# samuel-vitorino/sopro

Measured on AMD Instinct MI355X. Metric: audio_seconds_per_second, higher is better.
Workload: dtype f32; 1 GPU; Sopro-135M synthesize, 32 utterances x 200 frames per GPU (BASELINE configs[1]), S=64 text tokens, 32 distinct 150-frame reference voice(s) per batch prepared outside the timed region, top_p=0.9 T=1.05 anti_loop (reference defaults), synthetic weights with EOS suppressed; batch_per_gpu=32, frames=200, voices_per_batch=32, parallelism=replicas x1 (utterance sharding, no collective), lanes_per_gpu=4

## Files before the change

include/sopro_hip.h:

```cpp
#ifndef SOPRO_HIP_H
#define SOPRO_HIP_H

#include <stdint.h>

#ifdef __cplusplus
extern "C" {
#endif

#define SOPRO_ABI_VERSION 43

const char* sopro_last_error(void);
int sopro_abi_version(void);
int sopro_build_flags(void);
int sopro_set_lds_floor(int bytes);
int sopro_set_host_wait(int blocking);
int sopro_device_info(int device, int* out4);

int sopro_capture_begin(void* stream);
int sopro_capture_end(void* stream, void** graph_exec_out);
int sopro_graph_launch(void* graph_exec, void* stream);
int sopro_graph_launch_n(void* graph_exec, void* stream, int32_t n);
int sopro_graph_destroy(void* graph_exec);
int sopro_stream_create_cu_range(int first_cu, int n_cus, void** stream_out);
int sopro_stream_create_cu_mask(const uint32_t* mask, int32_t words, void** stream_out);
int sopro_stream_destroy(void* stream);
int sopro_host_alloc(int64_t bytes, void** out);
int sopro_host_free(void* p);
int sopro_copy_to_host_async(void* dst_host, const void* src_dev, int64_t bytes, void* stream);

enum { SOPRO_PRO_NONE = 0, SOPRO_PRO_ELU = 1, SOPRO_PRO_ADDVEC = 2 };
enum { SOPRO_EPI_NONE = 0, SOPRO_EPI_GELU = 1, SOPRO_EPI_GLU = 2, SOPRO_EPI_RES = 3, SOPRO_EPI_TANH = 4,
       SOPRO_EPI_GLU_DW = 5 ,
       SOPRO_EPI_ROPE = 6  };

typedef struct sopro_gemm_args {
  const float* A; int64_t lda; int64_t a_seg_stride;
  const float* W; int64_t ldw;
  const float* bias;
  float* C; int64_t ldc; int64_t c_seg_stride;
  const float* R; int64_t ldr; int64_t r_seg_stride;
  const float* scale;
  const float* pro_vec;
  long long* dbg;
  int32_t M, N, K, rows_per_seg;
  int32_t prologue, epilogue;
} sopro_gemm_args;
int sopro_gemm_f32(const sopro_gemm_args* args, void* stream);
int sopro_gemm_set_tile_override(int cfg);

typedef struct sopro_gemm_split_ext {
  int32_t a_format;
  int32_t c_mode;
  float* C2; int64_t ldc2; int64_t c2_seg_stride;
  int32_t rms_norm; float rms_eps;
  int32_t ksplit;
  int32_t n_tickets;
  float* ws; int64_t ws_bytes;
  int32_t* tickets;
  int32_t group_m;
  float acc_scale;
  int32_t* range_events;
  const float* rope_cos; const float* rope_sin;
  int32_t rope_cols, rope_dh, rope_pos0, rope_rows_per_seg;
  const float* ln_stats;
  float* ln_stats_out;
} sopro_gemm_split_ext;
int sopro_gemm_bf16x3(const sopro_gemm_args* a, const void* packed_w, const sopro_gemm_split_ext* ext, void* stream);
int64_t sopro_packed_w_rows_bytes(int32_t N, int32_t K);
int sopro_pack_w_rows_bf16(const float* W, int64_t ldw, int32_t N, int32_t K, void* packed, void* stream);
int sopro_gemm_8p_takes(const sopro_gemm_args* a, const sopro_gemm_split_ext* ext);
int sopro_gemm_bf16x3_8p(const sopro_gemm_args* a, const void* w_rows, const sopro_gemm_split_ext* ext, void* stream);
int sopro_gemm_bf16x6(const sopro_gemm_args* a, const void* packed_w, const sopro_gemm_split_ext* ext, void* stream);
int sopro_gemm_bf16x1(const sopro_gemm_args* a, const void* packed_w, const sopro_gemm_split_ext* ext, void* stream);
int sopro_pack_w_bf16(const float* W, int64_t ldw, int32_t N, int32_t K, int32_t pieces, void* packed, void* stream);
int sopro_pack_w_f16x2(const float* W, int64_t ldw, int32_t N, int32_t K, float wscale, void* packed, void* stream);
float sopro_f16x3_a_scale(void);
int sopro_gemm_f16x3(const sopro_gemm_args* a, const void* packed_w, const sopro_gemm_split_ext* ext, void* stream);
int64_t sopro_packed_w_bytes(int32_t N, int32_t K, int32_t pieces);
int sopro_gemm_bf16_set_tile_override(int cfg);
int sopro_gemm_set_group_m(int g);
int sopro_gemm_auto_ksplit(int32_t M, int32_t N, int32_t K, int32_t pieces, int32_t f16, int32_t epilogue, int64_t ws_bytes, int32_t n_tickets);

typedef struct sopro_skinny_args {
  const float* X; int64_t ldx;
  const float* W; int64_t ldw;
  const float* bias;
  float* Y; int64_t ldy;
  const float* R; int64_t ldr;
  const float* scale;
  float* ring;
  const float* dw_w;
  const float* dw_b;
  const int32_t* step;
  const float* Xp; int64_t xp_stride;
  int64_t y_part_stride;
  long long* dbg;
  float eps;
  int32_t B, N, K, epilogue;
  int32_t ring_len, ring_bcap, dil, ksize;
  int32_t np, ksplit, rms_norm;
  int32_t w_layout;
  const float* aux_W; const float* aux_bias; const float* aux_R; float* aux_Y;
  int64_t aux_ldy, aux_ldr, aux_y_part_stride;
  int32_t aux_tiles, aux_flags;
  int32_t ring_format;
  int32_t mt, nt;
} sopro_skinny_args;
int sopro_skinny_f32(const sopro_skinny_args* args, void* stream);
int sopro_pack_skinny_w(const float* W, int64_t ldw, int32_t N, int32_t K, int32_t glu, float* out, void* stream);
int64_t sopro_skinny_packed_floats(int32_t N, int32_t K, int32_t glu);
int sopro_pack_skinny_w_bf16(const float* W, int64_t ldw, int32_t N, int32_t K, int32_t glu, void* out, void* stream);

int sopro_fill2d_u32(void* p, int64_t pitch, int32_t rows, int32_t width, uint32_t value, void* stream);
int sopro_copy2d_u32(void* dst, int64_t dpitch, const void* src, int64_t spitch, int32_t rows, int32_t width, void* stream);
int sopro_nar_seed_i32(int32_t* tokens, int32_t Q, const int32_t* cb0, int64_t cb0_bstride, int32_t B, int32_t T, int32_t vmax, void* stream);
int sopro_cvt_f32_bf16(const float* src, void* dst, int64_t n, void* stream);
int sopro_cvt_bf16_f32(const void* src, float* dst, int64_t n, void* stream);
enum { SOPRO_NORM_RMS = 0, SOPRO_NORM_LN = 1 };
int sopro_norm_f32(const float* x, int64_t ldx, int64_t x_seg_stride , float* out, int64_t ldo, const float* w, const float* b,
                   const float* mul, const float* add, int32_t rows, int32_t rows_per_seg, int32_t C,
                   float eps, int32_t kind, void* stream);
int sopro_row_stats_f32(const float* x, int64_t ldx, int64_t x_seg_stride , int32_t rows, int32_t rows_per_seg, int32_t C,
                        float* stats, void* stream);
int sopro_rms_match_f32(const float* a, const float* x, float* out, int32_t rows, int32_t C, void* stream);
int sopro_tanh_affine_f32(const float* in, float* out, float c0, float c1, int64_t n, void* stream);
int sopro_add_pos_f32(const float* rowvec, const float* table, float* out, int32_t B, int32_t T, int32_t C,
                      int32_t pos0, void* stream);
int sopro_masked_mean_f32(const float* x, const int32_t* lens, float* out, int32_t B, int32_t T, int32_t C,
                          void* stream);

int sopro_stats_pool_f32(const float* h, const float* logit, const int32_t* lens, float* out, int32_t B, int32_t T,
                         int32_t C, void* stream);
int sopro_l2norm_f32(const float* x, float* out, int32_t rows, int32_t C, float eps, void* stream);

int sopro_dwconv_f32(const float* x, const float* w, const float* bias, const float* res, float* out,
                     const int32_t* lens, int32_t B, int32_t T, int32_t C, int32_t ksize, int32_t dil,
                     int32_t left, int32_t mode, void* stream);

int sopro_codebook_sum_f32(const int32_t* tok, int32_t ldt, const int32_t* col, const int32_t* off, const float* wq,
                           int32_t nq, const float* table, int64_t table_rows, const float* base, float alpha,
                           float beta, float* out, int64_t ldo, int64_t o_seg_stride, int32_t rows,
                           int32_t rows_per_seg, int32_t D, void* stream);
int sopro_text_embed_f32(const int32_t* ids, const int32_t* lens, const float* table, int64_t table_rows,
                         const float* pe, float* out, int32_t B, int32_t T, int32_t C, void* stream);
int sopro_argmax_rows_f32(const float* x, int64_t ldx, int32_t* out, int64_t ldo, int32_t inner, int32_t rows, int32_t N,
                          void* stream);
int sopro_argmax_partials_i32(const float* partials, int64_t ldp, int32_t* out, int64_t ldo, int32_t heads, int32_t per_head, int32_t V,
                              int32_t rows, void* stream);

int sopro_fir1_f32(const float* x, int64_t x_seg_stride, int32_t n_in, const float* w, const float* bias, float* out,
                   int64_t ldo, int64_t o_seg_stride, int32_t B, int32_t n_out, int32_t C, int32_t K, int32_t stride,
                   int32_t left, void* stream);
int sopro_rvq_assign_f32(const float* scores, int64_t lds, int32_t V, const float* table, float* res, int64_t ldr,
                         int32_t D, int32_t* codes, int64_t ldc, int32_t rows, void* stream);

typedef struct sopro_attn_args {
  const float* Q; int64_t ldq; int64_t q_bstride;
  const float* K; int64_t ldk; int64_t k_bstride;
  const float* V; int64_t ldv; int64_t v_bstride;
  float* O; int64_t ldo; int64_t o_bstride;
  const int32_t* klens;
  int32_t B, H, dh, Tq, Tk;
  int32_t causal, q_pos0, k_pos0, window;
  float scale;
  const int32_t* kv_index;
} sopro_attn_args;
int sopro_attention_f32(const sopro_attn_args* args, void* stream);
int sopro_attention_split_bf16(const sopro_attn_args* args, int32_t passes, void* stream);
int sopro_attn_decode_f32(const sopro_attn_args* args, void* stream);
typedef struct sopro_xattn_args {
  const float* X; int64_t ldx;
  const float* Xp; int64_t xp_stride;
  const float* norm_w;
  const float* Kp; const float* Vp;
  const int32_t* klens;
  float* Y; int64_t y_part_stride;
  float eps, gate, scale;
  int32_t np, B, H, D, S_cap;
  const float* Qp; int64_t qp_stride;
  int32_t nqp, k_unfolded;
  int32_t kv_format;
} sopro_xattn_args;
int sopro_xattn_step_f32(const sopro_xattn_args* args, void* stream);

int sopro_rope_f32(float* x, int64_t ldx, const float* cos_t, const float* sin_t, int32_t rows,
                   int32_t rows_per_seg, int32_t pos0, int32_t H, int32_t dh, void* stream);

int sopro_upsample2_f32(const float* x, const float* w, float* y, int64_t y_seg_stride, int32_t B, int32_t T,
                        int32_t C, void* stream);
int sopro_final_conv_f32(const float* h, int64_t h_seg_stride, const float* w, float bias, float* wav,
                         int64_t wav_seg_stride, int32_t B, int32_t T, void* stream);

int sopro_seanet_tail_f32(const float* h, int64_t h_seg_stride, const float* w1, const float* b1, const float* w2,
                          const float* b2, const float* wf, float bf, float* wav, int64_t wav_seg_stride, int32_t B,
                          int32_t T, void* stream);
int sopro_seanet_tail_p_f32(const float* h, int64_t h_seg_stride, const float* w1, const float* b1, const float* w2,
                            const float* b2, const float* wf, float bf, float* wav, int64_t wav_seg_stride, int32_t B,
                            int32_t T, int32_t passes, void* stream);
int sopro_seanet_res128_f32(const float* h, int64_t h_seg_stride, const float* w1, const float* b1, const float* w2, const float* b2,
                            float* out, int64_t out_seg_stride, int32_t B, int32_t T, void* stream);
int sopro_seanet_res128_p_f32(const float* h, int64_t h_seg_stride, const float* w1, const float* b1, const float* w2, const float* b2,
                              float* out, int64_t out_seg_stride, int32_t B, int32_t T, int32_t passes , void* stream);
int sopro_seanet_res_set_tiles(int tiles);
int sopro_seanet_up128_f32(const float* x, int64_t x_seg_stride, const float* w, const float* bias, float* out,
                           int64_t out_seg_stride, int32_t B, int32_t T, int32_t passes, void* stream);
int sopro_seanet_res128_bf16(const void* h, int64_t h_seg_stride, const float* w1, const float* b1, const float* w2, const float* b2,
                             void* out, int64_t out_seg_stride, int32_t B, int32_t T, void* stream);
int sopro_seanet_up128_bf16(const void* x, int64_t x_seg_stride, const float* w, const float* bias, void* out, int64_t out_seg_stride,
                            int32_t B, int32_t T, void* stream);
int sopro_seanet_tail_bf16(const void* h, int64_t h_seg_stride, const float* w1, const float* b1, const float* w2, const float* b2,
                           const float* wf, float bf, float* wav, int64_t wav_seg_stride, int32_t B, int32_t T, void* stream);
int sopro_seanet_up_set_tiles(int tiles);
int sopro_seanet_uptail_f32(const float* x, int64_t x_seg_stride, const float* wu, const float* bu, const float* w1, const float* b1,
                            const float* w2, const float* b2, const float* wf, float bf, float* wav, int64_t wav_seg_stride, int32_t B,
                            int32_t T, int32_t passes, void* stream);
int sopro_seanet_uptail_bf16(const void* x, int64_t x_seg_stride, const float* wu, const float* bu, const float* w1, const float* b1,
                             const float* w2, const float* b2, const float* wf, float bf, float* wav, int64_t wav_seg_stride, int32_t B,
                             int32_t T, void* stream);
int sopro_seanet_uptail_set_tiles(int tiles);
int sopro_seanet_tail_set_tiles(int tiles);

typedef struct sopro_prof_row {
  char family[40];
  int64_t launches, gpu_bound;
// ... 251 lines not shown
```

sopro_amd/csrc/gemm_8p.hip:

```cpp
#include "common.h"
#include "gemm_epilogue.h"
#include "gemm_host.h"

namespace {

constexpr int P_BM = 256, P_BN = 256, P_NT = 512;
constexpr int P_ROWB = 128;
constexpr int P_TILE = 256 * P_ROWB;
constexpr int P_BUF = 2 * P_TILE;
constexpr int P_LDS = 2 * P_BUF;
constexpr int P_CLD = 128 + 4;
static_assert(2 * 64 * P_CLD * 4 <= P_LDS, "epilogue tiles alias the operand buffers");

typedef __bf16 pbf16x8 __attribute__((ext_vector_type(8)));
typedef unsigned pu32x4 __attribute__((ext_vector_type(4)));
typedef __attribute__((address_space(3))) void p_lds_void;
typedef const __attribute__((address_space(1))) void p_glb_void;

__device__ __forceinline__ pbf16x8 pfrag(const pu32x4& v) { return __builtin_bit_cast(pbf16x8, v); }
__device__ __forceinline__ void dma16(const void* g, unsigned lds_off) {
  __builtin_amdgcn_global_load_lds((p_glb_void*)(uintptr_t)g, (p_lds_void*)(uintptr_t)lds_off, 16, 0, 0);
}

template <int EPI, int OUT>
__global__ __launch_bounds__(P_NT, 1) void gemm_8p_kernel(const sopro_gemm_args g, const unsigned char* __restrict__ Wr, const sopro_gemm_split_ext ext) {
  extern __shared__ __attribute__((aligned(1024))) unsigned char smem[];
  const int tid = threadIdx.x, lane = tid & 63, wave = __builtin_amdgcn_readfirstlane(tid >> 6);
  const int wm = wave >> 2, wn = wave & 3;
  const int ntn = g.N / P_BN;
  const int bid = xcd_contiguous((int)blockIdx.x, (int)gridDim.x);
  int mt = bid / ntn, nt = bid % ntn;
  if (ext.group_m > 1) {
    const int ntm_all = (g.M + P_BM - 1) / P_BM;
    const int per = ext.group_m * ntn;
    const int grp = bid / per, rem = bid - grp * per;
    const int first = grp * ext.group_m;
    const int gsz = min(ntm_all - first, ext.group_m);
    mt = first + rem % gsz;
    nt = rem / gsz;
  }
  const int m0 = mt * P_BM, n0 = nt * P_BN;
  const int KT = g.K >> 5;
  const int64_t ldw = (int64_t)g.K * 4;

  const unsigned char* asrc[2][2];
  const unsigned char* wsrc[2][2];
  const int rps = g.rows_per_seg;
#pragma unroll
  for (int h = 0; h < 2; ++h)
#pragma unroll
    for (int q = 0; q < 2; ++q) {
      const int r = 128 * h + 8 * (wave + 8 * q) + (lane >> 3);
      const int ch = (lane & 7) ^ ((r >> 1) & 7);
      const int m = min(m0 + r, g.M - 1);
      const int seg = m / rps, rr = m - seg * rps;
      asrc[h][q] = reinterpret_cast<const unsigned char*>(g.A) + ((int64_t)seg * g.a_seg_stride + (int64_t)rr * g.lda) * 4 + ch * 16;
      wsrc[h][q] = Wr + (int64_t)(n0 + r) * ldw + ch * 16;
    }
  const unsigned lds0 = (unsigned)(uintptr_t)smem;
  auto issue_one = [&](bool isW, int h, int kt, int buf, int q) {
    const int ktc = min(kt, KT - 1);
    const unsigned char* src = (isW ? wsrc[h][q] : asrc[h][q]) + (int64_t)ktc * P_ROWB;
    dma16(src, lds0 + buf * P_BUF + (isW ? P_TILE : 0) + (128 * h + 8 * (wave + 8 * q)) * P_ROWB);
  };

  const int frow = lane & 31, fg = lane >> 5;
  const int swz = (frow >> 1) & 7;
  int foff[2][2];
#pragma unroll
  for (int p = 0; p < 2; ++p)
#pragma unroll
    for (int s = 0; s < 2; ++s) foff[p][s] = ((p * 4 + s * 2 + fg) ^ swz) * 16;
  const int arow = (wm * 32 + frow) * P_ROWB;
  const int brow = (wn * 32 + frow) * P_ROWB;

  f32x16 acc[4][2];
#pragma unroll
  for (int i = 0; i < 4; ++i)
#pragma unroll
    for (int j = 0; j < 2; ++j)
#pragma unroll
      for (int r = 0; r < 16; ++r) acc[i][j][r] = 0.f;

  pu32x4 af[2][2][2];
  pu32x4 bf[2][2][2];
  auto read_a = [&](int buf, int qi) {
    const unsigned char* base = smem + buf * P_BUF + arow + qi * 2 * 64 * P_ROWB;
#pragma unroll
    for (int i = 0; i < 2; ++i)
#pragma unroll
      for (int s = 0; s < 2; ++s)
#pragma unroll
        for (int p = 0; p < 2; ++p) af[i][s][p] = *reinterpret_cast<const pu32x4*>(base + i * 64 * P_ROWB + foff[p][s]);
  };
  auto read_b = [&](int buf, int j) {
    const unsigned char* base = smem + buf * P_BUF + P_TILE + brow + j * 128 * P_ROWB;
#pragma unroll
    for (int s = 0; s < 2; ++s)
#pragma unroll
      for (int p = 0; p < 2; ++p) bf[j][s][p] = *reinterpret_cast<const pu32x4*>(base + foff[p][s]);
  };
  auto phase_mfma = [&](int qi, int j, bool isW, int h, int kt, int buf) {
    constexpr int PA[3] = {1, 0, 0}, PB[3] = {0, 1, 0};
    int n = 0;
#pragma unroll
    for (int s = 0; s < 2; ++s)
#pragma unroll
      for (int q = 0; q < 3; ++q)
#pragma unroll
        for (int i = 0; i < 2; ++i) {
          acc[qi * 2 + i][j] = __builtin_amdgcn_mfma_f32_32x32x16_bf16(pfrag(af[i][s][PA[q]]), pfrag(bf[j][s][PB[q]]), acc[qi * 2 + i][j], 0, 0, 0);
          ++n;
          if (n == 4 || n == 8) {
            __builtin_amdgcn_sched_barrier(0);
            issue_one(isW, h, kt, buf, n == 4 ? 0 : 1);
            __builtin_amdgcn_sched_barrier(0);
          }
        }
  };
#define P_PHASE(QI, J, W_, H_, KT_, B_)                     \
  asm volatile("s_waitcnt vmcnt(6)" ::: "memory");          \
  __builtin_amdgcn_s_barrier();                             \
  asm volatile("s_waitcnt lgkmcnt(0)" ::: "memory");        \
  __builtin_amdgcn_sched_barrier(0);                        \
  __builtin_amdgcn_s_setprio(1);                            \
  phase_mfma(QI, J, W_, H_, KT_, B_);                       \
  __builtin_amdgcn_s_setprio(0);                            \
  __builtin_amdgcn_sched_barrier(0);                        \
  __builtin_amdgcn_s_barrier();

#pragma unroll
  for (int q = 0; q < 2; ++q) issue_one(false, 0, 0, 0, q);
#pragma unroll
  for (int q = 0; q < 2; ++q) issue_one(true, 0, 0, 0, q);
#pragma unroll
  for (int q = 0; q < 2; ++q) issue_one(true, 1, 0, 0, q);
#pragma unroll
  for (int q = 0; q < 2; ++q) issue_one(false, 1, 0, 0, q);
#pragma unroll
  for (int q = 0; q < 2; ++q) issue_one(false, 0, 1, 1, q);
#pragma unroll
  for (int q = 0; q < 2; ++q) issue_one(true, 0, 1, 1, q);
  asm volatile("s_waitcnt vmcnt(8)" ::: "memory");
  __builtin_amdgcn_s_barrier();
  if (wm == 1) __builtin_amdgcn_s_barrier();

  for (int t = 0; t < KT; ++t) {
    const int b = t & 1;
    read_a(b, 0);
    read_b(b, 0);
    P_PHASE(0, 0, true, 1, t + 1, b ^ 1)
    read_b(b, 1);
    P_PHASE(0, 1, false, 1, t + 1, b ^ 1)
    read_a(b, 1);
    P_PHASE(1, 1, false, 0, t + 2, b)
    P_PHASE(1, 0, true, 0, t + 2, b)
  }
#undef P_PHASE
  if (wm == 0) __builtin_amdgcn_s_barrier();
  asm volatile("s_waitcnt vmcnt(0)" ::: "memory");
  __syncthreads();

  float* Cs[2] = {reinterpret_cast<float*>(smem), reinterpret_cast<float*>(smem) + 64 * P_CLD};
#pragma unroll
  for (int i = 0; i < 4; ++i)
#pragma unroll
    for (int j = 0; j < 2; ++j) {
      const int nb = n0 + 128 * j;
      const int n = nb + wn * 32 + frow;
      const float bv[1] = {(g.bias && n < g.N) ? g.bias[n] : 0.f};
      gemm_store_tile<2, 4, 1, 1, EPI, OUT>(g, Cs[(i * 2 + j) & 1], reinterpret_cast<f32x16(&)[1][1]>(acc[i][j]), bv, m0 + 64 * i, nb, &ext, nullptr);
    }
}

__global__ __launch_bounds__(256) void pack_w_rows_kernel(const float* __restrict__ W, int64_t ldw, int N, int K, uint4* __restrict__ out, int64_t total) {
  const int64_t i = (int64_t)blockIdx.x * blockDim.x + threadIdx.x;
  if (i >= total) return;
  const int c = (int)(i & 7);
  const int64_t gi = i >> 3;
  const int kg = (int)(gi % (K >> 5));
  const int n = (int)(gi / (K >> 5));
  const float* src = W + (int64_t)n * ldw + kg * 32 + (c & 3) * 8;
  unsigned w[4];
#pragma unroll
  for (int e = 0; e < 4; ++e) {
    unsigned hi, lo;
    split2_bf16(src[2 * e], src[2 * e + 1], hi, lo);
    w[e] = (c >> 2) ? lo : hi;
  }
  out[i] = make_uint4(w[0], w[1], w[2], w[3]);
}

template <int EPI, int OUT>
int launch_8p(const sopro_gemm_args& g, const void* wrows, const sopro_gemm_split_ext& ext, hipStream_t s) {
  auto kern = gemm_8p_kernel<EPI, OUT>;
  SOPRO_SET_MAX_LDS_ONCE(kern, P_LDS);
  const int ntm = (g.M + P_BM - 1) / P_BM, ntn = g.N / P_BN;
  hipLaunchKernelGGL(kern, dim3(ntm * ntn), dim3(P_NT), P_LDS, s, g, reinterpret_cast<const unsigned char*>(wrows), ext);
  SOPRO_LAUNCH_CHECK();
}

}

extern "C" int64_t sopro_packed_w_rows_bytes(int32_t N, int32_t K) {
  if (N <= 0 || K <= 0 || (K & 31) != 0) return 0;
  return (int64_t)N * K * 4;
}

extern "C" int sopro_pack_w_rows_bf16(const float* W, int64_t ldw, int32_t N, int32_t K, void* packed, void* stream) {
  SOPRO_CHECK_ARG(W && packed && N > 0 && K > 0 && ldw >= K, "bad pointers or sizes");
  SOPRO_CHECK_ARG((K & 31) == 0 && (ldw & 1) == 0 && (reinterpret_cast<uintptr_t>(W) & 7u) == 0, "K % 32 == 0, 8-byte aligned rows");
  SOPRO_CHECK_ARG((reinterpret_cast<uintptr_t>(packed) & 127u) == 0, "packed must be 128-byte aligned");
  const int64_t total = (int64_t)N * (K >> 5) * 8;
  hipLaunchKernelGGL(pack_w_rows_kernel, dim3((unsigned)((total + 255) / 256)), dim3(256), 0, (hipStream_t)stream, W, ldw, N, K,
                     reinterpret_cast<uint4*>(packed), total);
  SOPRO_LAUNCH_CHECK();
}

extern "C" int sopro_gemm_8p_takes(const sopro_gemm_args* a, const sopro_gemm_split_ext* x) {
  if (!a || !x) return 0;
  if (x->a_format != 1 || a->prologue != SOPRO_PRO_NONE || a->epilogue != SOPRO_EPI_NONE || x->rms_norm || x->ln_stats || x->ln_stats_out) return 0;
  if (x->ksplit > 1) return 0;
  if (!(x->c_mode == 0 || x->c_mode == 1 || x->c_mode == 2 || x->c_mode == 4)) return 0;
  if ((a->N % P_BN) != 0 || (a->K & 31) != 0 || a->K < 1024) return 0;
  const int64_t tiles = (int64_t)((a->M + P_BM - 1) / P_BM) * (a->N / P_BN);
  return tiles >= 128 ? 1 : 0;
}

extern "C" int sopro_gemm_bf16x3_8p(const sopro_gemm_args* a, const void* w_rows, const sopro_gemm_split_ext* x, void* stream) {
  SOPRO_CHECK_ARG(a != nullptr && x != nullptr && w_rows != nullptr, "args / ext / w_rows is NULL");
  sopro_gemm_args g = *a;
  sopro_gemm_split_ext ext = *x;
  if (int rc = gemm_check_basic(__func__, g, &ext, w_rows, GEMM_SPLIT_ROWS)) return rc;
  SOPRO_CHECK_ARG((g.N % P_BN) == 0 && (g.K & 31) == 0, "the long-K form takes N % 256 == 0, K % 32 == 0");
  SOPRO_CHECK_ARG(ext.a_format == 1 && g.prologue == SOPRO_PRO_NONE, "A must be split-form rows (a_format 1, no prologue)");
  SOPRO_CHECK_ARG(g.epilogue == SOPRO_EPI_NONE && !ext.rms_norm && !ext.ln_stats && !ext.ln_stats_out && ext.ksplit <= 1,
                  "epilogue NONE, no fused norm, no split-K");
  SOPRO_CHECK_ARG(g.A && g.C && (reinterpret_cast<uintptr_t>(g.A) & 127u) == 0 && (g.lda & 31) == 0 && (g.a_seg_stride & 31) == 0,
                  "split-form A: 128-byte aligned base, lda / a_seg_stride multiples of 32");
  SOPRO_CHECK_ARG((reinterpret_cast<uintptr_t>(w_rows) & 127u) == 0, "w_rows must be 128-byte aligned (sopro_pack_w_rows_bf16)");
  SOPRO_CHECK_ARG(ext.c_mode == 0 || ext.c_mode == 1 || ext.c_mode == 2 || ext.c_mode == 4, "c_mode must be 0, 1, 2 or 4");
  if (int rc = gemm_check_out_rows(__func__, g, ext, true)) return rc;
  hipStream_t s = reinterpret_cast<hipStream_t>(stream);
  switch (ext.c_mode) {
    case 0: return launch_8p<SOPRO_EPI_NONE, 0>(g, w_rows, ext, s);
    case 1: return launch_8p<SOPRO_EPI_NONE, 1>(g, w_rows, ext, s);
    case 2: return launch_8p<SOPRO_EPI_NONE, 2>(g, w_rows, ext, s);
    default: return launch_8p<SOPRO_EPI_NONE, 4>(g, w_rows, ext, s);
  }
}
```

sopro_amd/csrc/gemm_bf16s.hip:

```cpp
#include "common.h"
#include "gemm_epilogue.h"
#include "gemm_host.h"

namespace {

constexpr int BK = 32;


typedef __bf16 bf16x8 __attribute__((ext_vector_type(8)));
typedef _Float16 f16x8 __attribute__((ext_vector_type(8)));
typedef _Float16 f16x2_t __attribute__((ext_vector_type(2)));

__device__ __forceinline__ bf16x8 as_frag(const uint4& v) { return *reinterpret_cast<const bf16x8*>(&v); }
__device__ __forceinline__ f16x8 as_frag16(const uint4& v) { return *reinterpret_cast<const f16x8*>(&v); }

constexpr float A16_SCALE = 8.0f;

template <int NPL, bool F16 = false>
__device__ __forceinline__ void split_pair(float x, float y, unsigned (&pc)[NPL]) {
#pragma unroll
  for (int p = 0; p < NPL; ++p) {
    const f32x2_t v = {x, y};
    if constexpr (F16) {
      const f16x2_t h = __builtin_convertvector(v, f16x2_t);
      pc[p] = *reinterpret_cast<const unsigned*>(&h);
      x -= (float)h[0];
      y -= (float)h[1];
    } else {
      const bf16x2_t h = __builtin_convertvector(v, bf16x2_t);
      pc[p] = *reinterpret_cast<const unsigned*>(&h);
      x -= __uint_as_float(pc[p] << 16);
      y -= __uint_as_float(pc[p] & 0xffff0000u);
    }
  }
}

template <int NPL, int WM, int WN, int TM, int TN, int EPI, int AMODE, int OUT, bool SK, bool F16 = false>
__global__ __launch_bounds__(WM* WN * 64) void gemm_bf16s_kernel(const sopro_gemm_args g, const uint4* __restrict__ Wp,
                                                                 int ksubs, const sopro_gemm_split_ext ext) {
  constexpr int AROW = NPL * 64 + 16;
  constexpr bool FOLD = F16;
  constexpr int NT = WM * WN * 64;
  constexpr int BM = WM * TM * 32;
  constexpr int BN = WN * TN * 32;
  constexpr int A_F4 = BM * 8 / NT;
  constexpr int RSTEP = NT / 8;
  extern __shared__ float4 smem4[];
  unsigned char* As = reinterpret_cast<unsigned char*>(smem4);

  const int tid = threadIdx.x, lane = tid & 63, wave = tid >> 6;
  const int wm = wave / WN, wn = wave % WN;
  const int ntn = (g.N + BN - 1) / BN;
  const int bid = xcd_contiguous((int)blockIdx.x, (int)gridDim.x);
  int mt = bid / ntn, nt = bid % ntn;
  if (ext.group_m > 1) {
    const int ntm_all = (g.M + BM - 1) / BM;
    const int per = ext.group_m * ntn;
    const int grp = bid / per, rem = bid - grp * per;
    const int first = grp * ext.group_m;
    const int gsz = min(ntm_all - first, ext.group_m);
    mt = first + rem % gsz;
    nt = rem / gsz;
  }
  const int m0 = mt * BM, n0 = nt * BN;
  const int lrow = tid >> 3, lc4 = tid & 7;
  const int rps = g.rows_per_seg;
  long long* dbg = g.dbg ? g.dbg + (int64_t)blockIdx.x * 8 : nullptr;
  if (dbg && tid == 0) dbg[0] = clock64();

  static_assert(AMODE != 5 || NPL == 1, "bf16 rows are a one-pass (bf16 mode) operand form");
  constexpr int AES = AMODE == 5 ? 2 : 4;
  const char* ap[A_F4];
#pragma unroll
  for (int i = 0; i < A_F4; ++i) {
    const int m = min(m0 + lrow + i * RSTEP, g.M - 1);
    const int seg = m / rps;
    const int r = m - seg * rps;
    ap[i] = reinterpret_cast<const char*>(g.A) + ((int64_t)seg * g.a_seg_stride + (int64_t)r * g.lda) * AES;
  }
  const int ntiles = (g.N + 31) >> 5;
  const uint4* bp[TN];
#pragma unroll
  for (int j = 0; j < TN; ++j) {
    const int t = min((n0 >> 5) + wn * TN + j, ntiles - 1);
    bp[j] = Wp + ((int64_t)t * ksubs * NPL) * 64 + lane;
  }
  int boff[TN];
#pragma unroll
  for (int j = 0; j < TN; ++j) {
    const int t = min((n0 >> 5) + wn * TN + j, ntiles - 1);
    boff[j] = (t * ksubs * NPL) * 64 + lane;
  }
  float biasv[TN];
#pragma unroll
  for (int j = 0; j < TN; ++j) {
    const int n = n0 + (wn * TN + j) * 32 + (lane & 31);
    biasv[j] = (g.bias && n < g.N) ? g.bias[n] : 0.f;
  }

  float4 raA[A_F4], raB[A_F4];
  float ssq[A_F4];
  float rsc[A_F4];
  float a16max = 0.f;
#pragma unroll
  for (int i = 0; i < A_F4; ++i) { ssq[i] = 0.f; rsc[i] = A16_SCALE; }
  float sapin[A_F4];
#pragma unroll
  for (int i = 0; i < A_F4; ++i) sapin[i] = A16_SCALE;
  float lmu[A_F4], lrs[A_F4];
  float4 pvA = make_float4(0.f, 0.f, 0.f, 0.f), pvB = pvA;
  const int KT = (g.K + BK - 1) / BK;
  const int klast = g.K - 4;

  auto gload = [&](int kt, float4 (&ra)[A_F4], float4& pv) {
    const int k = min(kt * BK + lc4 * 4, klast);
    if constexpr (AMODE == 5) {
#pragma unroll
      for (int i = 0; i < A_F4; ++i) {
        const uint2 v = *reinterpret_cast<const uint2*>(ap[i] + (int64_t)k * 2);
        ra[i].x = __uint_as_float(v.x);
        ra[i].y = __uint_as_float(v.y);
      }
    } else {
#pragma unroll
      for (int i = 0; i < A_F4; ++i) ra[i] = *reinterpret_cast<const float4*>(ap[i] + (int64_t)k * 4);
    }
    if (AMODE == 3) pv = *reinterpret_cast<const float4*>(g.pro_vec + k);
  };
  auto bload = [&](int kt, uint4 (&rb)[TN][2][NPL]) {
#pragma unroll
    for (int j = 0; j < TN; ++j)
#pragma unroll
      for (int s = 0; s < 2; ++s)
#pragma unroll
        for (int p = 0; p < NPL; ++p) rb[j][s][p] = bp[j][((int64_t)(kt * 2 + s) * NPL + p) * 64];
  };
  auto lstore_piece = [&](int buf, float4 (&ra)[A_F4], const float4& pv, int i, bool fresh, bool first) {
    if constexpr (FOLD) {
      if constexpr (AMODE == 4) asm volatile("" : "+v"(rsc[i]), "+v"(ssq[i]));
      else asm volatile("" : "+v"(sapin[i]));
    }
    if constexpr (AMODE == 5) {
      unsigned char* a = As + buf * BM * AROW + lrow * AROW + lc4 * 8;
      *reinterpret_cast<uint2*>(a + i * RSTEP * AROW) = make_uint2(__float_as_uint(ra[i].x), __float_as_uint(ra[i].y));
    } else if constexpr (AMODE == 2) {
      unsigned char* a = As + buf * BM * AROW + lrow * AROW + lc4 * 16;
      *reinterpret_cast<f32x4*>(a + i * RSTEP * AROW) = (f32x4){ra[i].x, ra[i].y, ra[i].z, ra[i].w};
    } else {
      if constexpr (AMODE == 1) {
        ra[i].x = eluf_(ra[i].x); ra[i].y = eluf_(ra[i].y); ra[i].z = eluf_(ra[i].z); ra[i].w = eluf_(ra[i].w);
      } else if constexpr (AMODE == 3) {
        ra[i].x += pv.x; ra[i].y += pv.y; ra[i].z += pv.z; ra[i].w += pv.w;
      } else if constexpr (AMODE == 6) {
        const f32x2_t r2 = {lrs[i], lrs[i]}, n2 = {lmu[i], lmu[i]};
        const f32x2_t lo2 = (f32x2_t){ra[i].x, ra[i].y} * r2 + n2, hi2 = (f32x2_t){ra[i].z, ra[i].w} * r2 + n2;
        ra[i].x = lo2[0]; ra[i].y = lo2[1]; ra[i].z = hi2[0]; ra[i].w = hi2[1];
      }
      if constexpr (AMODE == 4) {
        if (fresh) ssq[i] = fmaf(ra[i].x, ra[i].x, fmaf(ra[i].y, ra[i].y, fmaf(ra[i].z, ra[i].z, fmaf(ra[i].w, ra[i].w, ssq[i]))));
      }
      unsigned char* a = As + buf * BM * AROW + lrow * AROW + lc4 * 8;
      {
        unsigned c0[NPL], c1[NPL];
        if constexpr (F16) {
          const float F16MAX = 65504.0f;
          if constexpr (AMODE == 4) {
            if (first) {
              float mx = fmaxf(fmaxf(fabsf(ra[i].x), fabsf(ra[i].y)), fmaxf(fabsf(ra[i].z), fabsf(ra[i].w)));
              mx = fmaxf(mx, __shfl_xor(mx, 1, 64));
              mx = fmaxf(mx, __shfl_xor(mx, 2, 64));
              mx = fmaxf(mx, __shfl_xor(mx, 4, 64));
              const int ex = (int)((__float_as_uint(mx) >> 23) & 255u);
              rsc[i] = (ex == 0 || ex == 255) ? A16_SCALE : __uint_as_float((unsigned)min(max(261 - ex, 2), 252) << 23);
            }
          }
          const float sa = AMODE == 4 ? rsc[i] : sapin[i];
          const float vx = ra[i].x * sa, vy = ra[i].y * sa, vz = ra[i].z * sa, vw = ra[i].w * sa;
          a16max = fmaxf(a16max, fmaxf(fmaxf(fabsf(vx), fabsf(vy)), fmaxf(fabsf(vz), fabsf(vw))));
          split_pair<NPL, true>(__builtin_amdgcn_fmed3f(vx, -F16MAX, F16MAX), __builtin_amdgcn_fmed3f(vy, -F16MAX, F16MAX), c0);
          split_pair<NPL, true>(__builtin_amdgcn_fmed3f(vz, -F16MAX, F16MAX), __builtin_amdgcn_fmed3f(vw, -F16MAX, F16MAX), c1);
        } else {
          split_pair<NPL>(ra[i].x, ra[i].y, c0);
          split_pair<NPL>(ra[i].z, ra[i].w, c1);
        }
#pragma unroll
        for (int p = 0; p < NPL; ++p) *reinterpret_cast<uint2*>(a + i * RSTEP * AROW + p * 64) = make_uint2(c0[p], c1[p]);
      }
    }
  };
  auto lstore = [&](int buf, float4 (&ra)[A_F4], const float4& pv, bool fresh = true, bool first = false) {
#pragma unroll
    for (int i = 0; i < A_F4; ++i) lstore_piece(buf, ra, pv, i, fresh, first);
  };

  f32x16 acc[TM][TN];
#pragma unroll
  for (int i = 0; i < TM; ++i)
#pragma unroll
    for (int j = 0; j < TN; ++j)
#pragma unroll
      for (int r = 0; r < 16; ++r) acc[i][j][r] = 0.f;

  const int frow = lane & 31, fg = lane >> 5;
  constexpr int NPAIR = NPL == 1 ? 1 : (NPL == 2 ? 3 : 6);
  constexpr int PA[6] = {NPL == 1 ? 0 : (NPL == 2 ? 1 : 2), 0, NPL == 2 ? 0 : 1, 1, 0, 0};
  constexpr int PB[6] = {0, NPL == 2 ? 1 : 2, NPL == 2 ? 0 : 1, 0, 1, 0};
  auto compute = [&](int buf, const uint4 (&rb)[TN][2][NPL]) {
    const unsigned char* a = As + buf * BM * AROW + (wm * TM * 32 + frow) * AROW + fg * 16;
#pragma unroll
    for (int s = 0; s < 2; ++s) {
      uint4 af[TM][NPL];
#pragma unroll
      for (int i = 0; i < TM; ++i)
#pragma unroll
        for (int p = 0; p < NPL; ++p) af[i][p] = *reinterpret_cast<const uint4*>(a + i * 32 * AROW + p * 64 + s * 32);
#pragma unroll
      for (int q = 0; q < NPAIR; ++q)
#pragma unroll
        for (int i = 0; i < TM; ++i)
#pragma unroll
          for (int j = 0; j < TN; ++j)
            if constexpr (F16)
              acc[i][j] = __builtin_amdgcn_mfma_f32_32x32x16_f16(as_frag16(af[i][PA[q]]), as_frag16(rb[j][s][PB[q]]), acc[i][j], 0, 0, 0);
            else
              acc[i][j] = __builtin_amdgcn_mfma_f32_32x32x16_bf16(as_frag(af[i][PA[q]]), as_frag(rb[j][s][PB[q]]), acc[i][j], 0, 0, 0);
    }
  };

  auto compute_spread = [&](int buf, const uint4 (&rb)[TN][2][NPL], int kA, float4 (&ra)[A_F4], float4& pv, int kB, uint4 (&rbn)[TN][2][NPL],
                            float4 (&rs)[A_F4], const float4& pvs, bool fresh_s) {
    constexpr int NB = TN * 2 * NPL, NL = NB + A_F4, NM = 2 * NPAIR * TM * TN;
    constexpr int STRIDE = NM / NL > 0 ? NM / NL : 1;
    const int kcol = min(kA * BK + lc4 * 4, klast);
    if (AMODE == 3) pv = *reinterpret_cast<const float4*>(g.pro_vec + kcol);
    auto issue = [&](int n) {
      if (n < NB) {
        const int j = n / (2 * NPL), ss = (n / NPL) % 2, p = n % NPL;
        const uint4* wk = Wp + (int64_t)__builtin_amdgcn_readfirstlane(kB) * (2 * NPL * 64);
        rbn[j][ss][p] = wk[boff[j] + (ss * NPL + p) * 64];
      } else if (n < NL) {
        const int i = n - NB;
        if constexpr (AMODE == 5) {
          const uint2 v = *reinterpret_cast<const uint2*>(ap[i] + (int64_t)kcol * 2);
          ra[i].x = __uint_as_float(v.x);
          ra[i].y = __uint_as_float(v.y);
        } else {
          ra[i] = *reinterpret_cast<const float4*>(ap[i] + (int64_t)kcol * 4);
        }
      }
    };
    const unsigned char* a = As + buf * BM * AROW + (wm * TM * 32 + frow) * AROW + fg * 16;
    int m = 0, nl = 0;
#pragma unroll
    for (int s = 0; s < 2; ++s) {
      uint4 af[TM][NPL];
#pragma unroll
      for (int i = 0; i < TM; ++i)
#pragma unroll
        for (int p = 0; p < NPL; ++p) af[i][p] = *reinterpret_cast<const uint4*>(a + i * 32 * AROW + p * 64 + s * 32);
#pragma unroll
      for (int q = 0; q < NPAIR; ++q)
#pragma unroll
        for (int i = 0; i < TM; ++i)
#pragma unroll
          for (int j = 0; j < TN; ++j) {
            if constexpr (F16)
              acc[i][j] = __builtin_amdgcn_mfma_f32_32x32x16_f16(as_frag16(af[i][PA[q]]), as_frag16(rb[j][s][PB[q]]), acc[i][j], 0, 0, 0);
            else
              acc[i][j] = __builtin_amdgcn_mfma_f32_32x32x16_bf16(as_frag(af[i][PA[q]]), as_frag(rb[j][s][PB[q]]), acc[i][j], 0, 0, 0);
            ++m;
            if constexpr (FOLD) {
#pragma unroll
              for (int i = 0; i < A_F4; ++i)
                if (m == NM / 2 + i * (NM / 2) / A_F4) {
                  __builtin_amdgcn_sched_barrier(0x104);
                  lstore_piece(buf ^ 1, rs, pvs, i, fresh_s, false);
                }
            }
            if (m % STRIDE == 0 && nl < NL) {
              if constexpr (NPL == 1) {
                __builtin_amdgcn_sched_barrier(0);
                issue(nl++);
                __builtin_amdgcn_sched_barrier(0);
              } else {
                __builtin_amdgcn_sched_barrier(0x786);
                issue(nl++);
                __builtin_amdgcn_sched_barrier(0x786);
              }
            }
          }
    }
#pragma unroll
    for (int n = 0; n < NL; ++n)
      if (n >= nl) issue(n);
  };

  const int KS = SK ? ext.ksplit : 1;
  const int per = (KT + KS - 1) / KS;
  const int kt0 = (int)blockIdx.y * per;
  const int nkt = max(0, min(KT, kt0 + per) - kt0);
  const int ktl = max(kt0, kt0 + nkt - 1);

  uint4 rb0[TN][2][NPL], rb1[TN][2][NPL];
  constexpr bool DEEP = true;
  gload(min(kt0, KT - 1), raA, pvA);
  bload(min(kt0, KT - 1), rb0);
  if (DEEP) gload(min(min(kt0 + 1, ktl), KT - 1), raB, pvB);
  if constexpr (AMODE == 6) {
    const int P = g.K >> 6;
#pragma unroll
    for (int i = 0; i < A_F4; ++i) {
      const float2* st = reinterpret_cast<const float2*>(ext.ln_stats) + (int64_t)min(m0 + lrow + i * RSTEP, g.M - 1) * P;
      float sm = 0.f;
      for (int p = lc4; p < P; p += 8) sm += st[p].x;
      sm += __shfl_xor(sm, 1, 64); sm += __shfl_xor(sm, 2, 64); sm += __shfl_xor(sm, 4, 64);
      const float mean = sm / (float)P;
      float m2 = 0.f;
      for (int p = lc4; p < P; p += 8) {
        const float2 v = st[p];
        const float d = v.x - mean;
        m2 += fmaf(64.0f * d, d, v.y);
      }
      m2 += __shfl_xor(m2, 1, 64); m2 += __shfl_xor(m2, 2, 64); m2 += __shfl_xor(m2, 4, 64);
      lrs[i] = rsqrtf(m2 / (float)g.K + ext.rms_eps);
      lmu[i] = -mean * lrs[i];
    }
  }
  lstore(0, raA, pvA, true, true);
  __syncthreads();
  if (dbg && tid == 0) dbg[1] = clock64();
  {
    int it = 0;
    for (; it + 1 < nkt; it += 2) {
      const int k1 = min(kt0 + it + 1, ktl), k2 = min(kt0 + it + 2, ktl), k3 = min(kt0 + it + 3, ktl);
      compute_spread(0, rb0, k2, raA, pvA, k1, rb1, raB, pvB, true);
      if constexpr (!FOLD) lstore(1, raB, pvB, true);
      __syncthreads();
      compute_spread(1, rb1, k3, raB, pvB, k2, rb0, raA, pvA, it + 2 < nkt);
      if constexpr (!FOLD) lstore(0, raA, pvA, it + 2 < nkt);
      __syncthreads();
    }
    if (it < nkt) {
      compute(0, rb0);
      __syncthreads();
    }
  }
  if (dbg && tid == 0) dbg[2] = clock64();
  if constexpr (SK) {
    constexpr int PER_THREAD = TM * TN * 16;
    const int tile = bid, ntile = gridDim.x;
    float* mine = ext.ws + ((int64_t)((int64_t)blockIdx.y * ntile + tile) * NT + tid) * PER_THREAD;
#pragma unroll
    for (int i = 0; i < TM; ++i)
#pragma unroll
      for (int j = 0; j < TN; ++j)
#pragma unroll
        for (int r = 0; r < 16; r += 4)
          *reinterpret_cast<float4*>(mine + (i * TN + j) * 16 + r) = make_float4(acc[i][j][r], acc[i][j][r + 1], acc[i][j][r + 2], acc[i][j][r + 3]);
    __syncthreads();
    int* flag = reinterpret_cast<int*>(smem4);
    if (tid == 0) {
      __atomic_thread_fence(__ATOMIC_RELEASE);
      const int old = __hip_atomic_fetch_add(ext.tickets + tile, 1, __ATOMIC_ACQ_REL, __HIP_MEMORY_SCOPE_AGENT);
      *flag = old;
      if (old == KS - 1) __hip_atomic_store(ext.tickets + tile, 0, __ATOMIC_RELAXED, __HIP_MEMORY_SCOPE_AGENT);
    }
    __syncthreads();
    if (*flag != KS - 1) return;
    __atomic_thread_fence(__ATOMIC_ACQUIRE);
    __syncthreads();
#pragma unroll
    for (int i = 0; i < TM; ++i)
#pragma unroll
      for (int j = 0; j < TN; ++j)
#pragma unroll
        for (int r = 0; r < 16; ++r) acc[i][j][r] = 0.f;
    const int64_t sl_stride = (int64_t)ntile * NT * PER_THREAD;
    const float* part0 = ext.ws + ((int64_t)tile * NT + tid) * PER_THREAD;
    for (int s0 = 0; s0 < KS; s0 += 16) {
#pragma unroll
      for (int i = 0; i < TM; ++i)
#pragma unroll
        for (int j = 0; j < TN; ++j)
#pragma unroll
          for (int r = 0; r < 16; r += 4) {
            f32x4 v[16];
#pragma unroll
            for (int u = 0; u < 16; ++u) {
              const int sl = min(s0 + u, KS - 1);
              v[u] = __builtin_nontemporal_load(reinterpret_cast<const f32x4*>(part0 + sl * sl_stride + (i * TN + j) * 16 + r));
            }
#pragma unroll
            for (int u = 0; u < 16; ++u) {
              if (s0 + u < KS) {
                acc[i][j][r] += v[u][0]; acc[i][j][r + 1] += v[u][1]; acc[i][j][r + 2] += v[u][2]; acc[i][j][r + 3] += v[u][3];
              }
            }
          }
    }
  }
  float cscale = 1.0f;
  if constexpr (F16) {
    cscale = AMODE == 4 ? ext.acc_scale * A16_SCALE : ext.acc_scale;
    if (ext.range_events && !(a16max <= 65504.0f)) atomicAdd(ext.range_events, 1);
  }
  const float* rs = nullptr;
  if constexpr (AMODE == 4) {
    float* rsl = reinterpret_cast<float*>(smem4) + BM * (BN + 4);
#pragma unroll
    for (int i = 0; i < A_F4; ++i) {
      float v = ssq[i];
      v += __shfl_xor(v, 1, 64);
      v += __shfl_xor(v, 2, 64);
      v += __shfl_xor(v, 4, 64);
      float r = rsqrtf(v / (float)g.K + ext.rms_eps);
      if constexpr (F16) r *= __uint_as_float(0x7f000000u - __float_as_uint(rsc[i])) * cscale;
      if (lc4 == 0) rsl[lrow + i * RSTEP] = r;
    }
    __syncthreads();
    rs = rsl;
  }
  gemm_store_tile<WM, WN, TM, TN, EPI, OUT>(g, reinterpret_cast<float*>(smem4), acc, biasv, m0, n0, &ext, rs, cscale);
  if (dbg && tid == 0) dbg[3] = clock64();
}

template <int NPL, bool F16 = false>
__global__ __launch_bounds__(256) void pack_w_kernel(const float* __restrict__ W, int64_t ldw, int N, int K, uint4* __restrict__ out,
                                                     int ksubs, int64_t total, float wscale = 1.0f) {
  const int64_t i = (int64_t)blockIdx.x * blockDim.x + threadIdx.x;
  if (i >= total) return;
  const int lane = (int)(i & 63);
  const int64_t pk = i >> 6;
  const int p = (int)(pk % NPL);
  const int64_t tk = pk / NPL;
  const int ks = (int)(tk % ksubs);
  const int t = (int)(tk / ksubs);
  const int n = t * 32 + (lane & 31);
  const int k0 = ks * 16 + (lane >> 5) * 8;
  unsigned w[4];
#pragma unroll
  for (int e = 0; e < 4; ++e) {
    const int k = k0 + 2 * e;
    const float x = (n < N && k < K) ? W[(int64_t)n * ldw + k] : 0.f;
    const float y = (n < N && k + 1 < K) ? W[(int64_t)n * ldw + k + 1] : 0.f;
    unsigned pc[NPL];
    if constexpr (F16) split_pair<NPL, true>(x * wscale, y * wscale, pc);
    else split_pair<NPL>(x, y, pc);
    w[e] = pc[p];
  }
  out[i] = make_uint4(w[0], w[1], w[2], w[3]);
}

template <int NPL, int WM, int WN, int TM, int TN, int EPI, int AMODE, int OUT, bool F16 = false>
int launch_one(const sopro_gemm_args& g, const uint4* wp, int ksubs, const sopro_gemm_split_ext& ext, hipStream_t s) {
  constexpr int BM = WM * TM * 32, BN = WN * TN * 32;
  constexpr size_t lds_main = (size_t)2 * BM * (NPL * 64 + 16), lds_epi = (size_t)BM * (BN + 4 + (AMODE == 4 ? 1 : 0)) * sizeof(float);
  constexpr size_t lds = lds_main > lds_epi ? lds_main : lds_epi;
  const int ks = ext.ksplit > 1 ? ext.ksplit : 1;
  auto kern = ks > 1 ? gemm_bf16s_kernel<NPL, WM, WN, TM, TN, EPI, AMODE, OUT, true, F16> : gemm_bf16s_kernel<NPL, WM, WN, TM, TN, EPI, AMODE, OUT, false, F16>;
  constexpr size_t lds_cap = lds > (size_t)96 * 1024 ? lds : (size_t)96 * 1024;
  if (ks > 1) SOPRO_SET_MAX_LDS_ONCE(kern, lds_cap);
  else SOPRO_SET_MAX_LDS_ONCE(kern, lds_cap);
  const size_t lds_req = lds > (size_t)g_sopro_lds_floor ? lds : (size_t)g_sopro_lds_floor;
  const int ntm = (g.M + BM - 1) / BM, ntn = (g.N + BN - 1) / BN;
  if (ks > 1) {
    const int64_t need = (int64_t)ks * ntm * ntn * BM * BN * (int64_t)sizeof(float);
    if (!ext.ws || !ext.tickets || ext.ws_bytes < need || ext.n_tickets < ntm * ntn) {
      sopro_set_error("split-K needs a %lld-byte workspace and %d tickets (got %lld, %d)", (long long)need, ntm * ntn,
                      (long long)ext.ws_bytes, ext.n_tickets);
      return -2;
    }
  }
  hipLaunchKernelGGL(kern, dim3(ntm * ntn, ks), dim3(WM * WN * 64), lds_req, s, g, wp, ksubs, ext);
  SOPRO_LAUNCH_CHECK();
}

inline int amode_of(const sopro_gemm_args& g, const sopro_gemm_split_ext& ext) {
  if (ext.a_format == 1) return 2;
  if (ext.a_format == 2) return 5;
  if (ext.rms_norm) return 4;
  if (ext.ln_stats) return 6;
  return g.prologue == SOPRO_PRO_ELU ? 1 : (g.prologue == SOPRO_PRO_ADDVEC ? 3 : 0);
}

template <int NPL, int WM, int WN, int TM, int TN>
int launch_cfg3(const sopro_gemm_args& g, const uint4* wp, int ksubs, const sopro_gemm_split_ext& ext, hipStream_t s) {
  const int key = g.epilogue * 100 + amode_of(g, ext) * 10 + ext.c_mode;
#define SOPRO_CASE(E, A, O) \
  case (E) * 100 + (A) * 10 + (O): return launch_one<NPL, WM, WN, TM, TN, ((E) == SOPRO_EPI_GELU ? SOPRO_EPI_GELU_FAST : (E)), A, O>(g, wp, ksubs, ext, s)
  switch (key) {
    SOPRO_CASE(SOPRO_EPI_NONE, 0, 0);
    SOPRO_CASE(SOPRO_EPI_GELU, 0, 0);
    SOPRO_CASE(SOPRO_EPI_RES, 0, 0);
    SOPRO_CASE(SOPRO_EPI_ROPE, 0, 0);
    SOPRO_CASE(SOPRO_EPI_NONE, 6, 0);
    SOPRO_CASE(SOPRO_EPI_GELU, 6, 0);
    SOPRO_CASE(SOPRO_EPI_ROPE, 6, 0);
    SOPRO_CASE(SOPRO_EPI_NONE, 1, 0);
    SOPRO_CASE(SOPRO_EPI_RES, 1, 0);
    SOPRO_CASE(SOPRO_EPI_NONE, 0, 3);
    SOPRO_CASE(SOPRO_EPI_NONE, 0, 4);
    SOPRO_CASE(SOPRO_EPI_RES, 0, 3);
    default: break;
  }
  if constexpr (NPL == 1) {
    switch (key) {
      SOPRO_CASE(SOPRO_EPI_NONE, 0, 7);
      SOPRO_CASE(SOPRO_EPI_NONE, 5, 8);
      SOPRO_CASE(SOPRO_EPI_NONE, 5, 7);
      SOPRO_CASE(SOPRO_EPI_RES, 5, 7);
      SOPRO_CASE(SOPRO_EPI_NONE, 5, 6);
      SOPRO_CASE(SOPRO_EPI_NONE, 5, 0);
      default: break;
    }
  }
  if constexpr (NPL == 2) {
    switch (key) {
      SOPRO_CASE(SOPRO_EPI_NONE, 0, 1);
      SOPRO_CASE(SOPRO_EPI_NONE, 0, 2);
      SOPRO_CASE(SOPRO_EPI_NONE, 2, 0);
      SOPRO_CASE(SOPRO_EPI_NONE, 2, 1);
      SOPRO_CASE(SOPRO_EPI_NONE, 2, 2);
      SOPRO_CASE(SOPRO_EPI_NONE, 2, 4);
      SOPRO_CASE(SOPRO_EPI_RES, 2, 1);
      default: break;
    }
  }
#undef SOPRO_CASE
  sopro_set_error("sopro_gemm_bf16x%d: (epilogue %d, prologue %d, a_format %d, c_mode %d) is not an available combination",
                  NPL == 2 ? 3 : NPL, g.epilogue, g.prologue, ext.a_format, ext.c_mode);
  return -2;
}

template <int NPL, int WM, int WN, int TM, int TN, bool F16 = false>
int launch_cfg6(const sopro_gemm_args& g, const uint4* wp, int ksubs, const sopro_gemm_split_ext& ext, hipStream_t s) {
  const int key = g.epilogue * 10 + amode_of(g, ext);
#define SOPRO_CASE(E, A) \
  case (E) * 10 + (A): return launch_one<NPL, WM, WN, TM, TN, (((E) == SOPRO_EPI_GELU && (F16 || NPL != 3)) ? SOPRO_EPI_GELU_FAST : (E)), A, 0, F16>(g, wp, ksubs, ext, s)
  switch (key) {
    SOPRO_CASE(SOPRO_EPI_NONE, 0);
    SOPRO_CASE(SOPRO_EPI_GELU, 0);
    SOPRO_CASE(SOPRO_EPI_RES, 0);
    SOPRO_CASE(SOPRO_EPI_NONE, 3);
    SOPRO_CASE(SOPRO_EPI_GELU, 4);
    SOPRO_CASE(SOPRO_EPI_NONE, 4);
    default: break;
  }
#undef SOPRO_CASE
  if constexpr (WN * TN * 32 >= 64) {
    constexpr int GLU_ = (F16 || NPL != 3) ? SOPRO_EPI_GLU_FAST : SOPRO_EPI_GLU;
    if (key == SOPRO_EPI_GLU * 10) return launch_one<NPL, WM, WN, TM, TN, GLU_, 0, 0, F16>(g, wp, ksubs, ext, s);
    if (key == SOPRO_EPI_GLU * 10 + 4) return launch_one<NPL, WM, WN, TM, TN, GLU_, 4, 0, F16>(g, wp, ksubs, ext, s);
  }
  sopro_set_error("sopro_gemm_%s: (epilogue %d, prologue %d) is not an available combination", F16 ? "f16x3" : (NPL == 3 ? "bf16x6" : "bf16x1"), g.epilogue, g.prologue);
  return -2;
}

#define SOPRO_TILES(X) \
  X(T64, 2, 2, 1, 1) X(T64x128, 2, 2, 1, 2) X(T128x64, 2, 2, 2, 1) X(T128, 2, 2, 2, 2) X(T256x128, 2, 2, 4, 2) X(T128_W8, 2, 4, 2, 1) X(T128_W1x4, 1, 4, 4, 1)
#define SOPRO_TILE(T, WM, WN, TM, TN) T,
enum Tile { SOPRO_TILES(SOPRO_TILE) };
#undef SOPRO_TILE
struct TileSize { int bm, bn; };
TileSize tile_size(Tile t) {
#define SOPRO_TILE(T, WM, WN, TM, TN) if (t == T) return {WM * TM * 32, WN * TN * 32};
  SOPRO_TILES(SOPRO_TILE)
#undef SOPRO_TILE
  return {0, 0};
}

enum Family { BF16X1, BF16X3, BF16X6, F16X3 };

Tile default_tile(Family f, int M, int N, int epilogue) {
  const Tile small = epilogue == SOPRO_EPI_GLU ? T64x128 : T64;
  switch (f) {
    case BF16X3:
      return (N <= 64 || M <= 64) ? T64 : T128;
    case BF16X1: {
      const int64_t t128 = (int64_t)((M + 127) / 128) * ((N + 127) / 128);
      return (N <= 64 || M <= 64 || t128 < 256) ? small : T128;
    }
    case BF16X6:
      return small;
    case F16X3:
      return M >= 8192 ? T128 : small;
  }
  return T64;
}

enum Form { FORM_CFG3, FORM_CFG6, FORM_ARGMAX };

template <int NPL, bool F16, Form FORM>
constexpr bool has_tile(Tile t) {
#ifdef SOPRO_DEV_SWITCHES
  if (t == T128_W1x4) return NPL == 2 && FORM == (F16 ? FORM_CFG6 : FORM_CFG3);
#endif
  if (t == T64 || t == T128) return true;
  if (FORM != FORM_CFG3) return t == (FORM == FORM_ARGMAX ? T128x64 : T64x128);
  return NPL == 2 && (t == T128x64 || t == T256x128 || t == T128_W8);
}

struct Call {
  sopro_gemm_args g;
  sopro_gemm_split_ext ext;
  const uint4* wp;
  int ksubs;
  hipStream_t s;
};

template <int NPL, bool F16, Form FORM>
int launch_tile(Tile t, const Call& c) {
  switch (t) {
#define SOPRO_TILE(T, WM, WN, TM, TN)                                                                                                     \
  case T:                                                                                                                                 \
    if constexpr (!has_tile<NPL, F16, FORM>(T)) break;                                                                                    \
    else if constexpr (FORM == FORM_ARGMAX) return launch_one<NPL, WM, WN, TM, TN, SOPRO_EPI_NONE, 0, 5, F16>(c.g, c.wp, c.ksubs, c.ext, c.s); \
    else if constexpr (FORM == FORM_CFG6) return launch_cfg6<NPL, WM, WN, TM, TN, F16>(c.g, c.wp, c.ksubs, c.ext, c.s);                  \
    else return launch_cfg3<NPL, WM, WN, TM, TN>(c.g, c.wp, c.ksubs, c.ext, c.s);
    SOPRO_TILES(SOPRO_TILE)
#undef SOPRO_TILE
  }
  sopro_set_error("tile %d is not built for this kernel family", (int)t);
  return -2;
}

template <int NPL, bool F16 = false>
int launch_argmax(const Call& c) {
  const sopro_gemm_args& g = c.g;
  const sopro_gemm_split_ext& ext = c.ext;
  SOPRO_CHECK_ARG(g.epilogue == SOPRO_EPI_NONE && g.prologue == SOPRO_PRO_NONE && !ext.rms_norm && ext.a_format == 0,
                  "arg-max output takes a plain contraction (no prologue / epilogue / fused norm)");
  SOPRO_CHECK_ARG(ext.C2 && ext.ldc2 >= (g.N + 63) / 64, "arg-max output: C2 = [M][ldc2 >= ceil(N / 64)] (value, index) pairs");
  static const bool tm1 = SOPRO_DEV_ENV("SOPRO_ARGMAX_TM") != nullptr && SOPRO_DEV_ENV("SOPRO_ARGMAX_TM")[0] == '1';
  static const bool tn1 = SOPRO_DEV_ENV("SOPRO_ARGMAX_TN") != nullptr && SOPRO_DEV_ENV("SOPRO_ARGMAX_TN")[0] == '1';
  Tile t = T64;
  if (g.M >= 8192 && !tm1) t = (g.N >= 2048 && (g.N & 127) == 0 && !tn1) ? T128 : T128x64;
  return launch_tile<NPL, F16, FORM_ARGMAX>(t, c);
}

int check_rope(const sopro_gemm_args& g, const sopro_gemm_split_ext& ext) {
  if (g.epilogue != SOPRO_EPI_ROPE) return 0;
  const int dh = ext.rope_dh;
  SOPRO_CHECK_ARG(ext.rope_cos && ext.rope_sin && aligned16(ext.rope_cos) && aligned16(ext.rope_sin), "EPI_ROPE needs 16-byte aligned cos / sin tables");
  SOPRO_CHECK_ARG(dh >= 8 && dh <= 64 && (dh & (dh - 1)) == 0, "EPI_ROPE: rope_dh must be a power of two in 8..64 (heads must not straddle a 64-column tile)");
  SOPRO_CHECK_ARG(ext.rope_cols > 0 && ext.rope_cols <= g.N && ext.rope_cols % dh == 0, "EPI_ROPE: rope_cols must be whole heads within N");
  SOPRO_CHECK_ARG(ext.rope_rows_per_seg > 0 && ext.rope_pos0 >= 0, "EPI_ROPE: rope_rows_per_seg > 0, rope_pos0 >= 0");
  SOPRO_CHECK_ARG(ext.c_mode == 0 && ext.a_format == 0 && g.prologue == SOPRO_PRO_NONE && !ext.rms_norm, "EPI_ROPE is a plain fp32-rows form");
  SOPRO_CHECK_ARG((g.N & 3) == 0 && (g.ldc & 3) == 0 && (g.c_seg_stride & 3) == 0 && aligned16(g.C), "EPI_ROPE: 16-byte aligned output rows");
  return 0;
}

int check_ln(const sopro_gemm_args& g, const sopro_gemm_split_ext& ext) {
  if (ext.ln_stats) {
    SOPRO_CHECK_ARG((g.K & 63) == 0 && (reinterpret_cast<uintptr_t>(ext.ln_stats) & 7u) == 0, "fused LayerNorm: K % 64 == 0, 8-byte aligned ln_stats");
    SOPRO_CHECK_ARG(ext.a_format == 0 && g.prologue == SOPRO_PRO_NONE && !ext.rms_norm && ext.c_mode == 0, "fused LayerNorm takes plain fp32 rows (no prologue, c_mode 0)");
    SOPRO_CHECK_ARG(g.epilogue == SOPRO_EPI_NONE || g.epilogue == SOPRO_EPI_GELU || g.epilogue == SOPRO_EPI_ROPE, "fused LayerNorm: epilogue NONE, GELU or ROPE");
    SOPRO_CHECK_ARG(ext.rms_eps > 0.f, "fused LayerNorm: rms_eps carries the norm's eps (> 0)");
  }
  if (ext.ln_stats_out) {
    SOPRO_CHECK_ARG(g.epilogue == SOPRO_EPI_RES && ext.c_mode == 0 && (g.N & 63) == 0 && (reinterpret_cast<uintptr_t>(ext.ln_stats_out) & 7u) == 0,
                    "ln_stats_out: an EPI_RES contraction with fp32 output rows, N % 64 == 0, 8-byte aligned pairs");
    SOPRO_CHECK_ARG((g.ldc & 3) == 0 && (g.c_seg_stride & 3) == 0 && aligned16(g.C) && (g.ldr & 3) == 0 && (g.r_seg_stride & 3) == 0 && aligned16(g.R),
                    "ln_stats_out: 16-byte aligned output / residual rows");
  }
  return 0;
}

int check_common(sopro_gemm_args& g, sopro_gemm_split_ext& ext, const void* packed_w) {
  if (int rc = gemm_check_basic(__func__, g, &ext, packed_w, GEMM_PACKED_W)) return rc;
  SOPRO_CHECK_ARG(ext.ksplit >= 0 && ext.ksplit <= 64, "ksplit must be in 0..64");
  SOPRO_CHECK_ARG(ext.ksplit <= 1 || g.dbg == nullptr, "the clock-stamp probe is for unsplit launches");
  return 0;
}

int check_rms(const char* who, const sopro_gemm_args& g, const sopro_gemm_split_ext& ext, bool plain_out) {
  SOPRO_CHECK_AS(who, !ext.rms_norm || ((g.K & 31) == 0 && ext.ksplit <= 1 && g.prologue == SOPRO_PRO_NONE && ext.rms_eps > 0.f && (!plain_out || ext.c_mode == 0)),
                 plain_out ? "fused RMSNorm needs K % 32 == 0, no split-K, no prologue, eps > 0 and a plain output"
                           : "fused RMSNorm needs K % 32 == 0, no split-K, no prologue and eps > 0");
  return 0;
}

int g_group_m = 0;

typedef int (*forms_check)(const char* who, const sopro_gemm_args& g, const sopro_gemm_split_ext& ext);
int prepare(const char* who, const sopro_gemm_args* a, const void* packed_w, const sopro_gemm_split_ext* x, void* stream, bool ext_required,
            forms_check forms, Call& c) {
  SOPRO_CHECK_AS(who, a != nullptr && (x != nullptr || !ext_required), ext_required ? "args / ext is NULL (ext carries acc_scale)" : "args is NULL");
  c.g = *a;
  memset(&c.ext, 0, sizeof(c.ext));
  if (x) c.ext = *x;
  if (c.ext.group_m == 0) c.ext.group_m = g_group_m;
  if (forms)
    if (int rc = forms(who, c.g, c.ext)) return rc;
  if (int rc = check_common(c.g, c.ext, packed_w)) return rc;
  if (int rc = check_ln(c.g, c.ext)) return rc;
  c.wp = reinterpret_cast<const uint4*>(packed_w);
  c.ksubs = (c.g.K + 31) / 32 * 2;
  c.s = reinterpret_cast<hipStream_t>(stream);
  return 0;
}

int forms_bf16x1(const char* who, const sopro_gemm_args& g, const sopro_gemm_split_ext& ext) {
  SOPRO_CHECK_AS(who, (ext.a_format == 0 || ext.a_format == 2) && (ext.c_mode == 0 || (ext.c_mode >= 3 && ext.c_mode <= 8)),
                 "bf16x1 reads fp32 rows (a_format 0) or bf16 rows (2) and writes fp32 rows (c_mode 0, 3, 4), arg-max partials (5) or bf16 rows (6, 7, 8)");
  if (ext.a_format == 2 || ext.c_mode >= 6) {
    SOPRO_CHECK_AS(who, !ext.rms_norm && g.prologue == SOPRO_PRO_NONE && (g.epilogue == SOPRO_EPI_NONE || g.epilogue == SOPRO_EPI_RES),
                   "bf16 rows: no prologue / fused norm, epilogue NONE or RES (the activation is applied by the producer: c_mode 7 / 8)");
    SOPRO_CHECK_AS(who, ext.a_format != 2 || ((g.lda & 3) == 0 && (g.a_seg_stride & 3) == 0), "bf16 A rows: lda, a_seg_stride multiples of 4 elements");
    SOPRO_CHECK_AS(who, g.epilogue != SOPRO_EPI_RES || ext.c_mode >= 6, "EPI_RES with bf16 A writes bf16 rows (its skip operand R is bf16 then)");
  }
  return check_rms(who, g, ext, true);
}

template <bool F16>
int forms_x6(const char* who, const sopro_gemm_args& g, const sopro_gemm_split_ext& ext) {
  if (F16) SOPRO_CHECK_AS(who, ext.acc_scale > 0.f, "acc_scale = 1 / (sopro_f16x3_a_scale() * the weight's pack scale) must be set");
  SOPRO_CHECK_AS(who, ext.a_format == 0 && (ext.c_mode == 0 || ext.c_mode == 5),
                 F16 ? "the f16 three-pass path reads fp32 rows and writes fp32 rows, or arg-max partials (c_mode 5)"
                     : "the six-pass path reads fp32 rows and writes fp32 rows, or arg-max partials (c_mode 5)");
  return check_rms(who, g, ext, false);
}

}

extern "C" int sopro_gemm_set_group_m(int g) {
  g_group_m = g > 1 ? g : 0;
  return 0;
}

static bool eight_waves(const sopro_gemm_args& g) {
  static const bool on = SOPRO_DEV_ENV("SOPRO_GEMM_W8") != nullptr && SOPRO_DEV_ENV("SOPRO_GEMM_W8")[0] == '1';
  return on && g.N >= 512 && g.M >= 1024;
}

#ifdef SOPRO_DEV_SWITCHES
bool sopro_gemm_astat_takes(const sopro_gemm_args& g, const sopro_gemm_split_ext& ext);
int sopro_gemm_astat_bf16x3(const sopro_gemm_args& g, const void* packed_w, hipStream_t s);
#endif

static int g_tile_override = 0;
extern "C" int sopro_gemm_bf16_set_tile_override(int cfg) {
  g_tile_override = cfg;
  return 0;
}

extern "C" int sopro_gemm_auto_ksplit(int32_t M, int32_t N, int32_t K, int32_t pieces, int32_t f16, int32_t epilogue, int64_t ws_bytes, int32_t n_tickets) {
  static const bool no_splitk = getenv("SOPRO_NO_SPLITK") && getenv("SOPRO_NO_SPLITK")[0] == '1';
  if (no_splitk || M <= 0 || N <= 0 || K <= 0) return 1;
  if (f16 && M >= 8192) return 1;
  const TileSize t = tile_size(default_tile(f16 ? F16X3 : pieces == 3 ? BF16X6 : pieces == 1 ? BF16X1 : BF16X3, M, N, epilogue));
  const int64_t tiles = (int64_t)((M + t.bm - 1) / t.bm) * ((N + t.bn - 1) / t.bn);
  const int kt = (K + 31) / 32;
  if (tiles >= 96 || kt < 32 || tiles > n_tickets) return 1;
  int ks = (int)lrint(sqrt(2.5 * kt));
  if (ks > 16) ks = 16;
  if (ks > 512 / (int)tiles) ks = 512 / (int)tiles;
  if (ks < 1) ks = 1;
  while (ks > 1 && (int64_t)ks * tiles * t.bm * t.bn * 4 > ws_bytes) --ks;
  return ks;
}

extern "C" int64_t sopro_packed_w_bytes(int32_t N, int32_t K, int32_t pieces) {
  if (N <= 0 || K <= 0 || pieces < 1 || pieces > 3) return 0;
  return (int64_t)((N + 31) / 32) * ((K + 31) / 32 * 2) * pieces * 64 * 16;
}

extern "C" int sopro_pack_w_bf16(const float* W, int64_t ldw, int32_t N, int32_t K, int32_t pieces, void* packed, void* stream) {
  SOPRO_CHECK_ARG(W && packed && N > 0 && K > 0 && ldw >= K, "bad pointers or sizes");
  SOPRO_CHECK_ARG(pieces >= 1 && pieces <= 3, "pieces must be 1 (bf16x1), 2 (bf16x3) or 3 (bf16x6)");
  SOPRO_CHECK_ARG(aligned16(packed), "packed must be 16-byte aligned");
  const int ksubs = (K + 31) / 32 * 2;
  const int64_t total = (int64_t)((N + 31) / 32) * ksubs * pieces * 64;
  const dim3 grid((unsigned)((total + 255) / 256));
  if (pieces == 1)
    hipLaunchKernelGGL(pack_w_kernel<1>, grid, dim3(256), 0, (hipStream_t)stream, W, ldw, N, K, reinterpret_cast<uint4*>(packed), ksubs, total);
  else if (pieces == 2)
    hipLaunchKernelGGL(pack_w_kernel<2>, grid, dim3(256), 0, (hipStream_t)stream, W, ldw, N, K, reinterpret_cast<uint4*>(packed), ksubs, total);
  else
    hipLaunchKernelGGL(pack_w_kernel<3>, grid, dim3(256), 0, (hipStream_t)stream, W, ldw, N, K, reinterpret_cast<uint4*>(packed), ksubs, total);
  SOPRO_LAUNCH_CHECK();
}

extern "C" int sopro_gemm_bf16x3(const sopro_gemm_args* a, const void* packed_w, const sopro_gemm_split_ext* x, void* stream) {
  Call c;
  if (int rc = prepare(__func__, a, packed_w, x, stream, false, nullptr, c)) return rc;
  const sopro_gemm_args& g = c.g;
  const sopro_gemm_split_ext& ext = c.ext;
  SOPRO_CHECK_ARG(g.prologue == SOPRO_PRO_NONE || g.prologue == SOPRO_PRO_ELU, "prologue must be NONE or ELU");
  SOPRO_CHECK_ARG(g.epilogue == SOPRO_EPI_NONE || g.epilogue == SOPRO_EPI_GELU || g.epilogue == SOPRO_EPI_RES || g.epilogue == SOPRO_EPI_ROPE,
                  "epilogue must be NONE, GELU, RES or ROPE");
  if (int rc = check_rope(g, ext)) return rc;
  SOPRO_CHECK_ARG(ext.a_format == 0 || ext.a_format == 1, "a_format must be 0 (fp32) or 1 (split form)");
  SOPRO_CHECK_ARG(!ext.rms_norm, "fused RMSNorm is a six-pass (sopro_gemm_bf16x6) feature");
  if (ext.a_format == 1) {
    SOPRO_CHECK_ARG(g.prologue == SOPRO_PRO_NONE, "split-form A carries its activation already");
    SOPRO_CHECK_ARG((g.K & 31) == 0 && (g.lda & 31) == 0 && (g.a_seg_stride & 31) == 0 && (reinterpret_cast<uintptr_t>(g.A) & 127u) == 0,
                    "split-form A: K, lda, a_seg_stride multiples of 32 and a 128-byte aligned base");
  }
  SOPRO_CHECK_ARG(ext.c_mode >= 0 && ext.c_mode <= 4, "c_mode must be 0..4");
  if (int rc = gemm_check_out_rows(__func__, g, ext, true)) return rc;
#ifdef SOPRO_DEV_SWITCHES
  if (g_tile_override == 9 && sopro_gemm_astat_takes(g, ext)) return sopro_gemm_astat_bf16x3(g, packed_w, c.s);
#endif
  Tile t = default_tile(BF16X3, g.M, g.N, g.epilogue);
  static const bool narrow = SOPRO_DEV_ENV("SOPRO_GEMM_NARROW") != nullptr && SOPRO_DEV_ENV("SOPRO_GEMM_NARROW")[0] == '1';
  if (t == T128 && eight_waves(g)) t = T128_W8;
  else if (t == T128 && narrow && g.N <= 512 && g.M >= 8192) t = T128x64;
  switch (g_tile_override) {
    case 1: t = T128; break;
    case 2: t = T256x128; break;
    case 4: t = T128x64; break;
    case 5: t = T64; break;
    case 7: t = T128_W8; break;
#ifdef SOPRO_DEV_SWITCHES
    case 3: t = T128_W1x4; break;
#endif
    default: break;
  }
  return launch_tile<2, false, FORM_CFG3>(t, c);
}

extern "C" int sopro_gemm_bf16x1(const sopro_gemm_args* a, const void* packed_w, const sopro_gemm_split_ext* x, void* stream) {
  Call c;
  if (int rc = prepare(__func__, a, packed_w, x, stream, false, forms_bf16x1, c)) return rc;
  const sopro_gemm_args& g = c.g;
  const sopro_gemm_split_ext& ext = c.ext;
  if (ext.c_mode == 5) return launch_argmax<1>(c);
  if (int rc = gemm_check_out_rows(__func__, g, ext, false)) return rc;
  const Tile t = default_tile(BF16X1, g.M, g.N, g.epilogue);
  if (ext.rms_norm || g.epilogue == SOPRO_EPI_GLU || g.prologue == SOPRO_PRO_ADDVEC) {
    SOPRO_CHECK_ARG(ext.c_mode == 0 && (g.prologue == SOPRO_PRO_NONE || g.prologue == SOPRO_PRO_ADDVEC), "GLU / RMSNorm / ADDVEC forms write plain fp32");
    return launch_tile<1, false, FORM_CFG6>(t, c);
  }
  SOPRO_CHECK_ARG(g.prologue == SOPRO_PRO_NONE || g.prologue == SOPRO_PRO_ELU, "prologue must be NONE or ELU (or ADDVEC, with a plain fp32 output)");
  SOPRO_CHECK_ARG(g.epilogue == SOPRO_EPI_NONE || g.epilogue == SOPRO_EPI_GELU || g.epilogue == SOPRO_EPI_RES || g.epilogue == SOPRO_EPI_ROPE,
                  "epilogue must be NONE, GELU, RES or ROPE (or GLU, with a plain fp32 output)");
  if (int rc = check_rope(g, ext)) return rc;
  return launch_tile<1, false, FORM_CFG3>(t, c);
}

template <int NPL, bool F16>
static int gemm_x6(const char* who, const sopro_gemm_args* a, const void* packed_w, const sopro_gemm_split_ext* x, void* stream, int env_tile) {
  Call c;
  if (int rc = prepare(who, a, packed_w, x, stream, F16, forms_x6<F16>, c)) return rc;
  SOPRO_CHECK_AS(who, c.g.prologue == SOPRO_PRO_NONE || c.g.prologue == SOPRO_PRO_ADDVEC, "prologue must be NONE or ADDVEC");
  SOPRO_CHECK_AS(who, c.g.epilogue == SOPRO_EPI_NONE || c.g.epilogue == SOPRO_EPI_GELU || c.g.epilogue == SOPRO_EPI_RES || c.g.epilogue == SOPRO_EPI_GLU,
                 "epilogue must be NONE, GELU, RES or GLU");
  if (c.ext.c_mode == 5) return launch_argmax<NPL, F16>(c);
  const Tile small = default_tile(BF16X6, c.g.M, c.g.N, c.g.epilogue);
  Tile t = env_tile ? small : default_tile(F16 ? F16X3 : BF16X6, c.g.M, c.g.N, c.g.epilogue);
  switch (g_tile_override ? g_tile_override : env_tile) {
    case 1: t = T128; break;
#ifdef SOPRO_DEV_SWITCHES
    case 3: if (F16) t = T128_W1x4; break;
#endif
    case 4: t = T64x128; break;
    case 5: t = small; break;
    default: break;
  }
  return launch_tile<NPL, F16, FORM_CFG6>(t, c);
}

extern "C" int sopro_gemm_bf16x6(const sopro_gemm_args* a, const void* packed_w, const sopro_gemm_split_ext* x, void* stream) {
  return gemm_x6<3, false>(__func__, a, packed_w, x, stream, 0);
}

extern "C" int sopro_pack_w_f16x2(const float* W, int64_t ldw, int32_t N, int32_t K, float wscale, void* packed, void* stream) {
  SOPRO_CHECK_ARG(W && packed && N > 0 && K > 0 && ldw >= K, "bad pointers or sizes");
  SOPRO_CHECK_ARG(aligned16(packed), "packed must be 16-byte aligned");
  int ex = 0;
  SOPRO_CHECK_ARG(wscale > 0.f && frexpf(wscale, &ex) == 0.5f, "wscale must be a power of two (the scaling has to be exact)");
  const int ksubs = (K + 31) / 32 * 2;
  const int64_t total = (int64_t)((N + 31) / 32) * ksubs * 2 * 64;
  hipLaunchKernelGGL((pack_w_kernel<2, true>), dim3((unsigned)((total + 255) / 256)), dim3(256), 0, (hipStream_t)stream, W, ldw, N, K,
                     reinterpret_cast<uint4*>(packed), ksubs, total, wscale);
  SOPRO_LAUNCH_CHECK();
}

extern "C" float sopro_f16x3_a_scale(void) { return A16_SCALE; }

extern "C" int sopro_gemm_f16x3(const sopro_gemm_args* a, const void* packed_w, const sopro_gemm_split_ext* x, void* stream) {
  static const int env_tile = SOPRO_DEV_ENV("SOPRO_F16X3_TILE") ? atoi(SOPRO_DEV_ENV("SOPRO_F16X3_TILE")) : 0;
  return gemm_x6<2, true>(__func__, a, packed_w, x, stream, env_tile);
}
```

sopro_amd/csrc/gemm_epilogue.h:

```cpp
#pragma once
#include "common.h"

constexpr int SOPRO_EPI_GELU_FAST = 100;
constexpr int SOPRO_EPI_GLU_FAST = 101;
template <int WM, int WN, int TM, int TN, int EPI, int OUT = 0>
__device__ __forceinline__ void gemm_store_tile(const sopro_gemm_args& g, float* __restrict__ Cs, f32x16 (&acc)[TM][TN],
                                                const float (&biasv)[TN], int m0, int n0,
                                                const sopro_gemm_split_ext* __restrict__ ext = nullptr,
                                                const float* __restrict__ rs = nullptr, float cscale = 1.0f) {
  constexpr int NT = WM * WN * 64;
  constexpr int BM = WM * TM * 32;
  constexpr int BN = WN * TN * 32;
  const int tid = threadIdx.x, lane = tid & 63, wave = tid >> 6;
  const int wm = wave / WN, wn = wave % WN;
  const int rps = g.rows_per_seg;
  const bool big = (int64_t)g.M * g.N * (OUT >= 6 ? 2 : 4) >= SOPRO_BIG_BYTES;
  constexpr int CLD = BN + 4;
  constexpr bool RES_AHEAD = EPI == SOPRO_EPI_RES && OUT < 5;
  constexpr int RA_TPR = BN / 4, RA_RPP = NT / RA_TPR, RA_NPASS = BM / RA_RPP;
  float4 rahead[RES_AHEAD ? RA_NPASS : 1];
  const bool whole_tile = m0 + BM <= g.M && n0 + BN <= g.N && (m0 / rps) == ((m0 + BM - 1) / rps);
  if constexpr (RES_AHEAD) {
    const int prow = tid / RA_TPR, ocol = n0 + (tid % RA_TPR) * 4;
    const bool rvec = ((g.N & 3) == 0) && ((g.ldr & 3) == 0) && ((g.r_seg_stride & 3) == 0) && ((reinterpret_cast<uintptr_t>(g.R) & 15u) == 0);
    int m = m0 + prow;
    int seg = m / rps, rr = m - seg * rps;
    if (whole_tile && rvec) {
      const float* rptr = g.R + (int64_t)seg * g.r_seg_stride + (int64_t)rr * g.ldr + ocol;
      const int64_t rstep = (int64_t)RA_RPP * g.ldr;
#pragma unroll
      for (int q = 0; q < RA_NPASS; ++q) rahead[q] = *reinterpret_cast<const float4*>(rptr + q * rstep);
    } else {
#pragma unroll
    for (int q = 0; q < RA_NPASS; ++q) {
      rahead[q] = make_float4(0.f, 0.f, 0.f, 0.f);
      if (ocol < g.N && m < g.M) {
        const float* rptr = g.R + (int64_t)seg * g.r_seg_stride + (int64_t)rr * g.ldr + ocol;
        if (rvec) {
          rahead[q] = *reinterpret_cast<const float4*>(rptr);
        } else {
          rahead[q].x = rptr[0];
          if (ocol + 1 < g.N) rahead[q].y = rptr[1];
          if (ocol + 2 < g.N) rahead[q].z = rptr[2];
          if (ocol + 3 < g.N) rahead[q].w = rptr[3];
        }
      }
      m += RA_RPP; rr += RA_RPP;
      while (rr >= rps) { rr -= rps; ++seg; }
    }
    }
  }
  {
    const int col = lane & 31;
#pragma unroll
    for (int i = 0; i < TM; ++i)
#pragma unroll
      for (int k = 0; k < 4; ++k) {
        const int row0 = (wm * TM + i) * 32 + 8 * k + 4 * (lane >> 5);
        float rs4[4] = {cscale, cscale, cscale, cscale};
        if (rs) {
          const float4 t = *reinterpret_cast<const float4*>(rs + row0);
          rs4[0] = t.x; rs4[1] = t.y; rs4[2] = t.z; rs4[3] = t.w;
        }
#pragma unroll
        for (int j = 0; j < TN; ++j)
#pragma unroll
          for (int e = 0; e < 4; ++e) {
            float p = acc[i][j][4 * k + e] * rs4[e];
            if (rs) asm("" : "+v"(p));
            Cs[(row0 + e) * CLD + (wn * TN + j) * 32 + col] = p + biasv[j];
          }
      }
  }
  __syncthreads();
#ifdef SOPRO_DEV_SWITCHES
  if (g.dbg && tid == 0) g.dbg[(int64_t)blockIdx.x * 8 + 4] = clock64();
#endif
  if constexpr (OUT == 5) {
    constexpr int TPR5 = NT / BM;
    constexpr int CPT = BN / TPR5;
    const int row = tid / TPR5, part = tid % TPR5;
    float best = -INFINITY;
    int bi = 0x7fffffff;
#pragma unroll 8
    for (int c = 0; c < CPT; ++c) {
      const int n = n0 + part * CPT + c;
      const float v = Cs[row * CLD + part * CPT + c];
      if (n < g.N && v > best) { best = v; bi = n; }
    }
    constexpr int GRP = CPT >= 64 ? 1 : 64 / CPT;
    static_assert(BN % 64 == 0 && (CPT >= 64 ? CPT == 64 : 64 % CPT == 0), "arg-max partials are per 64 columns");
#pragma unroll
    for (int o = 1; o < GRP; o <<= 1) {
      const float ov = __shfl_xor(best, o, 64);
      const int oi = __shfl_xor(bi, o, 64);
      if (ov > best || (ov == best && oi < bi)) { best = ov; bi = oi; }
    }
    if (part % GRP == 0 && m0 + row < g.M) {
      float* pp = ext->C2 + ((int64_t)(m0 + row) * ext->ldc2 + n0 / 64 + part / GRP) * 2;
      pp[0] = best;
      pp[1] = __int_as_float(bi);
    }
    return;
  }
  if constexpr (OUT >= 6) {
    constexpr bool hres = EPI == SOPRO_EPI_RES;
    static_assert(EPI == SOPRO_EPI_NONE || EPI == SOPRO_EPI_RES, "bf16 rows take EPI_NONE or EPI_RES");
    constexpr int HTPR = BN / 4, HRPP = NT / HTPR, HNPASS = BM / HRPP;
    const int prow = tid / HTPR, pc4 = tid % HTPR;
    const int ocol = n0 + pc4 * 4;
    const bool col_ok = ocol < g.N;
    float4 sc4 = make_float4(1.f, 1.f, 1.f, 1.f);
    if (hres && g.scale && col_ok) sc4 = make_float4(g.scale[ocol], g.scale[ocol + 1], g.scale[ocol + 2], g.scale[ocol + 3]);
    int m = m0 + prow;
    int seg = m / rps, rr = m - seg * rps;
    char* const rawb = reinterpret_cast<char*>(g.C);
    char* const actb = OUT == 8 ? reinterpret_cast<char*>(ext->C2) : rawb;
    const int64_t ldact = OUT == 8 ? ext->ldc2 : g.ldc, segact = OUT == 8 ? ext->c2_seg_stride : g.c_seg_stride;
    const char* const rb = reinterpret_cast<const char*>(g.R);
    auto at = [&](int64_t sg, int64_t r, int64_t ld, int64_t sstride) { return (sg * sstride + r * ld + ocol) * 2; };
    const float* csrc = Cs + prow * CLD + pc4 * 4;
    constexpr int HB = HNPASS < 8 ? HNPASS : 8;
#pragma unroll 1
    for (int p0 = 0; p0 < HNPASS; p0 += HB) {
      int64_t oraw[HB], oact[HB];
      bool okq[HB];
      uint2 rv[HB];
#pragma unroll
      for (int q = 0; q < HB; ++q) {
        okq[q] = col_ok && m < g.M;
        oraw[q] = at(seg, rr, g.ldc, g.c_seg_stride);
        oact[q] = at(seg, rr, ldact, segact);
        rv[q] = make_uint2(0u, 0u);
        if (hres && okq[q]) rv[q] = *reinterpret_cast<const uint2*>(rb + at(seg, rr, g.ldr, g.r_seg_stride));
        m += HRPP; rr += HRPP;
        while (rr >= rps) { rr -= rps; ++seg; }
      }
#pragma unroll
      for (int q = 0; q < HB; ++q) {
        if (!okq[q]) continue;
        float4 v = *reinterpret_cast<const float4*>(csrc + (p0 + q) * HRPP * CLD);
        if (hres) {
          v.x = __uint_as_float(rv[q].x << 16) + sc4.x * v.x; v.y = __uint_as_float(rv[q].x & 0xffff0000u) + sc4.y * v.y;
          v.z = __uint_as_float(rv[q].y << 16) + sc4.z * v.z; v.w = __uint_as_float(rv[q].y & 0xffff0000u) + sc4.w * v.w;
        }
        unsigned lo_;
        if (OUT != 7) {
          uint2 h;
          split2_bf16(v.x, v.y, h.x, lo_);
          split2_bf16(v.z, v.w, h.y, lo_);
          bulk_store_u2(rawb + oraw[q], h, big);
        }
        if (OUT != 6) {
          uint2 h;
          split2_bf16(eluf_(v.x), eluf_(v.y), h.x, lo_);
          split2_bf16(eluf_(v.z), eluf_(v.w), h.y, lo_);
          bulk_store_u2(actb + oact[q], h, big);
        }
      }
    }
    return;
  }
  constexpr bool glu = EPI == SOPRO_EPI_GLU || EPI == SOPRO_EPI_GLU_FAST;
  constexpr bool res = EPI == SOPRO_EPI_RES;
  if constexpr (glu && OUT == 0) {
    constexpr int GT = BN / 4, GRPP = NT / GT, GNP = BM / GRPP;
    const int prow = tid / GT, t = tid % GT;
    const int grp = t >> 4, u = t & 15;
    const int ocol = ((n0 + grp * 64) >> 6) * 32 + 2 * u;
    const bool col_ok = n0 + grp * 64 < g.N;
    const bool st2 = ((g.ldc & 1) == 0) && ((g.c_seg_stride & 1) == 0) && ((reinterpret_cast<uintptr_t>(g.C) & 7u) == 0);
    const float* csrc = Cs + prow * CLD + grp * 64 + 2 * u;
    auto piece = [&](int q, float* cp) {
      const float2 v = *reinterpret_cast<const float2*>(csrc + q * GRPP * CLD), gt = *reinterpret_cast<const float2*>(csrc + q * GRPP * CLD + 32);
      const float ox = v.x * (EPI == SOPRO_EPI_GLU_FAST ? sigmoid_fast(gt.x) : sigmoidf_(gt.x)), oy = v.y * (EPI == SOPRO_EPI_GLU_FAST ? sigmoid_fast(gt.y) : sigmoidf_(gt.y));
      if (st2) {
        bulk_store_u2(cp, make_uint2(__float_as_uint(ox), __float_as_uint(oy)), big);
      } else {
        cp[0] = ox;
        cp[1] = oy;
      }
    };
    if (!col_ok) return;
    if (m0 + BM <= g.M && (m0 / rps) == ((m0 + BM - 1) / rps)) {
      const int m = m0 + prow, seg = m / rps, rr = m - seg * rps;
      float* cptr = g.C + (int64_t)seg * g.c_seg_stride + (int64_t)rr * g.ldc + ocol;
      const int64_t cstep = (int64_t)GRPP * g.ldc;
#pragma unroll
      for (int q = 0; q < GNP; ++q) {
        piece(q, cptr + q * cstep);
#ifdef SOPRO_DEV_SWITCHES
        if (g.dbg && tid == 0 && q == GNP / 2 - 1) g.dbg[(int64_t)blockIdx.x * 8 + 5] = clock64();
#endif
      }
    } else {
#pragma unroll 1
      for (int q = 0; q < GNP; ++q) {
        const int m = m0 + prow + q * GRPP;
        if (m >= g.M) break;
        const int seg = m / rps, rr = m - seg * rps;
        piece(q, g.C + (int64_t)seg * g.c_seg_stride + (int64_t)rr * g.ldc + ocol);
      }
    }
    return;
  }
  constexpr int TPR = BN / 4;
  constexpr int RPP = NT / TPR;
  constexpr int NPASS = BM / RPP;
  const int prow = tid / TPR, pc4 = tid % TPR;
  const int n_out_total = glu ? g.N / 2 : g.N;
  const int ncol = n0 + pc4 * 4;
  const int ocol = glu ? (ncol >> 6) * 32 + (ncol & 31) : ncol;
  const bool col_ok = ocol < n_out_total && (!glu || ((pc4 * 4) & 32) == 0);
  const bool vec_ok = ((n_out_total & 3) == 0) && ((g.ldc & 3) == 0) && ((g.c_seg_stride & 3) == 0) &&
                      ((reinterpret_cast<uintptr_t>(g.C) & 15u) == 0) &&
                      (!res || (((g.ldr & 3) == 0) && ((g.r_seg_stride & 3) == 0) && ((reinterpret_cast<uintptr_t>(g.R) & 15u) == 0)));
  float4 sc4 = make_float4(1.f, 1.f, 1.f, 1.f);
  if (res && g.scale) {
    sc4.x = ncol + 0 < g.N ? g.scale[ncol + 0] : 1.f; sc4.y = ncol + 1 < g.N ? g.scale[ncol + 1] : 1.f;
    sc4.z = ncol + 2 < g.N ? g.scale[ncol + 2] : 1.f; sc4.w = ncol + 3 < g.N ? g.scale[ncol + 3] : 1.f;
  }
  int m = m0 + prow;
  int seg = m / rps, rr = m - seg * rps;
// ... 126 lines not shown
```

sopro_amd/csrc/gemm_host.h:

```cpp
#pragma once
#include "common.h"

#define SOPRO_CHECK_AS(who, cond, msg)                        \
  do {                                                        \
    if (!(cond)) {                                            \
      sopro_set_error("%s: bad argument: %s", who, msg);      \
      return -2;                                              \
    }                                                         \
  } while (0)

enum gemm_operands {
  GEMM_F32_ROWS,
  GEMM_PACKED_W,
  GEMM_SPLIT_ROWS
};

inline int gemm_check_basic(const char* who, sopro_gemm_args& g, sopro_gemm_split_ext* ext, const void* w, gemm_operands ops) {
  if (g.a_seg_stride == 0) g.a_seg_stride = (int64_t)g.rows_per_seg * g.lda;
  if (g.c_seg_stride == 0) g.c_seg_stride = (int64_t)g.rows_per_seg * g.ldc;
  if (g.r_seg_stride == 0) g.r_seg_stride = (int64_t)g.rows_per_seg * g.ldr;
  if (ext && ext->c2_seg_stride == 0) ext->c2_seg_stride = (int64_t)g.rows_per_seg * ext->ldc2;
  if (ops == GEMM_SPLIT_ROWS) {
    SOPRO_CHECK_AS(who, g.M > 0 && g.N > 0 && g.K > 0 && g.rows_per_seg > 0, "M, N, K, rows_per_seg must be positive");
    return 0;
  }
  const bool packed = ops == GEMM_PACKED_W;
  SOPRO_CHECK_AS(who, g.M > 0 && g.N > 0 && g.K > 0, "M, N, K must be positive");
  SOPRO_CHECK_AS(who, (g.K & 3) == 0, "K must be a multiple of 4");
  SOPRO_CHECK_AS(who, g.rows_per_seg > 0, "rows_per_seg must be positive");
  SOPRO_CHECK_AS(who, g.A && w && (g.C || (ext && ext->c_mode == 5)), packed ? "A, packed_w, C must be non-NULL" : "A, W, C must be non-NULL");
  SOPRO_CHECK_AS(who, aligned16(g.A) && aligned16(w), packed ? "A and packed_w must be 16-byte aligned" : "A and W must be 16-byte aligned");
  SOPRO_CHECK_AS(who, (g.lda & 3) == 0 && (packed || (g.ldw & 3) == 0) && (g.a_seg_stride & 3) == 0,
                 packed ? "lda, a_seg_stride must be multiples of 4" : "lda, ldw, a_seg_stride must be multiples of 4");
  SOPRO_CHECK_AS(who, g.epilogue != SOPRO_EPI_RES || g.R != nullptr, "EPI_RES needs R");
  SOPRO_CHECK_AS(who, g.prologue != SOPRO_PRO_ADDVEC || (g.pro_vec && aligned16(g.pro_vec)), "PRO_ADDVEC needs an aligned pro_vec");
  SOPRO_CHECK_AS(who, g.epilogue != SOPRO_EPI_GLU || (g.N % 64) == 0, "EPI_GLU needs N % 64 == 0 (packed value/gate blocks)");
  return 0;
}

inline int gemm_check_out_rows(const char* who, const sopro_gemm_args& g, const sopro_gemm_split_ext& ext, bool n_apart) {
  if (ext.c_mode >= 6) {
    SOPRO_CHECK_AS(who, (g.N & 3) == 0 && g.C && (reinterpret_cast<uintptr_t>(g.C) & 7u) == 0 && (g.ldc & 3) == 0 && (g.c_seg_stride & 3) == 0 && g.ldc >= g.N,
                   "bf16 output rows must be 8-byte aligned (N, ld, seg stride multiples of 4)");
    SOPRO_CHECK_AS(who, ext.c_mode != 8 || (ext.C2 && (reinterpret_cast<uintptr_t>(ext.C2) & 7u) == 0 && (ext.ldc2 & 3) == 0 && (ext.c2_seg_stride & 3) == 0 && ext.ldc2 >= g.N),
                   "c_mode 8: C2 (the activated bf16 copy) must be given, 8-byte aligned rows");
    SOPRO_CHECK_AS(who, g.epilogue != SOPRO_EPI_RES || ((reinterpret_cast<uintptr_t>(g.R) & 7u) == 0 && (g.ldr & 3) == 0 && (g.r_seg_stride & 3) == 0),
                   "bf16 skip operand rows must be 8-byte aligned");
    return 0;
  }
  if (ext.c_mode < 1 || ext.c_mode > 4) return 0;
  if (n_apart) SOPRO_CHECK_AS(who, (g.N & 3) == 0, "activated output: N % 4 == 0");
  const bool second = ext.c_mode == 2 || ext.c_mode == 4;
  const float* d = second ? ext.C2 : g.C;
  const int64_t ldd = second ? ext.ldc2 : g.ldc, dseg = second ? ext.c2_seg_stride : g.c_seg_stride;
  if (ext.c_mode <= 2)
    SOPRO_CHECK_AS(who, d && (reinterpret_cast<uintptr_t>(d) & 127u) == 0 && (ldd & 31) == 0 && (dseg & 31) == 0 && ldd >= g.N,
                   "split-form output rows must start on 128-byte boundaries (ld, seg stride multiples of 32)");
  else
    SOPRO_CHECK_AS(who, (g.N & 3) == 0 && d && aligned16(d) && (ldd & 3) == 0 && (dseg & 3) == 0 && ldd >= g.N,
                   n_apart ? "activated output rows must be 16-byte aligned (ld, seg stride multiples of 4)"
                           : "activated output rows must be 16-byte aligned (N, ld, seg stride multiples of 4)");
  return 0;
}
```

sopro_amd/csrc/stages.hip:

```cpp
#include <stdlib.h>

#include <algorithm>
#include <map>
#include <string>
#include <vector>

#include "common.h"

int sopro_stream_batch_append(float* cur, float* other, const float* qkv, int32_t hs, int32_t rows, int64_t bstride, int32_t n, int32_t kv_len,
                              int32_t nkeep, hipStream_t s);
int sopro_stream_batch_gather(float* kv, const int32_t* keep, int32_t n_keep, int32_t layers, int32_t rows_cap, int64_t bstride, int32_t hs, int32_t half,
                              int32_t kv_len, hipStream_t s);

namespace {

struct Ten {
  const void* p = nullptr;
  int64_t shape[4] = {0, 0, 0, 0};
  int ndim = 0;
  const float* f() const { return reinterpret_cast<const float*>(p); }
};

struct Wt {
  const float* f32 = nullptr;
  const void* packed = nullptr;
  const void* rows = nullptr;
  int pieces = 0;
  bool f16 = false;
  float acc_scale = 1.f;
};

constexpr float RMS_EPS = 1e-6f;

struct Carver {
  char* base;
  size_t off = 0;
  explicit Carver(void* b) : base(reinterpret_cast<char*>(b)) {}
  template <class T>
  T* take(size_t n) {
    T* p = base ? reinterpret_cast<T*>(base + off) : nullptr;
    off += (n * sizeof(T) + 255) & ~size_t(255);
    return p;
  }
};

struct ArPlan {
  int B = 0, S = 0, S_cap = 0, Tar = 0;
  void* ws = nullptr;
  float *cond, *x[4], *part, *u, *logits, *kp[16], *vp[16], *xp, *params, *rings[16], *nkv, *kvd;
  float *qa = nullptr, *qpart = nullptr;
  bool k_unfold = false;
  float *fold_k = nullptr, *fold_v = nullptr;
  int32_t *klens, *hist, *ctr, *first_eos, *stop_t, *recent;
  uint32_t* nonce;
  uint32_t* key;
  int32_t* row_step;
  sopro_ar_state st;
  void* graph = nullptr;
  int graph_B = 0, graph_S_cap = 0, graph_Tar = 0;
  void* graph_ws = nullptr;
};

}

struct sopro_engine {
  sopro_engine_cfg c;
  std::map<std::string, Ten> t;
  std::map<std::string, Wt> w;
  std::map<std::string, const float*> sk;
  std::vector<void*> owned;
  bool final = false;
  bool has_ar = false, has_nar = false, has_mimi = false, has_cond = false, has_enc = false;
  int32_t *q_col = nullptr, *q_off = nullptr;
  std::vector<int32_t*> nar_cols, nar_offs;
  std::vector<float*> nar_cw, ad_mul, ad_add;
  std::vector<int> nar_known;
  int32_t *sem_col = nullptr, *sem_off = nullptr, *ac_col = nullptr, *ac_off = nullptr;
  float* ones = nullptr;
  ArPlan ar;
  int ar_tiles[4] = {0, 0, 0, 0};
};

namespace {

#define STG(call)                       \
  do {                                  \
    const int rc_ = (call);             \
    if (rc_ != 0) return rc_;           \
  } while (0)

int need(const sopro_engine* e, const std::string& name, const Ten** out, int ndim = 0) {
  auto it = e->t.find(name);
  if (it == e->t.end() || !it->second.p) {
    sopro_set_error("stage API: tensor '%s' was not given to sopro_engine_set_tensor", name.c_str());
    return -2;
  }
  if (ndim && it->second.ndim != ndim) {
    sopro_set_error("stage API: tensor '%s' has %d dimensions, expected %d", name.c_str(), it->second.ndim, ndim);
    return -2;
  }
  *out = &it->second;
  return 0;
}

const Wt& WT(const sopro_engine* e, const std::string& key) {
  static const Wt none;
  auto it = e->w.find(key);
  return it == e->w.end() ? none : it->second;
}

const float* F(const sopro_engine* e, const std::string& name) {
  auto it = e->t.find(name);
  return it == e->t.end() ? nullptr : it->second.f();
}

template <class T>
int dev_alloc(sopro_engine* e, size_t n, T** out) {
  void* p = nullptr;
  SOPRO_HIP(hipMalloc(&p, n * sizeof(T)));
  e->owned.push_back(p);
  *out = reinterpret_cast<T*>(p);
  return 0;
}

template <class T>
int dev_upload(sopro_engine* e, const std::vector<T>& h, T** out) {
  STG(dev_alloc(e, h.size(), out));
  SOPRO_HIP(hipMemcpy(*out, h.data(), h.size() * sizeof(T), hipMemcpyHostToDevice));
  return 0;
}

constexpr int F16X2 = 22;
const char* const NAR_SAFE = "#x6";

int pack_pieces(sopro_engine* e, const std::string& key, const std::string& out_key, int pieces, const char* fold_vec, hipStream_t s,
                bool with_rows = false) {
  const Ten* t;
  STG(need(e, key, &t, 2));
  const int N = (int)t->shape[0], K = (int)t->shape[1];
  const float* src = t->f();
  if (fold_vec) {
    const Ten* v;
    STG(need(e, fold_vec, &v));
    std::vector<float> hw((size_t)N * K), hv(K);
    SOPRO_HIP(hipMemcpy(hw.data(), src, hw.size() * 4, hipMemcpyDeviceToHost));
    SOPRO_HIP(hipMemcpy(hv.data(), v->p, (size_t)K * 4, hipMemcpyDeviceToHost));
    for (int n = 0; n < N; ++n)
      for (int k = 0; k < K; ++k) hw[(size_t)n * K + k] *= hv[k];
    float* d;
    STG(dev_upload(e, hw, &d));
    src = d;
  }
  const bool f16 = pieces == F16X2;
  if (f16) pieces = 2;
  const int64_t bytes = sopro_packed_w_bytes(N, K, pieces);
  char* dst;
  STG(dev_alloc(e, (size_t)bytes, &dst));
  Wt w;
  if (f16) {
    std::vector<float> hw((size_t)N * K);
    SOPRO_HIP(hipMemcpy(hw.data(), src, hw.size() * 4, hipMemcpyDeviceToHost));
    float amax = 0.f;
    for (float v : hw) amax = fmaxf(amax, fabsf(v));
    int ex = 0;
    (void)frexpf(amax, &ex);
    const float wscale = amax > 0.f ? ldexpf(1.0f, 13 - ex + 1) : 1.0f;
    STG(sopro_pack_w_f16x2(src, K, N, K, wscale, dst, s));
    w.f16 = true;
    w.acc_scale = 1.0f / (sopro_f16x3_a_scale() * wscale);
  } else {
    STG(sopro_pack_w_bf16(src, K, N, K, pieces, dst, s));
  }
  if (with_rows && pieces == 2 && !f16 && (K & 31) == 0) {
    char* rows;
    STG(dev_alloc(e, (size_t)sopro_packed_w_rows_bytes(N, K) + 128, &rows));
    rows += (128 - (reinterpret_cast<uintptr_t>(rows) & 127u)) & 127u;
    STG(sopro_pack_w_rows_bf16(src, K, N, K, rows, s));
    w.rows = rows;
  }
  w.f32 = fold_vec ? nullptr : t->f();
  w.packed = dst;
  w.pieces = pieces;
  e->w[out_key] = w;
  return 0;
}

int fold_bias(sopro_engine* e, const std::string& w_key, const std::string& v_key, const std::string& out_key) {
  const Ten *t, *v;
  STG(need(e, w_key, &t, 2));
  STG(need(e, v_key, &v));
  const int N = (int)t->shape[0], K = (int)t->shape[1];
  std::vector<float> hw((size_t)N * K), hv(K), ho(N);
  SOPRO_HIP(hipMemcpy(hw.data(), t->p, hw.size() * 4, hipMemcpyDeviceToHost));
  SOPRO_HIP(hipMemcpy(hv.data(), v->p, (size_t)K * 4, hipMemcpyDeviceToHost));
  for (int n = 0; n < N; ++n) {
    double acc = 0.0;
    for (int k = 0; k < K; ++k) acc += (double)hw[(size_t)n * K + k] * hv[k];
    ho[n] = (float)acc;
  }
  float* d;
  STG(dev_upload(e, ho, &d));
  Ten o;
  o.p = d; o.shape[0] = N; o.ndim = 1;
  e->t[out_key] = o;
  return 0;
}

int plain(sopro_engine* e, const std::string& key) {
  const Ten* t;
  STG(need(e, key, &t));
  Wt w;
  w.f32 = t->f();
  e->w[key] = w;
  return 0;
}

constexpr size_t SPLITK_WS_BYTES = (size_t)32 << 20;
constexpr int SPLITK_TICKETS = 1024;
struct SplitK {
  float* ws = nullptr;
  int32_t* tickets = nullptr;
};

struct G {
  int M = 0, N = 0, K = 0;
  int64_t lda = -1, ldc = -1, ldr = -1, ldw = -1;
  const float *bias = nullptr, *R = nullptr, *scale = nullptr, *pro_vec = nullptr;
  int epi = SOPRO_EPI_NONE, pro = SOPRO_PRO_NONE, rows_per_seg = -1;
  int64_t a_seg = 0, c_seg = 0, r_seg = 0;
  int c_mode = 0;
  int a_fmt = 0;
  float* C2 = nullptr;
  int64_t ldc2 = -1, c2_seg = 0;
  float rms_eps = 0.f;
  const SplitK* sk = nullptr;
  int32_t* range_events = nullptr;
  const float *rope_cos = nullptr, *rope_sin = nullptr;
  int rope_cols = 0, rope_dh = 0, rope_pos0 = 0, rope_rps = 0;
  const float* ln_stats = nullptr;
  float* ln_stats_out = nullptr;
  float ln_eps = 0.f;
};

int attend(const sopro_attn_args& a, hipStream_t s, int split_passes = 0) {
  double pairs = (double)a.Tq * a.Tk;
  if (a.causal) {
    pairs = 0;
    for (int q = 0; q < a.Tq; ++q) {
      const int hi = std::min(a.Tk - 1, a.q_pos0 + q - a.k_pos0), lo = std::max(0, a.q_pos0 + q - a.window + 1 - a.k_pos0);
      pairs += std::max(0, hi - lo + 1);
    }
  }
  sopro_prof_scope prof(split_passes ? "attention_split_kernel" : "attention_kernel", 4.0 * a.dh * pairs * a.B * a.H, s);
  if (split_passes) return sopro_attention_split_bf16(&a, split_passes, s);
  return sopro_attention_f32(&a, s);
}

int gemm(hipStream_t s, const float* A, const Wt& w, const float* w_f32_override, float* C, const G& o) {
  const int n_out = o.epi == SOPRO_EPI_GLU ? o.N / 2 : o.N;
  sopro_gemm_args g;
  memset(&g, 0, sizeof(g));
  g.A = A;
  g.lda = o.lda < 0 ? o.K : o.lda;
  g.a_seg_stride = o.a_seg;
  g.W = w_f32_override ? w_f32_override : w.f32;
  g.ldw = o.ldw < 0 ? o.K : o.ldw;
  g.bias = o.bias;
  g.C = C;
  g.ldc = o.ldc < 0 ? n_out : o.ldc;
  g.c_seg_stride = o.c_seg;
  g.R = o.R;
  g.ldr = o.ldr < 0 ? n_out : o.ldr;
  g.r_seg_stride = o.r_seg;
  g.scale = o.scale;
  g.pro_vec = o.pro_vec;
  g.M = o.M; g.N = o.N; g.K = o.K;
  g.rows_per_seg = o.rows_per_seg < 0 ? o.M : o.rows_per_seg;
  g.prologue = o.pro; g.epilogue = o.epi;
  const bool split = !w_f32_override && w.packed;
  sopro_prof_scope prof(!split ? "gemm_f32_kernel" : w.f16 ? "gemm_f16x3_kernel" : w.pieces == 3 ? "gemm_bf16x6_kernel"
                        : w.pieces == 1 ? "gemm_bf16x1_kernel" : "gemm_bf16x3_kernel", 2.0 * o.M * o.N * o.K, s);
  if (split) {
    sopro_gemm_split_ext x;
    memset(&x, 0, sizeof(x));
    x.c_mode = o.c_mode;
    x.a_format = o.a_fmt;
    x.C2 = o.C2;
    x.ldc2 = o.ldc2 < 0 ? n_out : o.ldc2;
    x.c2_seg_stride = o.c2_seg;
    if (o.rms_eps > 0.f) { x.rms_norm = 1; x.rms_eps = o.rms_eps; }
    x.rope_cos = o.rope_cos; x.rope_sin = o.rope_sin; x.rope_cols = o.rope_cols; x.rope_dh = o.rope_dh; x.rope_pos0 = o.rope_pos0;
    x.rope_rows_per_seg = o.rope_rps;
    x.ln_stats = o.ln_stats; x.ln_stats_out = o.ln_stats_out;
    if (o.ln_stats) x.rms_eps = o.ln_eps;
    if (o.sk && o.sk->ws && o.rms_eps <= 0.f && o.c_mode != 5) {
      const int ks = sopro_gemm_auto_ksplit(o.M, o.N, o.K, w.pieces, w.f16, o.epi, (int64_t)SPLITK_WS_BYTES, SPLITK_TICKETS);
      if (ks > 1) {
        x.ksplit = ks; x.n_tickets = SPLITK_TICKETS; x.ws = o.sk->ws; x.ws_bytes = (int64_t)SPLITK_WS_BYTES; x.tickets = o.sk->tickets;
      }
    }
    if (w.f16) {
      x.acc_scale = w.acc_scale;
      x.range_events = o.range_events;
      return sopro_gemm_f16x3(&g, w.packed, &x, s);
    }
    if (w.pieces == 3) return sopro_gemm_bf16x6(&g, w.packed, &x, s);
    if (w.pieces == 1) return sopro_gemm_bf16x1(&g, w.packed, &x, s);
    if (w.rows) {
      sopro_gemm_split_ext x8 = x;
      x8.ksplit = 0;
      if (sopro_gemm_8p_takes(&g, &x8)) return sopro_gemm_bf16x3_8p(&g, w.rows, &x8, s);
    }
    return sopro_gemm_bf16x3(&g, w.packed, &x, s);
  }
  if (!g.W) {
    sopro_set_error("stage API: a contraction has neither an fp32 nor a packed weight");
    return -2;
  }
  return sopro_gemm_f32(&g, s);
}

int norm(hipStream_t s, const float* x, float* out, const float* w, int rows, int C, float eps, int kind = SOPRO_NORM_RMS,
         const float* b = nullptr, const float* mul = nullptr, const float* add = nullptr, int rows_per_seg = -1, int64_t x_seg = 0) {
  return sopro_norm_f32(x, C, x_seg, out, C, w, b, mul, add, rows, rows_per_seg < 0 ? rows : rows_per_seg, C, eps, kind, s);
}

}

extern "C" {

int sopro_engine_create(const sopro_engine_cfg* cfg, sopro_engine** out) {
  SOPRO_CHECK_ARG(cfg && out, "NULL argument");
  SOPRO_CHECK_ARG(cfg->d_model == 384 && cfg->n_layers_ar >= 1 && cfg->n_layers_ar <= 16 && cfg->n_layers_nar >= 1 && cfg->n_layers_nar <= 16,
                  "d_model must be 384 (kernel family), 1..16 layers");
  SOPRO_CHECK_ARG(cfg->n_stages >= 1 && cfg->n_stages <= 8 && cfg->num_codebooks <= 64 && cfg->mimi_n_ratios >= 1 && cfg->mimi_n_ratios <= 8,
                  "1..8 NAR stages, <= 64 codebooks, 1..8 decoder ratios");
  sopro_engine* e = new sopro_engine();
  e->c = *cfg;
  *out = e;
  return 0;
}

int sopro_engine_set_tensor(sopro_engine* e, const char* name, const void* dev_ptr, const int64_t* shape, int32_t ndim) {
  SOPRO_CHECK_ARG(e && name && dev_ptr && shape && ndim >= 1 && ndim <= 4, "bad arguments");
  SOPRO_CHECK_ARG(!e->final, "the engine is finalized");
  Ten t;
  t.p = dev_ptr;
  t.ndim = ndim;
  for (int i = 0; i < ndim; ++i) t.shape[i] = shape[i];
  e->t[name] = t;
  return 0;
}

int sopro_engine_upload_tensor(sopro_engine* e, const char* name, const float* host_ptr, const int64_t* shape, int32_t ndim, void* stream) {
  SOPRO_CHECK_ARG(e && name && host_ptr && shape && ndim >= 1 && ndim <= 4, "bad arguments");
  SOPRO_CHECK_ARG(!e->final, "the engine is finalized");
  size_t n = 1;
  for (int i = 0; i < ndim; ++i) {
    SOPRO_CHECK_ARG(shape[i] > 0, "empty dimension");
    n *= (size_t)shape[i];
  }
  float* d = nullptr;
  STG(dev_alloc(e, n, &d));
  (void)stream;
  SOPRO_HIP(hipMemcpy(d, host_ptr, n * sizeof(float), hipMemcpyHostToDevice));
  return sopro_engine_set_tensor(e, name, d, shape, ndim);
}

int sopro_engine_set_ar_tiles(sopro_engine* e, int32_t glu, int32_t ff1, int32_t ff2, int32_t head) {
  SOPRO_CHECK_ARG(e != nullptr, "engine is NULL");
  e->ar_tiles[0] = glu; e->ar_tiles[1] = ff1; e->ar_tiles[2] = ff2; e->ar_tiles[3] = head;
  if (e->ar.graph) {
    (void)sopro_graph_destroy(e->ar.graph);
    e->ar.graph = nullptr;
  }
  return 0;
}

int sopro_engine_destroy(sopro_engine* e) {
  if (!e) return 0;
  if (e->ar.graph) (void)sopro_graph_destroy(e->ar.graph);
  for (void* p : e->owned) (void)hipFree(p);
  delete e;
  return 0;
}

int sopro_engine_finalize(sopro_engine* e, void* stream) {
  SOPRO_CHECK_ARG(e && !e->final, "NULL or already finalized engine");
  hipStream_t s = (hipStream_t)stream;
  const sopro_engine_cfg& c = e->c;
  const Ten* t;
  const bool bf16 = c.precision == 1;
  e->has_ar = e->t.count("ar.head.w") != 0;
  e->has_nar = e->t.count("nar.pre.w") != 0;
  e->has_mimi = e->t.count("rvq_proj.w") != 0;
  e->has_cond = e->t.count("text_enc.embed") != 0;
  e->has_enc = e->t.count("enc.conv0.w") != 0;
  if (!e->has_ar && !e->has_nar && !e->has_mimi && !e->has_cond && !e->has_enc) {
    STG(need(e, "ar.blocks.0.glu.w", &t, 2));
  }
  if (e->has_ar) {
    auto pack_skinny = [&](const std::string& key, int glu) -> int {
      STG(need(e, key, &t, 2));
      const int N = (int)t->shape[0], K = (int)t->shape[1];
      const int64_t nfl = sopro_skinny_packed_floats(N, K, glu);
      float* d;
      STG(dev_alloc(e, (size_t)(bf16 ? nfl / 2 : nfl), &d));
      if (bf16) STG(sopro_pack_skinny_w_bf16(t->f(), K, N, K, glu, d, s));
      else STG(sopro_pack_skinny_w(t->f(), K, N, K, glu, d, s));
      e->sk[key] = d;
      return 0;
    };
    for (int i = 0; i < c.n_layers_ar; ++i) {
      const std::string p = "ar.blocks." + std::to_string(i);
      STG(pack_skinny(p + ".glu.w", 1));
      STG(pack_skinny(p + ".ff1.w", 0));
      STG(pack_skinny(p + ".ff2.w", 0));
      for (const char* nm : {".glu.b", ".dw.w", ".dw.b", ".ff1.b", ".ff2.b"}) STG(need(e, p + nm, &t));
      if (c.ar_xattn[i]) {
        const std::string pa = "ar.x_attns." + std::to_string(i);
        for (const char* nm : {".nkv.weight", ".kv.w", ".q.wT", ".o.w"}) STG(need(e, pa + nm, &t));
        if (!bf16 && e->t.count(pa + ".qa.w") && e->t.count(pa + ".qu.w") && e->t.count(pa + ".q.b")) {
          STG(pack_skinny(pa + ".qa.w", 0));
          STG(pack_skinny(pa + ".qu.w", 0));
        }
      }
    }
    STG(pack_skinny("ar.head.w", 0));
    STG(need(e, "ar.head.b", &t));
    STG(need(e, "cb_embed", &t, 2));
  }
  if (e->has_nar) {
    const int np = bf16 ? 1 : F16X2;
    for (int i = 0; i < c.n_layers_nar; ++i) {
      const std::string p = "nar.blocks." + std::to_string(i);
      STG(pack_pieces(e, p + ".glu.w", p + ".glu.wn", np, (p + ".norm.weight").c_str(), s));
      STG(pack_pieces(e, p + ".ff1.w", p + ".ff1.wn", np, (p + ".ff.norm.weight").c_str(), s));
      STG(pack_pieces(e, p + ".ff2.w", p + ".ff2.w", np, nullptr, s));
      if (!bf16) {
        STG(pack_pieces(e, p + ".glu.w", p + ".glu.wn" + NAR_SAFE, 3, (p + ".norm.weight").c_str(), s));
        STG(pack_pieces(e, p + ".ff1.w", p + ".ff1.wn" + NAR_SAFE, 3, (p + ".ff.norm.weight").c_str(), s));
        STG(pack_pieces(e, p + ".ff2.w", p + ".ff2.w" + NAR_SAFE, 3, nullptr, s));
      }
      for (const char* nm : {".glu.b", ".dw.w", ".dw.b", ".ff1.b", ".ff2.b"}) STG(need(e, p + nm, &t));
    }
    STG(pack_pieces(e, "nar.pre.w", "nar.pre.w", np, nullptr, s));
    if (!bf16) STG(pack_pieces(e, "nar.pre.w", std::string("nar.pre.w") + NAR_SAFE, 3, nullptr, s));
    const char* stage_names[8] = {"B", "C", "D", "E", "F", "G", "H", "I"};
    std::vector<int> known = {0};
    for (int sgi = 0; sgi < c.n_stages; ++sgi) {
      const std::string hk = std::string("nar.heads.") + stage_names[sgi];
      STG(pack_pieces(e, hk + ".w", hk + ".w", np, nullptr, s));
      if (!bf16) STG(pack_pieces(e, hk + ".w", hk + ".w" + NAR_SAFE, 3, nullptr, s));
      STG(need(e, hk + ".b", &t));
      std::vector<int32_t> cols(known.begin(), known.end()), offs;
      std::vector<float> cw;
      float mx = -1e30f, sum = 0.f;
      for (int k : known) mx = fmaxf(mx, c.nar_prev_cb_weights[k]);
      for (int k : known) { cw.push_back(expf(c.nar_prev_cb_weights[k] - mx)); sum += cw.back(); }
      for (float& v : cw) v /= sum;
      for (int k : known) offs.push_back(k * c.codebook_size);
      int32_t *dc, *dofs;
      float* dw;
      STG(dev_upload(e, cols, &dc));
      STG(dev_upload(e, offs, &dofs));
      STG(dev_upload(e, cw, &dw));
// ... 1084 lines not shown
```

sopro_amd/hip.py:

```python
from __future__ import annotations

import ctypes as C
import gc
import os
import threading
from typing import List, Optional, Tuple

import torch

_HERE = os.path.dirname(os.path.abspath(__file__))
LIB_PATH = os.path.join(_HERE, "libsopro_hip.so")
ABI_VERSION = 43
DEV_MODE = os.environ.get("SOPRO_DEV", "0") == "1"


def dev_env(name: str, default: str) -> str:
    return os.environ.get(name, default) if DEV_MODE else default


DEFAULT_GROUP_M = 8
PRO_NONE, PRO_ELU, PRO_ADDVEC = 0, 1, 2
EPI_ROPE = 6
EPI_NONE, EPI_GELU, EPI_GLU, EPI_RES, EPI_TANH, EPI_GLU_DW = 0, 1, 2, 3, 4, 5
NORM_RMS, NORM_LN = 0, 1

_p = C.c_void_p
_i32, _i64, _f32 = C.c_int32, C.c_int64, C.c_float


class GemmArgs(C.Structure):
    _fields_ = [("A", _p), ("lda", _i64), ("a_seg_stride", _i64), ("W", _p), ("ldw", _i64), ("bias", _p),
                ("C", _p), ("ldc", _i64), ("c_seg_stride", _i64), ("R", _p), ("ldr", _i64), ("r_seg_stride", _i64),
                ("scale", _p), ("pro_vec", _p), ("dbg", _p), ("M", _i32), ("N", _i32), ("K", _i32), ("rows_per_seg", _i32),
                ("prologue", _i32), ("epilogue", _i32)]


class SplitExt(C.Structure):
    _fields_ = [("a_format", _i32), ("c_mode", _i32), ("C2", _p), ("ldc2", _i64), ("c2_seg_stride", _i64),
                ("rms_norm", _i32), ("rms_eps", _f32), ("ksplit", _i32), ("n_tickets", _i32), ("ws", _p), ("ws_bytes", _i64),
                ("tickets", _p), ("group_m", _i32), ("acc_scale", _f32), ("range_events", _p), ("rope_cos", _p), ("rope_sin", _p),
                ("rope_cols", _i32), ("rope_dh", _i32), ("rope_pos0", _i32), ("rope_rows_per_seg", _i32), ("ln_stats", _p), ("ln_stats_out", _p)]


class SkinnyArgs(C.Structure):
    _fields_ = [("X", _p), ("ldx", _i64), ("W", _p), ("ldw", _i64), ("bias", _p), ("Y", _p), ("ldy", _i64),
                ("R", _p), ("ldr", _i64), ("scale", _p), ("ring", _p), ("dw_w", _p), ("dw_b", _p), ("step", _p),
                ("Xp", _p), ("xp_stride", _i64), ("y_part_stride", _i64), ("dbg", _p), ("eps", _f32),
                ("B", _i32), ("N", _i32), ("K", _i32), ("epilogue", _i32),
                ("ring_len", _i32), ("ring_bcap", _i32), ("dil", _i32), ("ksize", _i32),
                ("np", _i32), ("ksplit", _i32), ("rms_norm", _i32), ("w_layout", _i32),
                ("aux_W", _p), ("aux_bias", _p), ("aux_R", _p), ("aux_Y", _p), ("aux_ldy", _i64), ("aux_ldr", _i64), ("aux_y_part_stride", _i64),
                ("aux_tiles", _i32), ("aux_flags", _i32), ("ring_format", _i32), ("mt", _i32), ("nt", _i32)]


class AttnArgs(C.Structure):
    _fields_ = [("Q", _p), ("ldq", _i64), ("q_bstride", _i64), ("K", _p), ("ldk", _i64), ("k_bstride", _i64),
                ("V", _p), ("ldv", _i64), ("v_bstride", _i64), ("O", _p), ("ldo", _i64), ("o_bstride", _i64),
                ("klens", _p), ("B", _i32), ("H", _i32), ("dh", _i32), ("Tq", _i32), ("Tk", _i32),
                ("causal", _i32), ("q_pos0", _i32), ("k_pos0", _i32), ("window", _i32), ("scale", _f32), ("kv_index", _p)]


class XattnArgs(C.Structure):
    _fields_ = [("X", _p), ("ldx", _i64), ("Xp", _p), ("xp_stride", _i64), ("norm_w", _p), ("Kp", _p), ("Vp", _p), ("klens", _p),
                ("Y", _p), ("y_part_stride", _i64), ("eps", _f32), ("gate", _f32), ("scale", _f32),
                ("np", _i32), ("B", _i32), ("H", _i32), ("D", _i32), ("S_cap", _i32),
                ("Qp", _p), ("qp_stride", _i64), ("nqp", _i32), ("k_unfolded", _i32), ("kv_format", _i32)]


class ArState(C.Structure):
    _fields_ = [("x_cur", _p), ("cond", _p), ("emb", _p), ("hist", _p), ("step", _p), ("row_step", _p),
                ("first_eos", _p), ("stop_t", _p), ("n_stopped", _p), ("recent", _p), ("params", _p), ("seed", C.c_uint64),
                ("B", _i32), ("D", _i32), ("Tar", _i32), ("max_steps", _i32), ("V", _i32), ("bos_row", _i32),
                ("start", _p), ("row_max", _p), ("row_params", _p), ("nonce", _p), ("row_id", _p), ("key", _p), ("dbg", _p)]


AR_MAX_LAYERS = 16


class ArBlock(C.Structure):
    _fields_ = [("glu_w", _p), ("glu_b", _p), ("dw_w", _p), ("dw_b", _p), ("ff1_w", _p), ("ff1_b", _p), ("ff2_w", _p), ("ff2_b", _p),
                ("ring", _p), ("kp", _p), ("vp", _p), ("dil", _i32), ("xattn", _i32), ("gate", _f32), ("pad_", _i32),
                ("qa_w", _p), ("qu_w", _p), ("q_b", _p)]


class ArFrame(C.Structure):
    _fields_ = [("blk", ArBlock * AR_MAX_LAYERS), ("head_w", _p), ("head_b", _p), ("x0", _p), ("xa", _p), ("xb", _p), ("part", _p),
                ("u", _p), ("xp", _p), ("qa", _p), ("qpart", _p), ("logits", _p), ("klens", _p),
                ("n_layers", _i32), ("B", _i32), ("D", _i32), ("S_cap", _i32), ("V1", _i32), ("H", _i32), ("ksize", _i32), ("w_layout", _i32),
                ("tile_glu", _i32), ("tile_ff1", _i32), ("tile_ff2", _i32), ("tile_head", _i32), ("eps", _f32), ("k_unfold", _i32), ("store_format", _i32),
                ("st", ArState)]


class EngineCfg(C.Structure):
    _fields_ = [("d_model", _i32), ("codebook_size", _i32), ("num_codebooks", _i32), ("nar_head_dim", _i32), ("bos_row", _i32),
                ("n_layers_ar", _i32), ("ar_kernel", _i32), ("ar_dilations", _i32 * 16), ("ar_xattn", _i32 * 16), ("ar_gate", _f32 * 16),
                ("n_layers_nar", _i32), ("nar_kernel", _i32), ("nar_dilations", _i32 * 16),
                ("n_stages", _i32), ("stage_first_cb", _i32 * 8), ("stage_n_cb", _i32 * 8), ("nar_mix", (_f32 * 2) * 8),
                ("nar_prev_cb_weights", _f32 * 64),
                ("mimi_hidden", _i32), ("mimi_codebook_dim", _i32), ("mimi_heads", _i32), ("mimi_head_dim", _i32), ("mimi_layers", _i32),
                ("mimi_window", _i32), ("mimi_inter", _i32), ("mimi_n_ratios", _i32), ("mimi_ratios", _i32 * 8), ("mimi_num_filters", _i32),
                ("mimi_kernel", _i32), ("mimi_res_kernel", _i32), ("mimi_last_kernel", _i32), ("mimi_compress", _i32),
                ("mimi_n_semantic", _i32), ("mimi_rope_positions", _i32), ("mimi_norm_eps", _f32), ("mimi_final_bias", _f32), ("precision", _i32),
                ("n_layers_text", _i32), ("ref_enc_layers", _i32), ("ref_xattn_layers", _i32), ("ref_xattn_heads", _i32), ("sv_student_dim", _i32),
                ("enc_kernel", _i32)]


class NarIO(C.Structure):
    _fields_ = [("cond", _p), ("cond_bstride", _i64), ("cb0", _p), ("cb0_bstride", _i64), ("lens", _p), ("tokens", _p), ("range_out", _p),
                ("safe", _i32)]


class MimiStreamState(C.Structure):
    _fields_ = [("kv", _p), ("cap_rows", _i32), ("kv_len", _i32), ("pos", _i32), ("evict", _i32), ("half", _i32)]


class MimiStreamBatch(C.Structure):
    _fields_ = [("kv", _p), ("rows_cap", _i32), ("rows", _i32), ("cap_rows", _i32), ("kv_len", _i32), ("pos", _i32), ("evict", _i32),
                ("half", _i32)]


SYMBOLS = {
    "sopro_last_error": (C.c_char_p, []),
    "sopro_abi_version": (C.c_int, []),
    "sopro_build_flags": (C.c_int, []),
    "sopro_graph_launch_n": (C.c_int, [_p, _p, _i32]),
    "sopro_host_alloc": (C.c_int, [_i64, C.POINTER(_p)]),
    "sopro_host_free": (C.c_int, [_p]),
    "sopro_copy_to_host_async": (C.c_int, [_p, _p, _i64, _p]),
    "sopro_set_lds_floor": (C.c_int, [C.c_int]),
    "sopro_set_host_wait": (C.c_int, [C.c_int]),
    "sopro_device_info": (C.c_int, [C.c_int, C.POINTER(C.c_int)]),
    "sopro_capture_begin": (C.c_int, [_p]),
    "sopro_capture_end": (C.c_int, [_p, C.POINTER(_p)]),
    "sopro_graph_launch": (C.c_int, [_p, _p]),
    "sopro_graph_destroy": (C.c_int, [_p]),
    "sopro_stream_create_cu_range": (C.c_int, [C.c_int, C.c_int, C.POINTER(_p)]),
    "sopro_stream_create_cu_mask": (C.c_int, [_p, _i32, _p]),
    "sopro_stream_destroy": (C.c_int, [_p]),
    "sopro_gemm_f32": (C.c_int, [C.POINTER(GemmArgs), _p]),
    "sopro_gemm_bf16x3": (C.c_int, [_p, _p, _p, _p]),
    "sopro_gemm_bf16x6": (C.c_int, [_p, _p, _p, _p]),
    "sopro_gemm_bf16x1": (C.c_int, [_p, _p, _p, _p]),
    "sopro_pack_w_bf16": (C.c_int, [_p, _i64, _i32, _i32, _i32, _p, _p]),
    "sopro_fill2d_u32": (C.c_int, [_p, _i64, _i32, _i32, C.c_uint32, _p]),
    "sopro_copy2d_u32": (C.c_int, [_p, _i64, _p, _i64, _i32, _i32, _p]),
    "sopro_pack_w_f16x2": (C.c_int, [_p, _i64, _i32, _i32, _f32, _p, _p]),
    "sopro_f16x3_a_scale": (C.c_float, []),
    "sopro_gemm_f16x3": (C.c_int, [_p, _p, _p, _p]),
    "sopro_packed_w_bytes": (C.c_int64, [_i32, _i32, _i32]),
    "sopro_packed_w_rows_bytes": (C.c_int64, [_i32, _i32]),
    "sopro_pack_w_rows_bf16": (C.c_int, [_p, _i64, _i32, _i32, _p, _p]),
    "sopro_gemm_8p_takes": (C.c_int, [_p, _p]),
    "sopro_gemm_auto_ksplit": (C.c_int, [C.c_int32, C.c_int32, C.c_int32, C.c_int32, C.c_int32, C.c_int32, C.c_int64, C.c_int32]),
    "sopro_gemm_bf16x3_8p": (C.c_int, [_p, _p, _p, _p]),
    "sopro_gemm_bf16_set_tile_override": (C.c_int, [C.c_int]),
    "sopro_gemm_set_group_m": (C.c_int, [C.c_int]),
    "sopro_seanet_tail_set_tiles": (C.c_int, [C.c_int]),
    "sopro_seanet_res_set_tiles": (C.c_int, [C.c_int]),
    "sopro_seanet_res128_bf16": (C.c_int, [_p, _i64, _p, _p, _p, _p, _p, _i64, _i32, _i32, _p]),
    "sopro_seanet_up128_bf16": (C.c_int, [_p, _i64, _p, _p, _p, _i64, _i32, _i32, _p]),
    "sopro_seanet_tail_bf16": (C.c_int, [_p, _i64, _p, _p, _p, _p, _p, _f32, _p, _i64, _i32, _i32, _p]),
    "sopro_seanet_up_set_tiles": (C.c_int, [C.c_int]),
    "sopro_seanet_uptail_set_tiles": (C.c_int, [C.c_int]),
    "sopro_seanet_uptail_f32": (C.c_int, [_p, _i64, _p, _p, _p, _p, _p, _p, _p, _f32, _p, _i64, _i32, _i32, _i32, _p]),
    "sopro_seanet_uptail_bf16": (C.c_int, [_p, _i64, _p, _p, _p, _p, _p, _p, _p, _f32, _p, _i64, _i32, _i32, _p]),
    "sopro_seanet_up128_f32": (C.c_int, [_p, _i64, _p, _p, _p, _i64, _i32, _i32, _i32, _p]),
    "sopro_seanet_res128_f32": (C.c_int, [_p, _i64, _p, _p, _p, _p, _p, _i64, _i32, _i32, _p]),
    "sopro_gemm_set_tile_override": (C.c_int, [C.c_int]),
    "sopro_pack_skinny_w": (C.c_int, [_p, _i64, _i32, _i32, _i32, _p, _p]),
    "sopro_pack_skinny_w_bf16": (C.c_int, [_p, _i64, _i32, _i32, _i32, _p, _p]),
    "sopro_skinny_packed_floats": (_i64, [_i32, _i32, _i32]),
    "sopro_skinny_f32": (C.c_int, [C.POINTER(SkinnyArgs), _p]),
    "sopro_row_stats_f32": (C.c_int, [_p, _i64, _i64, _i32, _i32, _i32, _p, _p]),
    "sopro_norm_f32": (C.c_int, [_p, _i64, _i64, _p, _i64, _p, _p, _p, _p, _i32, _i32, _i32, _f32, _i32, _p]),
    "sopro_rms_match_f32": (C.c_int, [_p, _p, _p, _i32, _i32, _p]),
    "sopro_tanh_affine_f32": (C.c_int, [_p, _p, _f32, _f32, _i64, _p]),
    "sopro_add_pos_f32": (C.c_int, [_p, _p, _p, _i32, _i32, _i32, _i32, _p]),
    "sopro_masked_mean_f32": (C.c_int, [_p, _p, _p, _i32, _i32, _i32, _p]),
    "sopro_stats_pool_f32": (C.c_int, [_p, _p, _p, _p, _i32, _i32, _i32, _p]),
    "sopro_l2norm_f32": (C.c_int, [_p, _p, _i32, _i32, _f32, _p]),
    "sopro_dwconv_f32": (C.c_int, [_p, _p, _p, _p, _p, _p, _i32, _i32, _i32, _i32, _i32, _i32, _i32, _p]),
    "sopro_codebook_sum_f32": (C.c_int, [_p, _i32, _p, _p, _p, _i32, _p, _i64, _p, _f32, _f32, _p, _i64, _i64, _i32, _i32, _i32, _p]),
    "sopro_text_embed_f32": (C.c_int, [_p, _p, _p, _i64, _p, _p, _i32, _i32, _i32, _p]),
    "sopro_argmax_rows_f32": (C.c_int, [_p, _i64, _p, _i64, _i32, _i32, _i32, _p]),
    "sopro_argmax_partials_i32": (C.c_int, [_p, _i64, _p, _i64, _i32, _i32, _i32, _i32, _p]),
    "sopro_fir1_f32": (C.c_int, [_p, _i64, _i32, _p, _p, _p, _i64, _i64, _i32, _i32, _i32, _i32, _i32, _i32, _p]),
    "sopro_rvq_assign_f32": (C.c_int, [_p, _i64, _i32, _p, _p, _i64, _i32, _p, _i64, _i32, _p]),
    "sopro_attention_f32": (C.c_int, [C.POINTER(AttnArgs), _p]),
    "sopro_attention_split_bf16": (C.c_int, [C.POINTER(AttnArgs), C.c_int32, _p]),
    "sopro_attn_decode_f32": (C.c_int, [C.POINTER(AttnArgs), _p]),
    "sopro_xattn_step_f32": (C.c_int, [C.POINTER(XattnArgs), _p]),
    "sopro_rope_f32": (C.c_int, [_p, _i64, _p, _p, _i32, _i32, _i32, _i32, _i32, _p]),
    "sopro_upsample2_f32": (C.c_int, [_p, _p, _p, _i64, _i32, _i32, _i32, _p]),
    "sopro_final_conv_f32": (C.c_int, [_p, _i64, _p, _f32, _p, _i64, _i32, _i32, _p]),
    "sopro_seanet_tail_f32": (C.c_int, [_p, _i64, _p, _p, _p, _p, _p, _f32, _p, _i64, _i32, _i32, _p]),
    "sopro_seanet_res128_p_f32": (C.c_int, [_p, _i64, _p, _p, _p, _p, _p, _i64, _i32, _i32, _i32, _p]),
    "sopro_seanet_tail_p_f32": (C.c_int, [_p, _i64, _p, _p, _p, _p, _p, _f32, _p, _i64, _i32, _i32, _i32, _p]),
    "sopro_engine_create": (C.c_int, [C.POINTER(EngineCfg), C.POINTER(_p)]),
    "sopro_engine_set_tensor": (C.c_int, [_p, C.c_char_p, _p, C.POINTER(_i64), _i32]),
    "sopro_engine_finalize": (C.c_int, [_p, _p]),
    "sopro_engine_destroy": (C.c_int, [_p]),
    "sopro_ar_workspace_bytes": (_i64, [_p, _i32, _i32, _i32]),
    "sopro_ar_begin": (C.c_int, [_p, _p, _i32, _p, _p, _p, _i32, _i32, C.POINTER(_f32), C.c_uint64, C.c_uint32, _p]),
    "sopro_ar_run_graph": (C.c_int, [_p, _i32, _p]),
    "sopro_ar_tokens": (C.c_int, [_p, _p, _p, _p, _p]),
    "sopro_nar_workspace_bytes": (_i64, [_p, _i32, _i32]),
    "sopro_nar_refine": (C.c_int, [_p, _p, _p, _i64, _p, _p, _i32, _i32, _p, _p]),
    "sopro_nar_refine_io": (C.c_int, [_p, _p, C.POINTER(NarIO), _i32, _i32, _p]),
    "sopro_nar_seed_i32": (C.c_int, [_p, _i32, _p, _i64, _i32, _i32, _i32, _p]),
    "sopro_mimi_workspace_bytes": (_i64, [_p, _i32, _i32]),
    "sopro_mimi_decode": (C.c_int, [_p, _p, _p, _i32, _i32, _p, _p]),
    "sopro_mimi_chunk_rows": (_i32, [_i32, _i32]),
    "sopro_mimi_decode_parts": (C.c_int, [_p, _p, _p, _i32, _i32, _p, _i32, _p]),
    "sopro_mimi_stream_kv_bytes": (_i64, [_p, _i32]),
    "sopro_mimi_stream_init": (C.c_int, [_p, C.POINTER(MimiStreamState), _p, _i32]),
    "sopro_mimi_stream_trim": (C.c_int, [C.POINTER(MimiStreamState), _i32]),
    "sopro_mimi_decode_stream": (C.c_int, [_p, _p, C.POINTER(MimiStreamState), _p, _i32, _p, _p]),
    "sopro_mimi_stream_batch_kv_bytes": (_i64, [_p, _i32, _i32]),
    "sopro_mimi_stream_batch_init": (C.c_int, [_p, C.POINTER(MimiStreamBatch), _p, _i32, _i32]),
    "sopro_mimi_stream_batch_trim": (C.c_int, [C.POINTER(MimiStreamBatch), _i32]),
    "sopro_mimi_stream_batch_keep": (C.c_int, [_p, C.POINTER(MimiStreamBatch), C.POINTER(_i32), _i32, _p]),
    "sopro_mimi_decode_stream_batch": (C.c_int, [_p, _p, C.POINTER(MimiStreamBatch), _p, _i32, _p, _p]),
    "sopro_ar_init": (C.c_int, [C.POINTER(ArState), _p]),
    "sopro_ar_sample": (C.c_int, [C.POINTER(ArState), _p, _i64, _p]),
    "sopro_ar_admit": (C.c_int, [C.POINTER(ArState), _i32, _p]),
    "sopro_ar_issue_frame": (C.c_int, [C.POINTER(ArFrame), _p]),
    "sopro_ar_fold_text": (C.c_int, [_p, _p, _p, _p, _p, _p, _p, _p, _p, _i32, _i32, _i32, _i32, _i32, _f32, _p]),
    "sopro_ar_fold_text_uk": (C.c_int, [_p, _p, _p, _p, _p, _p, _p, _p, _i32, _i32, _i32, _i32, _i32, _f32, _p]),
    "sopro_engine_upload_tensor": (C.c_int, [_p, C.c_char_p, _p, C.POINTER(_i64), _i32, _p]),
    "sopro_checkpoint_open": (C.c_int, [C.c_char_p, C.c_char_p, C.POINTER(_p)]),
    "sopro_checkpoint_close": (C.c_int, [_p]),
    "sopro_checkpoint_count": (_i32, [_p]),
    "sopro_checkpoint_tensor": (C.c_int, [_p, _i32, C.POINTER(C.c_char_p), C.POINTER(_p), C.POINTER(_i64), C.POINTER(_i32)]),
    "sopro_checkpoint_engine_cfg": (C.c_int, [_p, _i32, C.POINTER(EngineCfg)]),
    "sopro_engine_from_checkpoint": (C.c_int, [_p, _i32, _p, C.POINTER(_p)]),
    "sopro_engine_set_ar_tiles": (C.c_int, [_p, _i32, _i32, _i32, _i32]),
    "sopro_cond_workspace_bytes": (_i64, [_p, _i32, _i32, _i32]),
    "sopro_cond_prepare": (C.c_int, [_p, _p, _p, _p, _i32, _p, _p, _p, _p, _i64, _p, _p, _i32, _i32, _i32, _i32, _p, _p, _p, _p]),
    "sopro_film_coeffs": (C.c_int, [_p, _p, _f32, _i32, _p, _p, _p, _p]),
    "sopro_ref_workspace_bytes": (_i64, [_p, _i32]),
    "sopro_ref_prepare": (C.c_int, [_p, _p, _p, _i32, _p, _p, _p, _p]),
    "sopro_mimi_encode_workspace_bytes": (_i64, [_p, _i32, _i32]),
    "sopro_mimi_encode": (C.c_int, [_p, _p, _p, _i32, _i32, _p, _p]),
    "sopro_cvt_f32_bf16": (C.c_int, [_p, _p, _i64, _p]),
    "sopro_cvt_bf16_f32": (C.c_int, [_p, _p, _i64, _p]),
    "sopro_prof_enable": (C.c_int, [C.c_int]),
    "sopro_prof_collect": (C.c_int, [_p, _i32, _p]),
    "sopro_join_workspace_bytes": (_i64, [_i32, _i64, _i32]),
    "sopro_join_edges_f32": (C.c_int, [_p, _i64, _p, _i32, _i64, _i32, _f32, _i32, _i32, _p, _p, _p]),
    "sopro_join_layout_i64": (C.c_int, [_p, _p, _i32, _p, _p]),
    "sopro_join_mix_f32": (C.c_int, [_p, _i64, _p, _p, _p, _i32, _i32, _p, _i64, _p]),
    "sopro_tsm_out_len": (_i64, [_i64, _i64]),
    "sopro_tsm_blocks": (_i64, [_i64]),
    "sopro_tsm_chunk_out_cap": (_i64, [_i64]),
    "sopro_tsm_state_bytes": (_i64, [_i32]),
    "sopro_tsm_rows_f32": (C.c_int, [_p, _i64, _p, _i64, _p, _i32, _p, _i32, _p, _p, _i64, _i64, _p, _p, _i32, _p]),
    "sopro_pitch_out_len": (_i64, [_i64, _i64]),
    "sopro_pitch_chunk_out_cap": (_i64, [_i64]),
    "sopro_pitch_state_bytes": (_i64, [_i32]),
    "sopro_pitch_rows_f32": (C.c_int, [_p, _i64, _p, _i64, _p, _p, _p, _i32, _i32, _p, _i32, _p, _i64, _i64, _p, _p]),
    "sopro_wm_state_bytes": (_i64, [_i32]),
    "sopro_wm_chunk_out_cap": (_i64, [_i64]),
    "sopro_wm_fold_ws_bytes": (_i64, [_i32, _i64]),
    "sopro_wm_embed_rows_f32": (C.c_int, [_p, _i64, _p, _i64, _p, _p, _i32, _p, _i32, _p, _i32, _p, _p, _i64, _i64, _p, _p]),
    "sopro_wm_fold_rows_f32": (C.c_int, [_p, _i64, _p, _i64, _i32, _p, _p, _p, _p]),
    "sopro_wm_corr_rows_f32": (C.c_int, [_p, _p, _i32, _p, _i32, _p, _p]),
    "sopro_wm_peak_rows_f32": (C.c_int, [_p, _i32, _p, _p]),
    "sopro_sil_state_bytes": (_i64, [_i32]),
    "sopro_sil_chunk_out_cap": (_i64, [_i64]),
    "sopro_sil_ws_bytes": (_i64, [_i32, _i64]),
    "sopro_sil_rows_f32": (C.c_int, [_p, _i64, _p, _i64, _p, _p, _p, _i32, _p, _i32, _p, _p, _p, _i64, _i64, _p, _p, _i32, _p, _p]),
    "sopro_align_ws_bytes": (_i64, [_i32, _i32, _i32]),
    "sopro_align_scores_f32": (C.c_int, [_p, _i64, _i64, _p, _i64, _i64, _p, _p, _i32, _i32, _i32, _i32, _i32, _f32, C.c_uint32, _f32, _i32, _p, _i64,
                                         _i64, _p]),
    "sopro_align_dp_f32": (C.c_int, [_p, _i64, _i64, _p, _p, _i32, _i32, _i32, _p, _i64, _p, _i64, _p, _p, _p, _p]),
    "sopro_align_online_f32": (C.c_int, [_p, _i64, _i64, _p, _p, _p, _i32, _i32, _i32, _i32, _p, _p, _i64, _p]),
    "sopro_denoise_workspace_bytes": (_i64, [_i32, _i64]),
    "sopro_denoise_rows_f32": (C.c_int, [_p, _i64, _p, _p, _i32, _p, _i64, _p, _p, _i64, _p]),
}

_lib: Optional[C.CDLL] = None


class SoproHipError(RuntimeError):
    pass


def load() -> C.CDLL:
    global _lib
    if _lib is not None:
        return _lib
    path = os.environ.get("SOPRO_HIP_LIB") or LIB_PATH
    if not os.path.exists(path):
        raise SoproHipError(
            f"{path} not found: the HIP kernel library is not built. Run `python -c 'import __graft_entry__ as g; g.build()'` "
            "(or `make -C sopro_amd/csrc`). There is no CPU / torch fallback for the Sopro hot path.")
# ... 43 lines not shown
        for r in rows[: n.value]:
            d = out.setdefault(r.family.decode(), new())
            d["launches"] += r.launches
            d["flops"] += r.flops
            d["ms_all"] += r.ms_all
            d["gpu_bound"] += r.gpu_bound
            d["ms_bound"] += r.ms_bound
            d["flops_bound"] += r.flops_bound
        for fam, fl, e0, e1, bound in self.rec:
            d = out.setdefault(fam, new())
            t = e0.elapsed_time(e1)
            d["ms_all"] += t
            d["launches"] += 1
            d["flops"] += fl
            if bound:
                d["gpu_bound"] += 1
                d["ms_bound"] += t
                d["flops_bound"] += fl
        for d in out.values():
            if d["gpu_bound"] * 10 >= d["launches"] and d["ms_bound"] > 0:
                scale = (d["flops"] / d["flops_bound"]) if d["flops_bound"] > 0 else d["launches"] / d["gpu_bound"]
                d["ms"] = d["ms_bound"] * scale
            else:
                d["ms"] = d["ms_all"]
        return out


_prof: Optional[Profiler] = None
phase_log = None


def set_profiler(p: Optional[Profiler]) -> None:
    global _prof
    _prof = p
    load().sopro_prof_enable(1 if p is not None else 0)


def _check(rc: int, what: str) -> None:
    if rc != 0:
        raise SoproHipError(f"{what} failed ({rc}): {load().sopro_last_error().decode()}")


def _stream() -> int:
    return torch.cuda.current_stream().cuda_stream


def ptr(t: Optional[torch.Tensor], dtype: torch.dtype = torch.float32) -> Optional[int]:
    if t is None:
        return None
    if not t.is_cuda:
        raise SoproHipError("tensor is not on a HIP device: the Sopro hot path has no CPU fallback")
    if t.dtype != dtype:
        raise SoproHipError(f"expected {dtype}, got {t.dtype}")
    return t.data_ptr()


def gemm(A: torch.Tensor, W, Cout: torch.Tensor, *, M: int, N: int, K: int, lda: Optional[int] = None,
         ldc: Optional[int] = None, bias: Optional[torch.Tensor] = None, epilogue: int = EPI_NONE,
         prologue: int = PRO_NONE, R: Optional[torch.Tensor] = None, ldr: Optional[int] = None,
         scale: Optional[torch.Tensor] = None, pro_vec: Optional[torch.Tensor] = None, rows_per_seg: Optional[int] = None,
         a_seg_stride: int = 0, c_seg_stride: int = 0, r_seg_stride: int = 0, a_off: int = 0, c_off: int = 0,
         r_off: int = 0, ldw: Optional[int] = None, dbg: Optional[torch.Tensor] = None, a_split: bool = False, c_mode: int = 0,
         C2: Optional[torch.Tensor] = None, ldc2: Optional[int] = None, c2_seg_stride: int = 0,
         c2_off: int = 0, rms_eps: float = 0.0, range_events: Optional[torch.Tensor] = None, rope: Optional[tuple] = None,
         ln_stats: Optional[torch.Tensor] = None, ln_eps: float = 0.0, ln_stats_out: Optional[torch.Tensor] = None,
         long_k: Optional[bool] = None, ksplit: Optional[int] = None, group_m: Optional[int] = None) -> None:
    n_out = N // 2 if epilogue == EPI_GLU else N
    g = GemmArgs()
    a16 = A.dtype == torch.bfloat16
    c16 = c_mode in (6, 7, 8)
    cdt = torch.bfloat16 if c16 else torch.float32
    g.A = ptr(A, A.dtype if a16 else torch.float32) + (2 if a16 else 4) * a_off
    g.lda = K if lda is None else lda
    g.a_seg_stride = a_seg_stride
    packed = isinstance(W, PackedW)
    if packed and (W.N != N or W.K != K):
        raise SoproHipError(f"packed weight is [{W.N}, {W.K}], the call wants [{N}, {K}]")
    g.W = None if packed else ptr(W)
    g.ldw = K if ldw is None else ldw
    g.bias = ptr(bias)
    g.C = (ptr(Cout, cdt) + (2 if c16 else 4) * c_off) if Cout is not None else None
    g.ldc = n_out if ldc is None else ldc
    g.c_seg_stride = c_seg_stride
    g.R = (ptr(R, cdt) + (2 if c16 else 4) * r_off) if R is not None else None
    g.ldr = (n_out if ldr is None else ldr)
    g.r_seg_stride = r_seg_stride
    g.scale = ptr(scale)
    g.pro_vec = ptr(pro_vec)
    g.dbg = ptr(dbg, torch.int64)
    g.M, g.N, g.K = M, N, K
    g.rows_per_seg = M if rows_per_seg is None else rows_per_seg
    g.prologue, g.epilogue = prologue, epilogue
    e0 = _prof.begin() if _prof is not None else None
    x = None
    if packed:
        x = SplitExt()
        if rope is not None:
            x.rope_cos, x.rope_sin = ptr(rope[0]), ptr(rope[1])
            x.rope_cols, x.rope_dh, x.rope_pos0, x.rope_rows_per_seg = int(rope[2]), int(rope[3]), int(rope[4]), int(rope[5])
        if ln_stats is not None:
            x.ln_stats, x.rms_eps = ptr(ln_stats), float(ln_eps)
        x.ln_stats_out = ptr(ln_stats_out)
        if rms_eps > 0.0:
            if W.pieces == 2 and not W.f16:
                raise SoproHipError("fused RMSNorm is a six-pass (pieces = 3), f16 three-pass or one-pass (pieces = 1) feature")
            x.rms_norm, x.rms_eps = 1, float(rms_eps)
        if group_m is not None:
            x.group_m = int(group_m)
        if ksplit is not None:
            ks = int(ksplit)
            t64 = -(-M // 64) * -(-N // 64)
            if ks > 1 and (ks * t64 * 64 * 64 * 4 > _SPLITK_WS_BYTES or t64 > _SPLITK_TICKETS):
                raise SoproHipError(f"ksplit={ks}: {M} x {N} does not fit the split-K workspace / tickets of a stream")
        else:
            ks = _auto_ksplit(M, N, K, W.pieces, epilogue, W.f16) if (dbg is None and _splitk_enabled and rms_eps <= 0.0) else 1
        if ks > 1 or ksplit is not None:
            ws, tk = _splitk_buffers()
            x.ksplit, x.n_tickets, x.ws, x.ws_bytes, x.tickets = ks, int(tk.numel()), ptr(ws), int(ws.numel()) * 4, ptr(tk, torch.int32)
    if (a16 or c16) and not (packed and W.pieces == 1 and not W.f16):
        raise SoproHipError("bf16 rows (a_format 2, c_mode 6 / 7 / 8) belong to the one-pass (pieces = 1) path")
    if packed and W.f16:
        if a_split or c_mode not in (0, 5):
            raise SoproHipError("split-form operands belong to the bf16 three-pass (pieces = 2) path")
        if c_mode == 5:
            x.c_mode, x.C2, x.ldc2 = 5, ptr(C2) + 4 * c2_off, (-(-N // 64) if ldc2 is None else ldc2)
        x.acc_scale = W.acc_scale
        x.range_events = ptr(range_events, torch.int32)
        _check(load().sopro_gemm_f16x3(C.byref(g), ptr(W.data, torch.int32), C.byref(x), _stream()), "sopro_gemm_f16x3")
    elif packed and W.pieces == 1:
        if a_split or c_mode in (1, 2):
            raise SoproHipError("split-form operands belong to the three-pass (pieces = 2) path")
        x.c_mode = c_mode
        x.a_format = 2 if a16 else 0
        x.C2 = (ptr(C2, cdt) + (2 if c16 else 4) * c2_off) if C2 is not None else None
        x.ldc2, x.c2_seg_stride = (n_out if ldc2 is None else ldc2), c2_seg_stride
        _check(load().sopro_gemm_bf16x1(C.byref(g), ptr(W.data, torch.int32), C.byref(x), _stream()), "sopro_gemm_bf16x1")
    elif packed and W.pieces == 3:
        if a_split or c_mode not in (0, 5):
            raise SoproHipError("split-form operands belong to the three-pass (pieces = 2) path")
        if c_mode == 5:
            x.c_mode, x.C2, x.ldc2 = 5, ptr(C2) + 4 * c2_off, (-(-N // 64) if ldc2 is None else ldc2)
        _check(load().sopro_gemm_bf16x6(C.byref(g), ptr(W.data, torch.int32), C.byref(x), _stream()), "sopro_gemm_bf16x6")
    elif packed:
        if a16 or c16:
            raise SoproHipError("bf16 rows (a_format 2, c_mode 6 / 7 / 8) belong to the one-pass (pieces = 1) path")
        x.a_format, x.c_mode = int(bool(a_split)), c_mode
        x.C2 = (ptr(C2) + 4 * c2_off) if C2 is not None else None
        x.ldc2, x.c2_seg_stride = (n_out if ldc2 is None else ldc2), c2_seg_stride
        use_8p = long_k if long_k is not None else (W.rows is not None and bool(load().sopro_gemm_8p_takes(C.byref(g), C.byref(x))))
        if use_8p:
            if W.rows is None:
                raise SoproHipError("the long-K form needs the weight's split-form rows (pack_w_bf16x3(W, rows=True))")
            x.ksplit = 0
            _check(load().sopro_gemm_bf16x3_8p(C.byref(g), W.rows.data_ptr(), C.byref(x), _stream()), "sopro_gemm_bf16x3_8p")
        else:
            _check(load().sopro_gemm_bf16x3(C.byref(g), ptr(W.data, torch.int32), C.byref(x), _stream()), "sopro_gemm_bf16x3")
    elif a_split or c_mode:
        raise SoproHipError("split-plane operands need a PackedW weight (the fp32 kernel reads and writes fp32 rows)")
    elif ksplit is not None or group_m is not None:
        raise SoproHipError("ksplit / group_m belong to the packed-weight paths (sopro_gemm_split_ext)")
    else:
        _check(load().sopro_gemm_f32(C.byref(g), _stream()), "sopro_gemm_f32")
    if e0 is not None:
        fam = "gemm_f32_kernel" if not packed else ("gemm_f16x3_kernel" if W.f16 else {1: "gemm_bf16x1_kernel", 2: "gemm_bf16x3_kernel", 3: "gemm_bf16x6_kernel"}[W.pieces])
        _prof.end(fam, 2.0 * M * N * K, e0)


_splitk_enabled = True
_splitk_pool: dict = {}
_SPLITK_WS_BYTES = 32 << 20
_SPLITK_TICKETS = 1024


def _auto_ksplit(M: int, N: int, K: int, pieces: int, epilogue: int, f16: bool = False) -> int:
    return load().sopro_gemm_auto_ksplit(M, N, K, pieces, int(f16), epilogue, _SPLITK_WS_BYTES, _SPLITK_TICKETS)


def _splitk_buffers():
    key = _stream()
    bufs = _splitk_pool.get(key)
    if bufs is None:
        dev = torch.cuda.current_device()
        bufs = (torch.empty(_SPLITK_WS_BYTES // 4, dtype=torch.float32, device=f"cuda:{dev}"),
                torch.zeros(_SPLITK_TICKETS, dtype=torch.int32, device=f"cuda:{dev}"))
        _splitk_pool[key] = bufs
    return bufs


class PackedW:

    __slots__ = ("data", "N", "K", "pieces", "f16", "acc_scale", "rows")

    def __init__(self, data: torch.Tensor, N: int, K: int, pieces: int, f16: bool = False, acc_scale: float = 1.0):
        self.data, self.N, self.K, self.pieces, self.f16, self.acc_scale = data, N, K, pieces, f16, acc_scale
        self.rows = None


def pack_w_bf16(W: torch.Tensor, pieces: int) -> PackedW:
    if W.dim() != 2 or not W.is_contiguous():
        raise SoproHipError("pack_w_bf16 wants a contiguous [N, K] matrix")
    N, K = int(W.shape[0]), int(W.shape[1])
    lib = load()
    data = torch.empty(int(lib.sopro_packed_w_bytes(N, K, pieces)) // 4, dtype=torch.int32, device=W.device)
    _check(lib.sopro_pack_w_bf16(ptr(W), K, N, K, pieces, ptr(data, torch.int32), _stream()), "sopro_pack_w_bf16")
    return PackedW(data, N, K, pieces)


def pack_w_bf16x3(W: torch.Tensor, rows: bool = False) -> PackedW:
    pw = pack_w_bf16(W, 2)
    if rows:
        N, K = pw.N, pw.K
        lib = load()
        nb = int(lib.sopro_packed_w_rows_bytes(N, K))
        if nb <= 0:
            raise SoproHipError("split-form weight rows need K % 32 == 0")
        buf = torch.empty(nb // 4 + 32, dtype=torch.int32, device=W.device)
        off = (-buf.data_ptr() % 128) // 4
        pw.rows = buf[off: off + nb // 4]
        _check(lib.sopro_pack_w_rows_bf16(ptr(W), K, N, K, pw.rows.data_ptr(), _stream()), "sopro_pack_w_rows_bf16")
    return pw


def pack_w_f16x3(W: torch.Tensor) -> PackedW:
    if W.dim() != 2 or not W.is_contiguous():
        raise SoproHipError("pack_w_f16x3 wants a contiguous [N, K] matrix")
    import math

    N, K = int(W.shape[0]), int(W.shape[1])
    lib = load()
    amax = float(W.abs().max())
    wscale = 2.0 ** (13 - math.frexp(amax)[1] + 1) if amax > 0.0 else 1.0
    data = torch.empty(int(lib.sopro_packed_w_bytes(N, K, 2)) // 4, dtype=torch.int32, device=W.device)
    _check(lib.sopro_pack_w_f16x2(ptr(W), K, N, K, wscale, ptr(data, torch.int32), _stream()), "sopro_pack_w_f16x2")
    return PackedW(data, N, K, 2, f16=True, acc_scale=1.0 / (float(lib.sopro_f16x3_a_scale()) * wscale))


def pack_w_bf16x6(W: torch.Tensor) -> PackedW:
    return pack_w_bf16(W, 3)


def pack_w_bf16x1(W: torch.Tensor) -> PackedW:
    return pack_w_bf16(W, 1)


class SkinnyW:

    __slots__ = ("data", "N", "K", "glu", "bf16")

    def __init__(self, data: torch.Tensor, N: int, K: int, glu: bool, bf16: bool = False):
        self.data, self.N, self.K, self.glu, self.bf16 = data, N, K, glu, bf16


def pack_skinny_w(W: torch.Tensor, glu: bool = False, bf16: bool = False) -> SkinnyW:
    N, K = int(W.shape[0]), int(W.shape[1])
    n = int(load().sopro_skinny_packed_floats(N, K, int(glu)))
    if n <= 0:
        raise SoproHipError(f"pack_skinny_w: unsupported shape {N}x{K} (K % 32 == 0; glu: N even)")
    Wc = W.contiguous()
    with torch.cuda.device(W.device):
        if bf16:
            out = torch.empty(n // 2, dtype=torch.int32, device=W.device)
            _check(load().sopro_pack_skinny_w_bf16(ptr(Wc), K, N, K, int(glu), ptr(out, torch.int32), _stream()), "sopro_pack_skinny_w_bf16")
        else:
            out = torch.empty(n, dtype=torch.float32, device=W.device)
            _check(load().sopro_pack_skinny_w(ptr(Wc), K, N, K, int(glu), ptr(out), _stream()), "sopro_pack_skinny_w")
    return SkinnyW(out, N, K, bool(glu), bool(bf16))


def skinny(X: torch.Tensor, W, Y: torch.Tensor, *, B: int, N: int, K: int, ldx: Optional[int] = None,
           ldy: Optional[int] = None, rms_norm: bool = False, eps: float = 1e-6, bias: Optional[torch.Tensor] = None,
           epilogue: int = EPI_NONE, R: Optional[torch.Tensor] = None, ldr: Optional[int] = None,
           scale: Optional[torch.Tensor] = None, ring: Optional[torch.Tensor] = None, dw_w: Optional[torch.Tensor] = None,
           dw_b: Optional[torch.Tensor] = None, step: Optional[torch.Tensor] = None, ring_len: int = 0, ring_bcap: int = 0,
           dil: int = 1, ksize: int = 1, Xp: Optional[torch.Tensor] = None, np_: int = 0, xp_stride: int = 0,
           ksplit: bool = False, y_part_stride: int = 0, dbg: Optional[torch.Tensor] = None, mt: int = 1, nt: int = 1,
           aux_W=None, aux_Y: Optional[torch.Tensor] = None, aux_bias: Optional[torch.Tensor] = None, aux_R: Optional[torch.Tensor] = None,
           aux_flags: int = 0, aux_y_part_stride: int = 0) -> None:
    a = SkinnyArgs()
    a.X, a.ldx = ptr(X), (K if ldx is None else ldx)
    if isinstance(W, SkinnyW):
        if (W.N, W.K, W.glu) != (N, K, epilogue == EPI_GLU_DW):
            raise SoproHipError(f"packed weight is {W.N}x{W.K} glu={W.glu}, the call says {N}x{K} glu={epilogue == EPI_GLU_DW}")
        a.W, a.ldw, a.w_layout = (ptr(W.data, torch.int32), K, 2) if W.bf16 else (ptr(W.data), K, 1)
    else:
        a.W, a.ldw = ptr(W), K
    a.bias = ptr(bias)
    n_out = N // 2 if epilogue == EPI_GLU_DW else N
    a.Y, a.ldy = ptr(Y), (n_out if ldy is None else ldy)
    a.R, a.ldr, a.scale = ptr(R), (n_out if ldr is None else ldr), ptr(scale)
    ring_bf16 = ring is not None and ring.dtype == torch.bfloat16
    a.ring, a.dw_w, a.dw_b, a.step = ptr(ring, torch.bfloat16 if ring_bf16 else torch.float32), ptr(dw_w), ptr(dw_b), ptr(step, torch.int32)
    a.ring_format = 1 if ring_bf16 else 0
    a.Xp, a.xp_stride, a.y_part_stride, a.dbg = ptr(Xp), xp_stride, y_part_stride, ptr(dbg, torch.int64)
    a.eps = eps
    a.B, a.N, a.K, a.epilogue = B, N, K, epilogue
    a.ring_len, a.ring_bcap, a.dil, a.ksize = ring_len, ring_bcap, dil, ksize
    a.np, a.ksplit, a.rms_norm = np_, int(ksplit), int(rms_norm)
    a.mt, a.nt = int(mt), int(nt)
    if aux_W is not None:
        if not isinstance(aux_W, SkinnyW) or aux_W.K != K or aux_W.glu or aux_W.bf16 != (a.w_layout == 2):
            raise SoproHipError("aux_W must be a packed (non-GLU) weight of the same K and element type as W")
        a.aux_W = ptr(aux_W.data, torch.int32) if aux_W.bf16 else ptr(aux_W.data)
        a.aux_tiles, a.aux_flags = (aux_W.N + 15) // 16, int(aux_flags)
        a.aux_Y, a.aux_ldy, a.aux_bias, a.aux_R, a.aux_ldr = ptr(aux_Y), aux_W.N, ptr(aux_bias), ptr(aux_R), aux_W.N
        a.aux_y_part_stride = aux_y_part_stride
    _check(load().sopro_skinny_f32(C.byref(a), _stream()), "sopro_skinny_f32")


def norm(x: torch.Tensor, out: torch.Tensor, w: torch.Tensor, *, rows: int, C_: int, eps: float, kind: int = NORM_RMS,
         b: Optional[torch.Tensor] = None, mul: Optional[torch.Tensor] = None, add: Optional[torch.Tensor] = None,
         rows_per_seg: Optional[int] = None, ldx: Optional[int] = None, ldo: Optional[int] = None, x_off: int = 0,
         o_off: int = 0, x_seg_stride: int = 0) -> None:
    _check(load().sopro_norm_f32(ptr(x) + 4 * x_off, C_ if ldx is None else ldx, x_seg_stride, ptr(out) + 4 * o_off,
                                 C_ if ldo is None else ldo, ptr(w), ptr(b), ptr(mul), ptr(add), rows,
                                 rows if rows_per_seg is None else rows_per_seg, C_, eps, kind, _stream()), "sopro_norm_f32")


def row_stats(x: torch.Tensor, rows: int, C_: int, stats: torch.Tensor, ldx: Optional[int] = None, x_seg_stride: int = 0,
              rows_per_seg: Optional[int] = None, x_off: int = 0) -> None:
    _check(load().sopro_row_stats_f32(ptr(x) + 4 * x_off, C_ if ldx is None else ldx, x_seg_stride, rows, rows if rows_per_seg is None else rows_per_seg,
                                      C_, ptr(stats), _stream()), "sopro_row_stats_f32")


def rms_match(a: torch.Tensor, x: torch.Tensor, out: torch.Tensor, rows: int, C_: int) -> None:
    _check(load().sopro_rms_match_f32(ptr(a), ptr(x), ptr(out), rows, C_, _stream()), "sopro_rms_match_f32")


def tanh_affine(x: torch.Tensor, out: torch.Tensor, c0: float, c1: float, n: int) -> None:
    _check(load().sopro_tanh_affine_f32(ptr(x), ptr(out), c0, c1, n, _stream()), "sopro_tanh_affine_f32")


def add_pos(rowvec: torch.Tensor, table: torch.Tensor, out: torch.Tensor, B: int, T: int, C_: int, pos0: int = 0) -> None:
    _check(load().sopro_add_pos_f32(ptr(rowvec), ptr(table), ptr(out), B, T, C_, pos0, _stream()), "sopro_add_pos_f32")


def masked_mean(x: torch.Tensor, lens: Optional[torch.Tensor], out: torch.Tensor, B: int, T: int, C_: int) -> None:
    _check(load().sopro_masked_mean_f32(ptr(x), ptr(lens, torch.int32), ptr(out), B, T, C_, _stream()), "sopro_masked_mean_f32")


def stats_pool(h: torch.Tensor, logit: torch.Tensor, lens: Optional[torch.Tensor], out: torch.Tensor, B: int, T: int, C_: int) -> None:
    _check(load().sopro_stats_pool_f32(ptr(h), ptr(logit), ptr(lens, torch.int32), ptr(out), B, T, C_, _stream()), "sopro_stats_pool_f32")


def l2norm(x: torch.Tensor, out: torch.Tensor, rows: int, C_: int, eps: float = 1e-6) -> None:
    _check(load().sopro_l2norm_f32(ptr(x), ptr(out), rows, C_, eps, _stream()), "sopro_l2norm_f32")


def dwconv(x: torch.Tensor, w: torch.Tensor, bias: Optional[torch.Tensor], out: torch.Tensor, *, B: int, T: int, C_: int,
           ksize: int, dil: int, left: int, mode: int = 0, res: Optional[torch.Tensor] = None,
           lens: Optional[torch.Tensor] = None) -> None:
    _check(load().sopro_dwconv_f32(ptr(x), ptr(w), ptr(bias), ptr(res), ptr(out), ptr(lens, torch.int32), B, T, C_, ksize,
                                   dil, left, mode, _stream()), "sopro_dwconv_f32")


def codebook_sum(tok: torch.Tensor, ldt: int, col: torch.Tensor, off: torch.Tensor, wq: torch.Tensor, table: torch.Tensor,
                 out: torch.Tensor, *, rows: int, D: int, base: Optional[torch.Tensor] = None, alpha: float = 0.0,
                 beta: float = 1.0, ldo: Optional[int] = None, rows_per_seg: Optional[int] = None, o_seg_stride: int = 0,
                 o_off: int = 0, tok_off: int = 0) -> None:
    _check(load().sopro_codebook_sum_f32(ptr(tok, torch.int32) + 4 * tok_off, ldt, ptr(col, torch.int32), ptr(off, torch.int32),
                                         ptr(wq), int(col.numel()), ptr(table), int(table.shape[0]), ptr(base), alpha, beta,
                                         ptr(out) + 4 * o_off, D if ldo is None else ldo, o_seg_stride, rows,
                                         rows if rows_per_seg is None else rows_per_seg, D, _stream()), "sopro_codebook_sum_f32")


def text_embed(ids: torch.Tensor, lens: Optional[torch.Tensor], table: torch.Tensor, pe: torch.Tensor, out: torch.Tensor,
               B: int, T: int, C_: int) -> None:
    _check(load().sopro_text_embed_f32(ptr(ids, torch.int32), ptr(lens, torch.int32), ptr(table), int(table.shape[0]), ptr(pe),
                                       ptr(out), B, T, C_, _stream()), "sopro_text_embed_f32")


def argmax_rows(x: torch.Tensor, out: torch.Tensor, *, rows: int, N: int, ldx: Optional[int] = None, ldo: int = 1,
                o_off: int = 0, inner: int = 1) -> None:
    _check(load().sopro_argmax_rows_f32(ptr(x), N if ldx is None else ldx, ptr(out, torch.int32) + 4 * o_off, ldo, inner, rows, N,
# ... 1174 lines not shown
```

Before: 27630 audio-s/s.

## Add 16x16x32 bf16 MFMA variant of three-pass GEMMs with matching weight packing

Adds a K32 template path to the bf16x3 tiled and long-K 8-phase GEMM kernels. It uses 16x16x32 MFMA instructions in place of 32x32x16, together with a new weight packing layout, fragment offsets, accumulator blocks and epilogue indexing. The stage API selects this path by default for bf16 three-pass weights that have split rows, with SOPRO_GEMM_K32=0 to opt out. The aim is higher MFMA throughput or better issue overlap, at the cost of twice as many MFMA instructions and a new layout that must stay numerically correct.

```diff
diff --git a/include/sopro_hip.h b/include/sopro_hip.h
--- a/include/sopro_hip.h
+++ b/include/sopro_hip.h
@@ -70,6 +70,9 @@
 int sopro_pack_w_rows_bf16(const float* W, int64_t ldw, int32_t N, int32_t K, void* packed, void* stream);
 int sopro_gemm_8p_takes(const sopro_gemm_args* a, const sopro_gemm_split_ext* ext);
 int sopro_gemm_bf16x3_8p(const sopro_gemm_args* a, const void* w_rows, const sopro_gemm_split_ext* ext, void* stream);
+int sopro_pack_w_bf16_k32(const float* W, int64_t ldw, int32_t N, int32_t K, void* packed, void* stream);
+int sopro_gemm_bf16x3_k32(const sopro_gemm_args* a, const void* packed_w, const sopro_gemm_split_ext* ext, void* stream);
+int sopro_gemm_bf16x3_8p_k32(const sopro_gemm_args* a, const void* w_rows, const sopro_gemm_split_ext* ext, void* stream);
 int sopro_gemm_bf16x6(const sopro_gemm_args* a, const void* packed_w, const sopro_gemm_split_ext* ext, void* stream);
 int sopro_gemm_bf16x1(const sopro_gemm_args* a, const void* packed_w, const sopro_gemm_split_ext* ext, void* stream);
 int sopro_pack_w_bf16(const float* W, int64_t ldw, int32_t N, int32_t K, int32_t pieces, void* packed, void* stream);
diff --git a/sopro_amd/csrc/gemm_8p.hip b/sopro_amd/csrc/gemm_8p.hip
--- a/sopro_amd/csrc/gemm_8p.hip
+++ b/sopro_amd/csrc/gemm_8p.hip
@@ -22,7 +22,7 @@
   __builtin_amdgcn_global_load_lds((p_glb_void*)(uintptr_t)g, (p_lds_void*)(uintptr_t)lds_off, 16, 0, 0);
 }
 
-template <int EPI, int OUT>
+template <int EPI, int OUT, bool K32 = false>
 __global__ __launch_bounds__(P_NT, 1) void gemm_8p_kernel(const sopro_gemm_args g, const unsigned char* __restrict__ Wr, const sopro_gemm_split_ext ext) {
   extern __shared__ __attribute__((aligned(1024))) unsigned char smem[];
   const int tid = threadIdx.x, lane = tid & 63, wave = __builtin_amdgcn_readfirstlane(tid >> 6);
@@ -64,23 +64,24 @@
     dma16(src, lds0 + buf * P_BUF + (isW ? P_TILE : 0) + (128 * h + 8 * (wave + 8 * q)) * P_ROWB);
   };
 
-  const int frow = lane & 31, fg = lane >> 5;
+  const int frow = K32 ? (lane & 15) : (lane & 31), fg = K32 ? (lane >> 4) : (lane >> 5);
   const int swz = (frow >> 1) & 7;
   int foff[2][2];
 #pragma unroll
   for (int p = 0; p < 2; ++p)
 #pragma unroll
-    for (int s = 0; s < 2; ++s) foff[p][s] = ((p * 4 + s * 2 + fg) ^ swz) * 16;
+    for (int s = 0; s < 2; ++s) foff[p][s] = K32 ? ((p * 4 + fg) ^ swz) * 16 + s * 16 * P_ROWB : ((p * 4 + s * 2 + fg) ^ swz) * 16;
   const int arow = (wm * 32 + frow) * P_ROWB;
   const int brow = (wn * 32 + frow) * P_ROWB;
 
-  f32x16 acc[4][2];
+  typedef typename gemm_acc_block<K32>::type acc_t;
+  acc_t acc[4][2];
 #pragma unroll
   for (int i = 0; i < 4; ++i)
 #pragma unroll
     for (int j = 0; j < 2; ++j)
 #pragma unroll
-      for (int r = 0; r < 16; ++r) acc[i][j][r] = 0.f;
+      for (int r = 0; r < 16; ++r) acc_set(acc[i][j], r, 0.f);
 
   pu32x4 af[2][2][2];
   pu32x4 bf[2][2][2];
@@ -103,6 +104,22 @@
   auto phase_mfma = [&](int qi, int j, bool isW, int h, int kt, int buf) {
     constexpr int PA[3] = {1, 0, 0}, PB[3] = {0, 1, 0};
     int n = 0;
+    if constexpr (K32) {
+#pragma unroll
+      for (int q = 0; q < 3; ++q)
+#pragma unroll
+        for (int i = 0; i < 2; ++i)
+#pragma unroll
+          for (int sb = 0; sb < 4; ++sb) {
+            acc[qi * 2 + i][j][sb] = __builtin_amdgcn_mfma_f32_16x16x32_bf16(pfrag(af[i][sb >> 1][PA[q]]), pfrag(bf[j][sb & 1][PB[q]]), acc[qi * 2 + i][j][sb], 0, 0, 0);
+            ++n;
+            if (n == 8 || n == 16) {
+              __builtin_amdgcn_sched_barrier(0);
+              issue_one(isW, h, kt, buf, n == 8 ? 0 : 1);
+              __builtin_amdgcn_sched_barrier(0);
+            }
+          }
+    } else {
 #pragma unroll
     for (int s = 0; s < 2; ++s)
 #pragma unroll
@@ -117,6 +134,7 @@
             __builtin_amdgcn_sched_barrier(0);
           }
         }
+    }
   };
 #define P_PHASE(QI, J, W_, H_, KT_, B_)                     \
   asm volatile("s_waitcnt vmcnt(6)" ::: "memory");          \
@@ -167,9 +185,13 @@
 #pragma unroll
     for (int j = 0; j < 2; ++j) {
       const int nb = n0 + 128 * j;
-      const int n = nb + wn * 32 + frow;
-      const float bv[1] = {(g.bias && n < g.N) ? g.bias[n] : 0.f};
-      gemm_store_tile<2, 4, 1, 1, EPI, OUT>(g, Cs[(i * 2 + j) & 1], reinterpret_cast<f32x16(&)[1][1]>(acc[i][j]), bv, m0 + 64 * i, nb, &ext, nullptr);
+      float bv[K32 ? 2 : 1];
+#pragma unroll
+      for (int c = 0; c < (K32 ? 2 : 1); ++c) {
+        const int n = nb + wn * 32 + c * 16 + frow;
+        bv[c] = (g.bias && n < g.N) ? g.bias[n] : 0.f;
+      }
+      gemm_store_tile<2, 4, 1, 1, EPI, OUT, K32>(g, Cs[(i * 2 + j) & 1], reinterpret_cast<acc_t(&)[1][1]>(acc[i][j]), bv, m0 + 64 * i, nb, &ext, nullptr);
     }
 }
 
@@ -191,9 +213,9 @@
   out[i] = make_uint4(w[0], w[1], w[2], w[3]);
 }
 
-template <int EPI, int OUT>
+template <int EPI, int OUT, bool K32>
 int launch_8p(const sopro_gemm_args& g, const void* wrows, const sopro_gemm_split_ext& ext, hipStream_t s) {
-  auto kern = gemm_8p_kernel<EPI, OUT>;
+  auto kern = gemm_8p_kernel<EPI, OUT, K32>;
   SOPRO_SET_MAX_LDS_ONCE(kern, P_LDS);
   const int ntm = (g.M + P_BM - 1) / P_BM, ntn = g.N / P_BN;
   hipLaunchKernelGGL(kern, dim3(ntm * ntn), dim3(P_NT), P_LDS, s, g, reinterpret_cast<const unsigned char*>(wrows), ext);
@@ -227,25 +249,35 @@
   return tiles >= 128 ? 1 : 0;
 }
 
-extern "C" int sopro_gemm_bf16x3_8p(const sopro_gemm_args* a, const void* w_rows, const sopro_gemm_split_ext* x, void* stream) {
-  SOPRO_CHECK_ARG(a != nullptr && x != nullptr && w_rows != nullptr, "args / ext / w_rows is NULL");
+template <bool K32>
+static int gemm_8p(const char* who, const sopro_gemm_args* a, const void* w_rows, const sopro_gemm_split_ext* x, void* stream) {
+  SOPRO_CHECK_AS(who, a != nullptr && x != nullptr && w_rows != nullptr, "args / ext / w_rows is NULL");
   sopro_gemm_args g = *a;
   sopro_gemm_split_ext ext = *x;
-  if (int rc = gemm_check_basic(__func__, g, &ext, w_rows, GEMM_SPLIT_ROWS)) return rc;
-  SOPRO_CHECK_ARG((g.N % P_BN) == 0 && (g.K & 31) == 0, "the long-K form takes N % 256 == 0, K % 32 == 0");
-  SOPRO_CHECK_ARG(ext.a_format == 1 && g.prologue == SOPRO_PRO_NONE, "A must be split-form rows (a_format 1, no prologue)");
-  SOPRO_CHECK_ARG(g.epilogue == SOPRO_EPI_NONE && !ext.rms_norm && !ext.ln_stats && !ext.ln_stats_out && ext.ksplit <= 1,
+  if (ext.group_m == 0) ext.group_m = sopro_gemm_default_group_m();
+  if (int rc = gemm_check_basic(who, g, &ext, w_rows, GEMM_SPLIT_ROWS)) return rc;
+  SOPRO_CHECK_AS(who, (g.N % P_BN) == 0 && (g.K & 31) == 0, "the long-K form takes N % 256 == 0, K % 32 == 0");
+  SOPRO_CHECK_AS(who, ext.a_format == 1 && g.prologue == SOPRO_PRO_NONE, "A must be split-form rows (a_format 1, no prologue)");
+  SOPRO_CHECK_AS(who, g.epilogue == SOPRO_EPI_NONE && !ext.rms_norm && !ext.ln_stats && !ext.ln_stats_out && ext.ksplit <= 1,
                   "epilogue NONE, no fused norm, no split-K");
-  SOPRO_CHECK_ARG(g.A && g.C && (reinterpret_cast<uintptr_t>(g.A) & 127u) == 0 && (g.lda & 31) == 0 && (g.a_seg_stride & 31) == 0,
+  SOPRO_CHECK_AS(who, g.A && g.C && (reinterpret_cast<uintptr_t>(g.A) & 127u) == 0 && (g.lda & 31) == 0 && (g.a_seg_stride & 31) == 0,
                   "split-form A: 128-byte aligned base, lda / a_seg_stride multiples of 32");
-  SOPRO_CHECK_ARG((reinterpret_cast<uintptr_t>(w_rows) & 127u) == 0, "w_rows must be 128-byte aligned (sopro_pack_w_rows_bf16)");
-  SOPRO_CHECK_ARG(ext.c_mode == 0 || ext.c_mode == 1 || ext.c_mode == 2 || ext.c_mode == 4, "c_mode must be 0, 1, 2 or 4");
-  if (int rc = gemm_check_out_rows(__func__, g, ext, true)) return rc;
+  SOPRO_CHECK_AS(who, (reinterpret_cast<uintptr_t>(w_rows) & 127u) == 0, "w_rows must be 128-byte aligned (sopro_pack_w_rows_bf16)");
+  SOPRO_CHECK_AS(who, ext.c_mode == 0 || ext.c_mode == 1 || ext.c_mode == 2 || ext.c_mode == 4, "c_mode must be 0, 1, 2 or 4");
+  if (int rc = gemm_check_out_rows(who, g, ext, true)) return rc;
   hipStream_t s = reinterpret_cast<hipStream_t>(stream);
   switch (ext.c_mode) {
-    case 0: return launch_8p<SOPRO_EPI_NONE, 0>(g, w_rows, ext, s);
-    case 1: return launch_8p<SOPRO_EPI_NONE, 1>(g, w_rows, ext, s);
-    case 2: return launch_8p<SOPRO_EPI_NONE, 2>(g, w_rows, ext, s);
-    default: return launch_8p<SOPRO_EPI_NONE, 4>(g, w_rows, ext, s);
-  }
-}
+    case 0: return launch_8p<SOPRO_EPI_NONE, 0, K32>(g, w_rows, ext, s);
+    case 1: return launch_8p<SOPRO_EPI_NONE, 1, K32>(g, w_rows, ext, s);
+    case 2: return launch_8p<SOPRO_EPI_NONE, 2, K32>(g, w_rows, ext, s);
+    default: return launch_8p<SOPRO_EPI_NONE, 4, K32>(g, w_rows, ext, s);
+  }
+}
+
+extern "C" int sopro_gemm_bf16x3_8p(const sopro_gemm_args* a, const void* w_rows, const sopro_gemm_split_ext* x, void* stream) {
+  return gemm_8p<false>(__func__, a, w_rows, x, stream);
+}
+
+extern "C" int sopro_gemm_bf16x3_8p_k32(const sopro_gemm_args* a, const void* w_rows, const sopro_gemm_split_ext* x, void* stream) {
+  return gemm_8p<true>(__func__, a, w_rows, x, stream);
+}
diff --git a/sopro_amd/csrc/gemm_bf16s.hip b/sopro_amd/csrc/gemm_bf16s.hip
--- a/sopro_amd/csrc/gemm_bf16s.hip
+++ b/sopro_amd/csrc/gemm_bf16s.hip
@@ -35,9 +35,10 @@
   }
 }
 
-template <int NPL, int WM, int WN, int TM, int TN, int EPI, int AMODE, int OUT, bool SK, bool F16 = false>
+template <int NPL, int WM, int WN, int TM, int TN, int EPI, int AMODE, int OUT, bool SK, bool F16 = false, bool K32 = false>
 __global__ __launch_bounds__(WM* WN * 64) void gemm_bf16s_kernel(const sopro_gemm_args g, const uint4* __restrict__ Wp,
                                                                  int ksubs, const sopro_gemm_split_ext ext) {
+  static_assert(!K32 || (NPL == 2 && !F16), "the 16x16x32 form is built for the bf16 three-pass kernels");
   constexpr int AROW = NPL * 64 + 16;
   constexpr bool FOLD = F16;
   constexpr int NT = WM * WN * 64;
@@ -91,10 +92,17 @@
     const int t = min((n0 >> 5) + wn * TN + j, ntiles - 1);
     boff[j] = (t * ksubs * NPL) * 64 + lane;
   }
-  float biasv[TN];
-#pragma unroll
-  for (int j = 0; j < TN; ++j) {
-    const int n = n0 + (wn * TN + j) * 32 + (lane & 31);
+  int boff16[K32 ? TN : 1][2];
+  if constexpr (K32) {
+#pragma unroll
+    for (int j = 0; j < TN; ++j)
+#pragma unroll
+      for (int cj = 0; cj < 2; ++cj) boff16[j][cj] = boff[j] + cj * (ksubs >> 1) * NPL * 64;
+  }
+  float biasv[TN * (K32 ? 2 : 1)];
+#pragma unroll
+  for (int j = 0; j < TN * (K32 ? 2 : 1); ++j) {
+    const int n = K32 ? n0 + wn * TN * 32 + j * 16 + (lane & 15) : n0 + (wn * TN + j) * 32 + (lane & 31);
     biasv[j] = (g.bias && n < g.N) ? g.bias[n] : 0.f;
   }
 
@@ -133,7 +141,10 @@
 #pragma unroll
       for (int s = 0; s < 2; ++s)
 #pragma unroll
-        for (int p = 0; p < NPL; ++p) rb[j][s][p] = bp[j][((int64_t)(kt * 2 + s) * NPL + p) * 64];
+        for (int p = 0; p < NPL; ++p) {
+          if constexpr (K32) rb[j][s][p] = Wp[boff16[j][s] + (kt * NPL + p) * 64];
+          else rb[j][s][p] = bp[j][((int64_t)(kt * 2 + s) * NPL + p) * 64];
+        }
   };
   auto lstore_piece = [&](int buf, float4 (&ra)[A_F4], const float4& pv, int i, bool fresh, bool first) {
     if constexpr (FOLD) {
@@ -193,20 +204,39 @@
     for (int i = 0; i < A_F4; ++i) lstore_piece(buf, ra, pv, i, fresh, first);
   };
 
-  f32x16 acc[TM][TN];
+  typename gemm_acc_block<K32>::type acc[TM][TN];
 #pragma unroll
   for (int i = 0; i < TM; ++i)
 #pragma unroll
     for (int j = 0; j < TN; ++j)
 #pragma unroll
-      for (int r = 0; r < 16; ++r) acc[i][j][r] = 0.f;
-
-  const int frow = lane & 31, fg = lane >> 5;
+      for (int r = 0; r < 16; ++r) acc_set(acc[i][j], r, 0.f);
+
+  const int frow = K32 ? (lane & 15) : (lane & 31), fg = K32 ? (lane >> 4) : (lane >> 5);
   constexpr int NPAIR = NPL == 1 ? 1 : (NPL == 2 ? 3 : 6);
   constexpr int PA[6] = {NPL == 1 ? 0 : (NPL == 2 ? 1 : 2), 0, NPL == 2 ? 0 : 1, 1, 0, 0};
   constexpr int PB[6] = {0, NPL == 2 ? 1 : 2, NPL == 2 ? 0 : 1, 0, 1, 0};
   auto compute = [&](int buf, const uint4 (&rb)[TN][2][NPL]) {
     const unsigned char* a = As + buf * BM * AROW + (wm * TM * 32 + frow) * AROW + fg * 16;
+    if constexpr (K32) {
+#pragma unroll
+      for (int ri = 0; ri < 2; ++ri) {
+        uint4 af[TM][NPL];
+#pragma unroll
+        for (int i = 0; i < TM; ++i)
+#pragma unroll
+          for (int p = 0; p < NPL; ++p) af[i][p] = *reinterpret_cast<const uint4*>(a + (i * 32 + ri * 16) * AROW + p * 64);
+#pragma unroll
+        for (int q = 0; q < NPAIR; ++q)
+#pragma unroll
+          for (int i = 0; i < TM; ++i)
+#pragma unroll
+            for (int j = 0; j < TN; ++j)
+#pragma unroll
+              for (int cj = 0; cj < 2; ++cj)
+                acc[i][j][2 * ri + cj] = __builtin_amdgcn_mfma_f32_16x16x32_bf16(as_frag(af[i][PA[q]]), as_frag(rb[j][cj][PB[q]]), acc[i][j][2 * ri + cj], 0, 0, 0);
+      }
+    } else {
 #pragma unroll
     for (int s = 0; s < 2; ++s) {
       uint4 af[TM][NPL];
@@ -225,19 +255,25 @@
             else
               acc[i][j] = __builtin_amdgcn_mfma_f32_32x32x16_bf16(as_frag(af[i][PA[q]]), as_frag(rb[j][s][PB[q]]), acc[i][j], 0, 0, 0);
     }
+    }
   };
 
   auto compute_spread = [&](int buf, const uint4 (&rb)[TN][2][NPL], int kA, float4 (&ra)[A_F4], float4& pv, int kB, uint4 (&rbn)[TN][2][NPL],
                             float4 (&rs)[A_F4], const float4& pvs, bool fresh_s) {
-    constexpr int NB = TN * 2 * NPL, NL = NB + A_F4, NM = 2 * NPAIR * TM * TN;
+    constexpr int NB = TN * 2 * NPL, NL = NB + A_F4, NM = (K32 ? 4 : 2) * NPAIR * TM * TN;
     constexpr int STRIDE = NM / NL > 0 ? NM / NL : 1;
     const int kcol = min(kA * BK + lc4 * 4, klast);
     if (AMODE == 3) pv = *reinterpret_cast<const float4*>(g.pro_vec + kcol);
     auto issue = [&](int n) {
       if (n < NB) {
         const int j = n / (2 * NPL), ss = (n / NPL) % 2, p = n % NPL;
-        const uint4* wk = Wp + (int64_t)__builtin_amdgcn_readfirstlane(kB) * (2 * NPL * 64);
-        rbn[j][ss][p] = wk[boff[j] + (ss * NPL + p) * 64];
+        if constexpr (K32) {
+          const uint4* wk = Wp + (int64_t)__builtin_amdgcn_readfirstlane(kB) * (NPL * 64);
+          rbn[j][ss][p] = wk[boff16[j][ss] + p * 64];
+        } else {
+          const uint4* wk = Wp + (int64_t)__builtin_amdgcn_readfirstlane(kB) * (2 * NPL * 64);
+          rbn[j][ss][p] = wk[boff[j] + (ss * NPL + p) * 64];
+        }
       } else if (n < NL) {
         const int i = n - NB;
         if constexpr (AMODE == 5) {
@@ -251,6 +287,32 @@
     };
     const unsigned char* a = As + buf * BM * AROW + (wm * TM * 32 + frow) * AROW + fg * 16;
     int m = 0, nl = 0;
+    if constexpr (K32) {
+#pragma unroll
+      for (int ri = 0; ri < 2; ++ri) {
+        uint4 af[TM][NPL];
+#pragma unroll
+        for (int i = 0; i < TM; ++i)
+#pragma unroll
+          for (int p = 0; p < NPL; ++p) af[i][p] = *reinterpret_cast<const uint4*>(a + (i * 32 + ri * 16) * AROW + p * 64);
+#pragma unroll
+        for (int q = 0; q < NPAIR; ++q)
+#pragma unroll
+          for (int i = 0; i < TM; ++i)
+#pragma unroll
+            for (int j = 0; j < TN; ++j)
+#pragma unroll
+              for (int cj = 0; cj < 2; ++cj) {
+                acc[i][j][2 * ri + cj] = __builtin_amdgcn_mfma_f32_16x16x32_bf16(as_frag(af[i][PA[q]]), as_frag(rb[j][cj][PB[q]]), acc[i][j][2 * ri + cj], 0, 0, 0);
+                ++m;
+                if (m % STRIDE == 0 && nl < NL) {
+                  __builtin_amdgcn_sched_barrier(0x786);
+                  issue(nl++);
+                  __builtin_amdgcn_sched_barrier(0x786);
+                }
+              }
+      }
+    } else {
 #pragma unroll
     for (int s = 0; s < 2; ++s) {
       uint4 af[TM][NPL];
@@ -290,6 +352,7 @@
             }
           }
     }
+    }
 #pragma unroll
     for (int n = 0; n < NL; ++n)
       if (n >= nl) issue(n);
@@ -356,7 +419,8 @@
       for (int j = 0; j < TN; ++j)
 #pragma unroll
         for (int r = 0; r < 16; r += 4)
-          *reinterpret_cast<float4*>(mine + (i * TN + j) * 16 + r) = make_float4(acc[i][j][r], acc[i][j][r + 1], acc[i][j][r + 2], acc[i][j][r + 3]);
+          *reinterpret_cast<float4*>(mine + (i * TN + j) * 16 + r) =
+              make_float4(acc_get(acc[i][j], r), acc_get(acc[i][j], r + 1), acc_get(acc[i][j], r + 2), acc_get(acc[i][j], r + 3));
     __syncthreads();
     int* flag = reinterpret_cast<int*>(smem4);
     if (tid == 0) {
@@ -374,7 +438,7 @@
 #pragma unroll
       for (int j = 0; j < TN; ++j)
 #pragma unroll
-        for (int r = 0; r < 16; ++r) acc[i][j][r] = 0.f;
+        for (int r = 0; r < 16; ++r) acc_set(acc[i][j], r, 0.f);
     const int64_t sl_stride = (int64_t)ntile * NT * PER_THREAD;
     const float* part0 = ext.ws + ((int64_t)tile * NT + tid) * PER_THREAD;
     for (int s0 = 0; s0 < KS; s0 += 16) {
@@ -393,7 +457,8 @@
 #pragma unroll
             for (int u = 0; u < 16; ++u) {
               if (s0 + u < KS) {
-                acc[i][j][r] += v[u][0]; acc[i][j][r + 1] += v[u][1]; acc[i][j][r + 2] += v[u][2]; acc[i][j][r + 3] += v[u][3];
+#pragma unroll
+                for (int e = 0; e < 4; ++e) acc_set(acc[i][j], r + e, acc_get(acc[i][j], r + e) + v[u][e]);
               }
             }
           }
@@ -420,11 +485,11 @@
     __syncthreads();
     rs = rsl;
   }
-  gemm_store_tile<WM, WN, TM, TN, EPI, OUT>(g, reinterpret_cast<float*>(smem4), acc, biasv, m0, n0, &ext, rs, cscale);
+  gemm_store_tile<WM, WN, TM, TN, EPI, OUT, K32>(g, reinterpret_cast<float*>(smem4), acc, biasv, m0, n0, &ext, rs, cscale);
   if (dbg && tid == 0) dbg[3] = clock64();
 }
 
-template <int NPL, bool F16 = false>
+template <int NPL, bool F16 = false, bool K32 = false>
 __global__ __launch_bounds__(256) void pack_w_kernel(const float* __restrict__ W, int64_t ldw, int N, int K, uint4* __restrict__ out,
                                                      int ksubs, int64_t total, float wscale = 1.0f) {
   const int64_t i = (int64_t)blockIdx.x * blockDim.x + threadIdx.x;
@@ -433,10 +498,11 @@
   const int64_t pk = i >> 6;
   const int p = (int)(pk % NPL);
   const int64_t tk = pk / NPL;
-  const int ks = (int)(tk % ksubs);
-  const int t = (int)(tk / ksubs);
-  const int n = t * 32 + (lane & 31);
-  const int k0 = ks * 16 + (lane >> 5) * 8;
+  const int kdiv = K32 ? ksubs >> 1 : ksubs;
+  const int ks = (int)(tk % kdiv);
+  const int t = (int)(tk / kdiv);
+  const int n = K32 ? t * 16 + (lane & 15) : t * 32 + (lane & 31);
+  const int k0 = K32 ? ks * 32 + (lane >> 4) * 8 : ks * 16 + (lane >> 5) * 8;
   unsigned w[4];
 #pragma unroll
   for (int e = 0; e < 4; ++e) {
@@ -451,13 +517,18 @@
   out[i] = make_uint4(w[0], w[1], w[2], w[3]);
 }
 
-template <int NPL, int WM, int WN, int TM, int TN, int EPI, int AMODE, int OUT, bool F16 = false>
+template <int NPL, int WM, int WN, int TM, int TN, int EPI, int AMODE, int OUT, bool F16 = false, bool K32 = false>
 int launch_one(const sopro_gemm_args& g, const uint4* wp, int ksubs, const sopro_gemm_split_ext& ext, hipStream_t s) {
   constexpr int BM = WM * TM * 32, BN = WN * TN * 32;
   constexpr size_t lds_main = (size_t)2 * BM * (NPL * 64 + 16), lds_epi = (size_t)BM * (BN + 4 + (AMODE == 4 ? 1 : 0)) * sizeof(float);
   constexpr size_t lds = lds_main > lds_epi ? lds_main : lds_epi;
   const int ks = ext.ksplit > 1 ? ext.ksplit : 1;
-  auto kern = ks > 1 ? gemm_bf16s_kernel<NPL, WM, WN, TM, TN, EPI, AMODE, OUT, true, F16> : gemm_bf16s_kernel<NPL, WM, WN, TM, TN, EPI, AMODE, OUT, false, F16>;
+  constexpr bool NO_SK = K32 && TM * TN >= 8;
+  if (NO_SK && ks > 1) {
+    sopro_set_error("the 256 x 128 tile of the 16x16x32 form takes no split-K");
+    return -2;
+  }
+  auto kern = (ks > 1 && !NO_SK) ? gemm_bf16s_kernel<NPL, WM, WN, TM, TN, EPI, AMODE, OUT, !NO_SK, F16, K32> : gemm_bf16s_kernel<NPL, WM, WN, TM, TN, EPI, AMODE, OUT, false, F16, K32>;
   constexpr size_t lds_cap = lds > (size_t)96 * 1024 ? lds : (size_t)96 * 1024;
   if (ks > 1) SOPRO_SET_MAX_LDS_ONCE(kern, lds_cap);
   else SOPRO_SET_MAX_LDS_ONCE(kern, lds_cap);
@@ -483,11 +554,11 @@
   return g.prologue == SOPRO_PRO_ELU ? 1 : (g.prologue == SOPRO_PRO_ADDVEC ? 3 : 0);
 }
 
-template <int NPL, int WM, int WN, int TM, int TN>
+template <int NPL, int WM, int WN, int TM, int TN, bool K32 = false>
 int launch_cfg3(const sopro_gemm_args& g, const uint4* wp, int ksubs, const sopro_gemm_split_ext& ext, hipStream_t s) {
   const int key = g.epilogue * 100 + amode_of(g, ext) * 10 + ext.c_mode;
 #define SOPRO_CASE(E, A, O) \
-  case (E) * 100 + (A) * 10 + (O): return launch_one<NPL, WM, WN, TM, TN, ((E) == SOPRO_EPI_GELU ? SOPRO_EPI_GELU_FAST : (E)), A, O>(g, wp, ksubs, ext, s)
+  case (E) * 100 + (A) * 10 + (O): return launch_one<NPL, WM, WN, TM, TN, ((E) == SOPRO_EPI_GELU ? SOPRO_EPI_GELU_FAST : (E)), A, O, false, K32>(g, wp, ksubs, ext, s)
   switch (key) {
     SOPRO_CASE(SOPRO_EPI_NONE, 0, 0);
     SOPRO_CASE(SOPRO_EPI_GELU, 0, 0);
@@ -608,7 +679,7 @@
   hipStream_t s;
 };
 
-template <int NPL, bool F16, Form FORM>
+template <int NPL, bool F16, Form FORM, bool K32 = false>
 int launch_tile(Tile t, const Call& c) {
   switch (t) {
 #define SOPRO_TILE(T, WM, WN, TM, TN)                                                                                                     \
@@ -616,7 +687,7 @@
     if constexpr (!has_tile<NPL, F16, FORM>(T)) break;                                                                                    \
     else if constexpr (FORM == FORM_ARGMAX) return launch_one<NPL, WM, WN, TM, TN, SOPRO_EPI_NONE, 0, 5, F16>(c.g, c.wp, c.ksubs, c.ext, c.s); \
     else if constexpr (FORM == FORM_CFG6) return launch_cfg6<NPL, WM, WN, TM, TN, F16>(c.g, c.wp, c.ksubs, c.ext, c.s);                  \
-    else return launch_cfg3<NPL, WM, WN, TM, TN>(c.g, c.wp, c.ksubs, c.ext, c.s);
+    else return launch_cfg3<NPL, WM, WN, TM, TN, K32>(c.g, c.wp, c.ksubs, c.ext, c.s);
     SOPRO_TILES(SOPRO_TILE)
 #undef SOPRO_TILE
   }
@@ -728,6 +799,8 @@
   return 0;
 }
 
+int sopro_gemm_default_group_m() { return g_group_m; }
+
 static bool eight_waves(const sopro_gemm_args& g) {
   static const bool on = SOPRO_DEV_ENV("SOPRO_GEMM_W8") != nullptr && SOPRO_DEV_ENV("SOPRO_GEMM_W8")[0] == '1';
   return on && g.N >= 512 && g.M >= 1024;
@@ -781,26 +854,37 @@
   SOPRO_LAUNCH_CHECK();
 }
 
-extern "C" int sopro_gemm_bf16x3(const sopro_gemm_args* a, const void* packed_w, const sopro_gemm_split_ext* x, void* stream) {
+extern "C" int sopro_pack_w_bf16_k32(const float* W, int64_t ldw, int32_t N, int32_t K, void* packed, void* stream) {
+  SOPRO_CHECK_ARG(W && packed && N > 0 && K > 0 && ldw >= K, "bad pointers or sizes");
+  SOPRO_CHECK_ARG(aligned16(packed), "packed must be 16-byte aligned");
+  const int ksubs = (K + 31) / 32 * 2;
+  const int64_t total = (int64_t)((N + 31) / 32) * ksubs * 2 * 64;
+  hipLaunchKernelGGL((pack_w_kernel<2, false, true>), dim3((unsigned)((total + 255) / 256)), dim3(256), 0, (hipStream_t)stream, W, ldw, N, K,
+                     reinterpret_cast<uint4*>(packed), ksubs, total);
+  SOPRO_LAUNCH_CHECK();
+}
+
+template <bool K32>
+static int gemm_bf16x3(const char* who, const sopro_gemm_args* a, const void* packed_w, const sopro_gemm_split_ext* x, void* stream) {
   Call c;
-  if (int rc = prepare(__func__, a, packed_w, x, stream, false, nullptr, c)) return rc;
+  if (int rc = prepare(who, a, packed_w, x, stream, false, nullptr, c)) return rc;
   const sopro_gemm_args& g = c.g;
   const sopro_gemm_split_ext& ext = c.ext;
-  SOPRO_CHECK_ARG(g.prologue == SOPRO_PRO_NONE || g.prologue == SOPRO_PRO_ELU, "prologue must be NONE or ELU");
-  SOPRO_CHECK_ARG(g.epilogue == SOPRO_EPI_NONE || g.epilogue == SOPRO_EPI_GELU || g.epilogue == SOPRO_EPI_RES || g.epilogue == SOPRO_EPI_ROPE,
+  SOPRO_CHECK_AS(who, g.prologue == SOPRO_PRO_NONE || g.prologue == SOPRO_PRO_ELU, "prologue must be NONE or ELU");
+  SOPRO_CHECK_AS(who, g.epilogue == SOPRO_EPI_NONE || g.epilogue == SOPRO_EPI_GELU || g.epilogue == SOPRO_EPI_RES || g.epilogue == SOPRO_EPI_ROPE,
                   "epilogue must be NONE, GELU, RES or ROPE");
   if (int rc = check_rope(g, ext)) return rc;
-  SOPRO_CHECK_ARG(ext.a_format == 0 || ext.a_format == 1, "a_format must be 0 (fp32) or 1 (split form)");
-  SOPRO_CHECK_ARG(!ext.rms_norm, "fused RMSNorm is a six-pass (sopro_gemm_bf16x6) feature");
+  SOPRO_CHECK_AS(who, ext.a_format == 0 || ext.a_format == 1, "a_format must be 0 (fp32) or 1 (split form)");
+  SOPRO_CHECK_AS(who, !ext.rms_norm, "fused RMSNorm is a six-pass (sopro_gemm_bf16x6) feature");
   if (ext.a_format == 1) {
-    SOPRO_CHECK_ARG(g.prologue == SOPRO_PRO_NONE, "split-form A carries its activation already");
-    SOPRO_CHECK_ARG((g.K & 31) == 0 && (g.lda & 31) == 0 && (g.a_seg_stride & 31) == 0 && (reinterpret_cast<uintptr_t>(g.A) & 127u) == 0,
+    SOPRO_CHECK_AS(who, g.prologue == SOPRO_PRO_NONE, "split-form A carries its activation already");
+    SOPRO_CHECK_AS(who, (g.K & 31) == 0 && (g.lda & 31) == 0 && (g.a_seg_stride & 31) == 0 && (reinterpret_cast<uintptr_t>(g.A) & 127u) == 0,
                     "split-form A: K, lda, a_seg_stride multiples of 32 and a 128-byte aligned base");
   }
-  SOPRO_CHECK_ARG(ext.c_mode >= 0 && ext.c_mode <= 4, "c_mode must be 0..4");
-  if (int rc = gemm_check_out_rows(__func__, g, ext, true)) return rc;
+  SOPRO_CHECK_AS(who, ext.c_mode >= 0 && ext.c_mode <= 4, "c_mode must be 0..4");
+  if (int rc = gemm_check_out_rows(who, g, ext, true)) return rc;
 #ifdef SOPRO_DEV_SWITCHES
-  if (g_tile_override == 9 && sopro_gemm_astat_takes(g, ext)) return sopro_gemm_astat_bf16x3(g, packed_w, c.s);
+  if (!K32 && g_tile_override == 9 && sopro_gemm_astat_takes(g, ext)) return sopro_gemm_astat_bf16x3(g, packed_w, c.s);
 #endif
   Tile t = default_tile(BF16X3, g.M, g.N, g.epilogue);
   static const bool narrow = SOPRO_DEV_ENV("SOPRO_GEMM_NARROW") != nullptr && SOPRO_DEV_ENV("SOPRO_GEMM_NARROW")[0] == '1';
@@ -817,7 +901,15 @@
 #endif
     default: break;
   }
-  return launch_tile<2, false, FORM_CFG3>(t, c);
+  return launch_tile<2, false, FORM_CFG3, K32>(t, c);
+}
+
+extern "C" int sopro_gemm_bf16x3(const sopro_gemm_args* a, const void* packed_w, const sopro_gemm_split_ext* x, void* stream) {
+  return gemm_bf16x3<false>(__func__, a, packed_w, x, stream);
+}
+
+extern "C" int sopro_gemm_bf16x3_k32(const sopro_gemm_args* a, const void* packed_w, const sopro_gemm_split_ext* x, void* stream) {
+  return gemm_bf16x3<true>(__func__, a, packed_w, x, stream);
 }
 
 extern "C" int sopro_gemm_bf16x1(const sopro_gemm_args* a, const void* packed_w, const sopro_gemm_split_ext* x, void* stream) {
diff --git a/sopro_amd/csrc/gemm_epilogue.h b/sopro_amd/csrc/gemm_epilogue.h
--- a/sopro_amd/csrc/gemm_epilogue.h
+++ b/sopro_amd/csrc/gemm_epilogue.h
@@ -3,9 +3,17 @@
 
 constexpr int SOPRO_EPI_GELU_FAST = 100;
 constexpr int SOPRO_EPI_GLU_FAST = 101;
-template <int WM, int WN, int TM, int TN, int EPI, int OUT = 0>
-__device__ __forceinline__ void gemm_store_tile(const sopro_gemm_args& g, float* __restrict__ Cs, f32x16 (&acc)[TM][TN],
-                                                const float (&biasv)[TN], int m0, int n0,
+typedef f32x4 f32x4x4[4];
+template <bool K32> struct gemm_acc_block { typedef f32x16 type; };
+template <> struct gemm_acc_block<true> { typedef f32x4x4 type; };
+__device__ __forceinline__ float acc_get(const f32x16& a, int r) { return a[r]; }
+__device__ __forceinline__ float acc_get(const f32x4x4& a, int r) { return a[r >> 2][r & 3]; }
+__device__ __forceinline__ void acc_set(f32x16& a, int r, float v) { a[r] = v; }
+__device__ __forceinline__ void acc_set(f32x4x4& a, int r, float v) { a[r >> 2][r & 3] = v; }
+
+template <int WM, int WN, int TM, int TN, int EPI, int OUT = 0, bool K32 = false, class ACC>
+__device__ __forceinline__ void gemm_store_tile(const sopro_gemm_args& g, float* __restrict__ Cs, ACC (&acc)[TM][TN],
+                                                const float (&biasv)[TN * (K32 ? 2 : 1)], int m0, int n0,
                                                 const sopro_gemm_split_ext* __restrict__ ext = nullptr,
                                                 const float* __restrict__ rs = nullptr, float cscale = 1.0f) {
   constexpr int NT = WM * WN * 64;
@@ -51,12 +59,13 @@
     }
   }
   {
-    const int col = lane & 31;
+    const int col = K32 ? (lane & 15) : (lane & 31);
 #pragma unroll
     for (int i = 0; i < TM; ++i)
 #pragma unroll
       for (int k = 0; k < 4; ++k) {
-        const int row0 = (wm * TM + i) * 32 + 8 * k + 4 * (lane >> 5);
+        const int row0 = (wm * TM + i) * 32 + (K32 ? 16 * (k >> 1) + 4 * (lane >> 4) : 8 * k + 4 * (lane >> 5));
+        const int cofs = K32 ? 16 * (k & 1) : 0;
         float rs4[4] = {cscale, cscale, cscale, cscale};
         if (rs) {
           const float4 t = *reinterpret_cast<const float4*>(rs + row0);
@@ -66,9 +75,9 @@
         for (int j = 0; j < TN; ++j)
 #pragma unroll
           for (int e = 0; e < 4; ++e) {
-            float p = acc[i][j][4 * k + e] * rs4[e];
+            float p = acc_get(acc[i][j], 4 * k + e) * rs4[e];
             if (rs) asm("" : "+v"(p));
-            Cs[(row0 + e) * CLD + (wn * TN + j) * 32 + col] = p + biasv[j];
+            Cs[(row0 + e) * CLD + (wn * TN + j) * 32 + cofs + col] = p + biasv[K32 ? 2 * j + (k & 1) : j];
           }
       }
   }
diff --git a/sopro_amd/csrc/gemm_host.h b/sopro_amd/csrc/gemm_host.h
--- a/sopro_amd/csrc/gemm_host.h
+++ b/sopro_amd/csrc/gemm_host.h
@@ -8,6 +8,8 @@
       return -2;                                              \
     }                                                         \
   } while (0)
+
+int sopro_gemm_default_group_m();
 
 enum gemm_operands {
   GEMM_F32_ROWS,
diff --git a/sopro_amd/csrc/stages.hip b/sopro_amd/csrc/stages.hip
--- a/sopro_amd/csrc/stages.hip
+++ b/sopro_amd/csrc/stages.hip
@@ -27,6 +27,7 @@
   const void* rows = nullptr;
   int pieces = 0;
   bool f16 = false;
+  bool k32 = false;
   float acc_scale = 1.f;
 };
 
@@ -153,6 +154,7 @@
   }
   const bool f16 = pieces == F16X2;
   if (f16) pieces = 2;
+  static const bool k32_off = getenv("SOPRO_GEMM_K32") && getenv("SOPRO_GEMM_K32")[0] == '0';
   const int64_t bytes = sopro_packed_w_bytes(N, K, pieces);
   char* dst;
   STG(dev_alloc(e, (size_t)bytes, &dst));
@@ -168,6 +170,9 @@
     STG(sopro_pack_w_f16x2(src, K, N, K, wscale, dst, s));
     w.f16 = true;
     w.acc_scale = 1.0f / (sopro_f16x3_a_scale() * wscale);
+  } else if (with_rows && pieces == 2 && (K & 31) == 0 && !k32_off) {
+    STG(sopro_pack_w_bf16_k32(src, K, N, K, dst, s));
+    w.k32 = true;
   } else {
     STG(sopro_pack_w_bf16(src, K, N, K, pieces, dst, s));
   }
@@ -309,9 +314,9 @@
     if (w.rows) {
       sopro_gemm_split_ext x8 = x;
       x8.ksplit = 0;
-      if (sopro_gemm_8p_takes(&g, &x8)) return sopro_gemm_bf16x3_8p(&g, w.rows, &x8, s);
-    }
-    return sopro_gemm_bf16x3(&g, w.packed, &x, s);
+      if (sopro_gemm_8p_takes(&g, &x8)) return w.k32 ? sopro_gemm_bf16x3_8p_k32(&g, w.rows, &x8, s) : sopro_gemm_bf16x3_8p(&g, w.rows, &x8, s);
+    }
+    return w.k32 ? sopro_gemm_bf16x3_k32(&g, w.packed, &x, s) : sopro_gemm_bf16x3(&g, w.packed, &x, s);
   }
   if (!g.W) {
     sopro_set_error("stage API: a contraction has neither an fp32 nor a packed weight");
diff --git a/sopro_amd/hip.py b/sopro_amd/hip.py
--- a/sopro_amd/hip.py
+++ b/sopro_amd/hip.py
@@ -142,6 +142,9 @@
     "sopro_gemm_bf16x6": (C.c_int, [_p, _p, _p, _p]),
     "sopro_gemm_bf16x1": (C.c_int, [_p, _p, _p, _p]),
     "sopro_pack_w_bf16": (C.c_int, [_p, _i64, _i32, _i32, _i32, _p, _p]),
+    "sopro_pack_w_bf16_k32": (C.c_int, [_p, _i64, _i32, _i32, _p, _p]),
+    "sopro_gemm_bf16x3_k32": (C.c_int, [_p, _p, _p, _p]),
+    "sopro_gemm_bf16x3_8p_k32": (C.c_int, [_p, _p, _p, _p]),
     "sopro_fill2d_u32": (C.c_int, [_p, _i64, _i32, _i32, C.c_uint32, _p]),
     "sopro_copy2d_u32": (C.c_int, [_p, _i64, _p, _i64, _i32, _i32, _p]),
     "sopro_pack_w_f16x2": (C.c_int, [_p, _i64, _i32, _i32, _f32, _p, _p]),
@@ -491,7 +494,10 @@
             if W.rows is None:
                 raise SoproHipError("the long-K form needs the weight's split-form rows (pack_w_bf16x3(W, rows=True))")
             x.ksplit = 0
-            _check(load().sopro_gemm_bf16x3_8p(C.byref(g), W.rows.data_ptr(), C.byref(x), _stream()), "sopro_gemm_bf16x3_8p")
+            fn = "sopro_gemm_bf16x3_8p_k32" if W.k32 else "sopro_gemm_bf16x3_8p"
+            _check(getattr(load(), fn)(C.byref(g), W.rows.data_ptr(), C.byref(x), _stream()), fn)
+        elif W.k32:
+            _check(load().sopro_gemm_bf16x3_k32(C.byref(g), ptr(W.data, torch.int32), C.byref(x), _stream()), "sopro_gemm_bf16x3_k32")
         else:
             _check(load().sopro_gemm_bf16x3(C.byref(g), ptr(W.data, torch.int32), C.byref(x), _stream()), "sopro_gemm_bf16x3")
     elif a_split or c_mode:
@@ -528,10 +534,11 @@
 
 class PackedW:
 
-    __slots__ = ("data", "N", "K", "pieces", "f16", "acc_scale", "rows")
+    __slots__ = ("data", "N", "K", "pieces", "f16", "acc_scale", "rows", "k32")
 
     def __init__(self, data: torch.Tensor, N: int, K: int, pieces: int, f16: bool = False, acc_scale: float = 1.0):
         self.data, self.N, self.K, self.pieces, self.f16, self.acc_scale = data, N, K, pieces, f16, acc_scale
+        self.k32 = False
         self.rows = None
 
 
@@ -546,7 +553,10 @@
 
 
 def pack_w_bf16x3(W: torch.Tensor, rows: bool = False) -> PackedW:
-    pw = pack_w_bf16(W, 2)
+    return _with_rows(pack_w_bf16(W, 2), W, rows)
+
+
+def _with_rows(pw: PackedW, W: torch.Tensor, rows: bool) -> PackedW:
     if rows:
         N, K = pw.N, pw.K
         lib = load()
@@ -558,6 +568,18 @@
         pw.rows = buf[off: off + nb // 4]
         _check(lib.sopro_pack_w_rows_bf16(ptr(W), K, N, K, pw.rows.data_ptr(), _stream()), "sopro_pack_w_rows_bf16")
     return pw
+
+
+def pack_w_bf16x3_k32(W: torch.Tensor, rows: bool = False) -> PackedW:
+    if W.dim() != 2 or not W.is_contiguous():
+        raise SoproHipError("pack_w_bf16x3_k32 wants a contiguous [N, K] matrix")
+    N, K = int(W.shape[0]), int(W.shape[1])
+    lib = load()
+    data = torch.empty(int(lib.sopro_packed_w_bytes(N, K, 2)) // 4, dtype=torch.int32, device=W.device)
+    _check(lib.sopro_pack_w_bf16_k32(ptr(W), K, N, K, ptr(data, torch.int32), _stream()), "sopro_pack_w_bf16_k32")
+    pw = PackedW(data, N, K, 2)
+    pw.k32 = True
+    return _with_rows(pw, W, rows)
 
 
 def pack_w_f16x3(W: torch.Tensor) -> PackedW:
```

After: 27650 audio-s/s (median of 2 runs). About the same (+0.1%).
